# apple/ml-stable-diffusion

Hardware: AMD Instinct MI355X
Metric: diffusion iter/s (UNet steps/s), SD2.1-base 512x512 fp16 (higher is better)
Workload: dtype fp16; 1 GPU; BASELINE config 2: SD2.1-base (865.9 M-parameter UNet), random-init, denoising iteration at 512x512 (64x64 latents), CFG batch 2 per prompt, DDIM, device-resident loop; unet=sd21-base, latent=64, attention=ORIGINAL, prompts_per_gpu=1, global_batch=2, hip_graph=True, parallelism=dp1 (independent prompts per rank, no data-path collective)

## Files before the change

include/sd_mi355x.h:

```cpp
#ifndef SD_MI355X_H
#define SD_MI355X_H

#include <stddef.h>
#include <stdint.h>

#ifdef __cplusplus
extern "C" {
#endif

typedef enum sd_status {
  SD_OK = 0,
  SD_ERR_INVALID_ARGUMENT = -1,
  SD_ERR_NOT_FOUND = -2,
  SD_ERR_HIP = -3,
  SD_ERR_UNSUPPORTED = -4,
  SD_ERR_INTERNAL = -5
} sd_status;

typedef enum sd_dtype { SD_F16 = 0, SD_F32 = 1 } sd_dtype;

typedef enum sd_attention_impl {
  SD_ATTN_ORIGINAL = 0,
  SD_ATTN_SPLIT_EINSUM = 1,
  SD_ATTN_SPLIT_EINSUM_V2 = 2
} sd_attention_impl;

const char* sd_last_error(void);
const char* sd_version(void);
int sd_device_count(void);

typedef struct sd_weights sd_weights;
int sd_weights_create(sd_weights** out);
int sd_weights_add(sd_weights* w, const char* name, const void* data, sd_dtype dtype, const int64_t* shape,
                   int ndim);
int sd_weights_load_safetensors(sd_weights* w, const char* path, const char* prefix);
int sd_weights_count(const sd_weights* w);
void sd_weights_destroy(sd_weights* w);

#define SD_MAX_LEVELS 6

typedef struct sd_unet_config {
  int32_t batch;
  int32_t in_channels, out_channels;
  int32_t height, width;
  int32_t n_levels;
  int32_t block_out_channels[SD_MAX_LEVELS];
  int32_t down_cross_attn[SD_MAX_LEVELS];
  int32_t up_cross_attn[SD_MAX_LEVELS];
  int32_t layers_per_block;
  int32_t attention_head_dim[SD_MAX_LEVELS];
  int32_t transformer_layers_per_block[SD_MAX_LEVELS];
  int32_t cross_attention_dim;
  int32_t context_len;
  int32_t norm_num_groups;
  float norm_eps;
  int32_t flip_sin_to_cos;
  float freq_shift;
  int32_t addition_time_embed_dim;
  int32_t projection_class_embeddings_input_dim;
  int32_t num_time_ids;
  int32_t support_controlnet;
  int32_t is_controlnet;
  int32_t is_vae_decoder;
  int32_t attention_impl;
  int32_t use_graph;
  int32_t compute_fp32;
} sd_unet_config;

typedef struct sd_unet sd_unet;

int sd_unet_create(const sd_unet_config* cfg, const sd_weights* w, int device, sd_unet** out);
void sd_unet_destroy(sd_unet* u);
int sd_unet_set_attention(sd_unet* u, int impl);
int sd_unet_num_residuals(const sd_unet* u);
size_t sd_unet_device_bytes(const sd_unet* u);

#define SD_FLAG_DEVICE_PTRS 1

typedef struct sd_unet_io {
  const void* sample;
  const void* timestep;
  const void* encoder_hidden_states;
  const void* time_ids;
  const void* text_embeds;
  const void* controlnet_cond;
  const void* const* additional_residuals;
  int32_t num_additional_residuals;
  void* noise_pred;
  void* const* residual_outputs;
  int32_t flags;
  const float* step_noise;
} sd_unet_io;

int sd_unet_forward(sd_unet* u, const sd_unet_io* io);

int sd_unet_time_forward(sd_unet* u, int warmup, int iters, float* ms_per_iter);

int sd_unet_profile(sd_unet* u, int iters, int cap, float* ms, double* flop, char* labels, int label_bytes,
                    int* n_ops);

int sd_tune_set_candidate(int tile, int staging, int splitk);
int sd_tune_set_plan_table(const char* rows, sd_unet* u, int* n_plans);

int sd_unet_denoise_loop(sd_unet* u, const sd_unet_io* io, float* latents, int n_images, int n_steps,
                         const float* timesteps, const float* coef, const float* sample_scale, int history,
                         float guidance_scale, float* history_io, float* ms_per_step);

int sd_unet_attach_controlnets(sd_unet* u, sd_unet* const* controlnets, int n);
int sd_controlnet_set_cond(sd_unet* controlnet, const void* controlnet_cond, int flags);

int sd_vae_decoder_create(const sd_unet_config* cfg, const sd_weights* w, int device, sd_unet** out);
int sd_vae_decode(sd_unet* vae, const void* z, sd_dtype z_dtype, float* image, int flags);
int sd_vae_encoder_create(const sd_unet_config* cfg, const sd_weights* w, int device, sd_unet** out);
int sd_vae_encode(sd_unet* vae, const void* x, sd_dtype x_dtype, float* moments, int flags);

typedef struct sd_text_encoder_config {
  int32_t vocab_size, hidden_size, intermediate_size, num_hidden_layers, num_attention_heads;
  int32_t max_position_embeddings;
  int32_t hidden_act;
  int32_t projection_dim;
  float layer_norm_eps;
  int32_t use_graph;
} sd_text_encoder_config;
typedef struct sd_text_encoder sd_text_encoder;
int sd_text_encoder_create(const sd_text_encoder_config* cfg, const sd_weights* w, int device, sd_text_encoder** out);
void sd_text_encoder_destroy(sd_text_encoder* t);
size_t sd_text_encoder_device_bytes(const sd_text_encoder* t);
int sd_text_encoder_encode(sd_text_encoder* t, const int32_t* input_ids, int eos_index, float* last_hidden_state,
                           float* hidden_embeds, float* pooled);

int sd_op_attention(int impl, const void* q, const void* k, const void* v, void* out, int B, int heads, int d,
                    int Sq, int Sk, int variant, int iters, float* ms);
int sd_op_layernorm(const void* x, const float* weight, const float* bias, void* out, int B, int C, int S, float eps,
                    int iters, float* ms);
int sd_op_groupnorm(const void* x, const float* weight, const float* bias, void* out, int B, int C, int H, int W,
                    int groups, float eps, int silu, int iters, float* ms);
int sd_op_groupnorm_shortcut(const void* x0, const void* x1, const float* gn_weight, const float* gn_bias, const void* w, const float* bias,
                             void* out_gn, void* out_sc, int B, int C0, int C1, int H, int W, int N, int groups, float eps, int silu,
                             int side, int iters, float* ms);
int sd_op_conv2d(const void* x, const void* w, const float* bias, const void* res, void* out, int B, int Cin, int H,
                 int W, int Cout, int ksize, int stride, int upsample, int tile, int splitk, int force_generic,
                 int iters, float* ms);
int sd_op_conv2d_groupnorm(const void* x, const void* w, const float* bias, const void* res, const float* gn_weight,
                           const float* gn_bias, void* conv_out, void* out, int B, int Cin, int H, int W, int Cout, int ksize,
                           int groups, float eps, int silu, int tile, int producer_stats, int* entries, int iters, float* ms);
int sd_op_conv2d_groupnorm_proj(const void* x, const void* w, const float* bias, const void* res, const float* gn_weight,
                                const float* gn_bias, const void* proj_w, const float* proj_bias, void* conv_out, void* out, int B,
                                int Cin, int H, int W, int Cout, int ksize, int Nproj, int groups, float eps, int fold, int tile,
                                int* entries, int iters, float* ms);
int sd_op_conv2d_groupnorm_conv3x3(const void* x, const void* w, const float* bias, const void* res, const float* gn_weight,
                                   const float* gn_bias, const void* w2, const float* bias2, const void* res2, void* conv_out, void* out,
                                   int B, int Cin, int H, int W, int Cout, int ksize, int N2, int groups, float eps, int silu, int fold,
                                   int tile, int staging2, int* entries, int iters, float* ms);
int sd_op_ffn_out_proj(const void* g, const void* w1, const float* b1, const void* res1, const void* w2, const float* b2, const void* res2,
                       void* out, float* gn_sums, int B, int C, int S, int groups, int fused, int iters, float* ms);
int sd_op_cross_attention_fused(const void* x, const float* ln_weight, const float* ln_bias, const void* wq, const void* k,
                                const void* v, void* out, int B, int heads, int Sq, int Sk, float eps, int nst, int iters,
                                float* ms);
int sd_op_cross_attention_block(const void* x, const float* ln_weight, const float* ln_bias, const void* wq, const void* k, const void* v,
                                const void* wo, const float* bo, const void* a1, const void* wo1, const float* bo1, void* out, int B, int heads,
                                int Sq, int Sk, float eps, int fused, int iters, float* ms);
int sd_op_geglu(const void* x, const void* w, const float* bias, void* out, int M, int C, int N2, int iters, float* ms);
int sd_op_geglu_ln(const void* x, const float* ln_weight, const float* ln_bias, const void* w, const float* bias, void* out, int M, int C,
                   int N2, float eps, int kernel, int iters, float* ms);
int sd_op_qkv_ln(const void* x, const float* ln_weight, const float* ln_bias, const void* w, void* out_qk, void* out_vt, int B, int HW, int C,
                 float eps, float q_scale, int vt_perm, int kernel, int iters, float* ms);
int sd_op_gn_proj_qkv(const void* x_in, const void* conv_w, const float* gn_weight, const float* gn_bias, const void* proj_w,
                      const float* proj_bias, const float* ln_weight, const float* ln_bias, const void* wqkv, void* out_h, void* out_qk,
                      void* out_vt, int B, int H, int W, int C, int groups, float gn_eps, float ln_eps, float q_scale, int vt_perm, int fused,
                      int* entries, int iters, float* ms);
int sd_op_timestep_embedding(const float* t, float* out, int n, int dim, int flip_sin_to_cos, float freq_shift);
int sd_numpy_randn(uint32_t seed, double* out, size_t n);
int sd_torch_randn(uint32_t seed, double* out, size_t n);
int sd_philox_randn(uint64_t seed, uint32_t offset, double* out, size_t n);
int sd_calibrate(int device, float* out9);
int sd_selftest_mfma(void);

#ifdef __cplusplus
}
#endif
#endif
```

ml-stable-diffusion_amd/csrc/capi.cpp:

```cpp
#include <algorithm>
#include <climits>
#include <cmath>
#include <cstdlib>
#include <cstring>

#include "unet.h"

namespace sd {
extern thread_local std::string g_last_error;
int selftest_mfma();

namespace {

template <typename F>
int guarded(F&& f) {
  try {
    f();
    g_last_error.clear();
    return kOk;
  } catch (const Error& e) {
    g_last_error = e.what();
    return e.code;
  } catch (const std::bad_alloc&) {
    g_last_error = "out of host memory";
// ... 316 lines not shown
    {
      size_t pb = 0;
      int nc = 0;
      if (perm && attention8_sk_scratch(a, &pb, &nc)) {
        a.sk_part = reinterpret_cast<float*>(sc.dev<char>(pb));
        a.sk_part_bytes = pb;
        a.sk_cnt = sc.dev<unsigned>(nc);
        a.sk_cnt_n = nc;
        SD_HIP(hipMemset(a.sk_cnt, 0, (size_t)nc * sizeof(unsigned)));
      } else {
        SD_REQUIRE(variant < 100, kInvalidArgument, "attention variant %d: the balanced form cannot run this shape", variant);
      }
    }
    sc.timed(iters, ms, [&] { launch_attention(a, sc.stream); });
    std::vector<half_t> ot((size_t)B * Sq * C);
    SD_HIP(hipMemcpy(ot.data(), o, ot.size() * 2, hipMemcpyDeviceToHost));
    half_t* oh = reinterpret_cast<half_t*>(out);
    for (int b = 0; b < B; ++b)
      for (int c = 0; c < C; ++c)
        for (int s = 0; s < Sq; ++s) oh[((size_t)b * C + c) * Sq + s] = ot[((size_t)b * Sq + s) * C + c];
  });
}

int sd_op_layernorm(const void* x, const float* weight, const float* bias, void* out, int B, int C, int S, float eps,
                    int iters, float* ms) {
  return guarded([&] {
    SD_REQUIRE(x && weight && bias && out, kInvalidArgument, "NULL argument");
    Scratch sc;
    std::vector<half_t> xt = nchw_to_nhwc(reinterpret_cast<const half_t*>(x), B, C, 1, S);
    half_t* dx = sc.dev<half_t>(xt.size(), xt.data());
    half_t* dy = sc.dev<half_t>(xt.size());
    float* dw = sc.dev<float>(C, weight);
    float* db = sc.dev<float>(C, bias);
    sc.timed(iters, ms, [&] { launch_layernorm(dx, dw, db, dy, B * S, C, eps, sc.stream); });
    SD_HIP(hipMemcpy(xt.data(), dy, xt.size() * 2, hipMemcpyDeviceToHost));
    nhwc_to_nchw(xt.data(), reinterpret_cast<half_t*>(out), B, C, 1, S);
  });
}

int sd_op_groupnorm(const void* x, const float* weight, const float* bias, void* out, int B, int C, int H, int W,
                    int groups, float eps, int silu, int iters, float* ms) {
  return guarded([&] {
    SD_REQUIRE(x && weight && bias && out, kInvalidArgument, "NULL argument");
    Scratch sc;
    std::vector<half_t> xt = nchw_to_nhwc(reinterpret_cast<const half_t*>(x), B, C, H, W);
    half_t* dx = sc.dev<half_t>(xt.size(), xt.data());
    half_t* dy = sc.dev<half_t>(xt.size());
    float* dw = sc.dev<float>(C, weight);
    float* db = sc.dev<float>(C, bias);
    float* partial = sc.dev<float>(groupnorm_scratch_floats(B, H * W, groups));
    sc.timed(iters, ms, [&] {
      launch_groupnorm(dx, C, nullptr, 0, partial, dw, db, dy, B, H * W, groups, eps, silu, sc.stream);
    });
    SD_HIP(hipMemcpy(xt.data(), dy, xt.size() * 2, hipMemcpyDeviceToHost));
    nhwc_to_nchw(xt.data(), reinterpret_cast<half_t*>(out), B, C, H, W);
  });
}

int sd_op_groupnorm_shortcut(const void* x0, const void* x1, const float* gn_weight, const float* gn_bias, const void* w, const float* bias,
                             void* out_gn, void* out_sc, int B, int C0, int C1, int H, int W, int N, int groups, float eps, int silu,
                             int side, int iters, float* ms) {
  return guarded([&] {
    SD_REQUIRE(x0 && gn_weight && gn_bias && w && out_gn && out_sc, kInvalidArgument, "NULL argument");
    if (!x1) C1 = 0;
    const int C = C0 + C1;
    Scratch sc;
    std::vector<half_t> x0t = nchw_to_nhwc(reinterpret_cast<const half_t*>(x0), B, C0, H, W);
    half_t* d0 = sc.dev<half_t>(x0t.size(), x0t.data());
    half_t* d1 = nullptr;
    if (x1) {
      std::vector<half_t> x1t = nchw_to_nhwc(reinterpret_cast<const half_t*>(x1), B, C1, H, W);
      d1 = sc.dev<half_t>(x1t.size(), x1t.data());
    }
    const size_t gn_n = (size_t)B * H * W * C, sc_n = (size_t)B * H * W * N;
    half_t* dy = sc.dev<half_t>(gn_n);
    half_t* ds = sc.dev<half_t>(sc_n);
    float* dgw = sc.dev<float>(C, gn_weight);
    float* dgb = sc.dev<float>(C, gn_bias);
    float* partial = sc.dev<float>(groupnorm_scratch_floats(B, H * W, groups));
    ConvDesc d;
    d.x0 = d0;
    d.C0 = C0;
    d.x1 = d1;
    d.C1 = C1;
    d.w = sc.dev<half_t>((size_t)N * C, reinterpret_cast<const half_t*>(w));
    d.bias = bias ? sc.dev<float>(N, bias) : nullptr;
    d.out = ds;
    d.B = B; d.Hi = H; d.Wi = W; d.Ho = H; d.Wo = W;
    d.N = N;
    SD_REQUIRE(conv_fast_path_ok(d), kInvalidArgument, "groupnorm_shortcut: C0=%d C1=%d N=%d not MFMA-tileable", C0, C1, N);
    SD_REQUIRE(!side || gn_side_gemm_ok(d), kUnsupported, "groupnorm_shortcut: the GEMM cannot ride in the GroupNorm launch (M=%d)", B * H * W);
    ConvWorkspace ws;
    ws.partial_bytes = conv_workspace_bytes(d);
    if (ws.partial_bytes) ws.partial = reinterpret_cast<float*>(sc.dev<char>(ws.partial_bytes));
    sc.timed(iters, ms, [&] {
      if (side) {
        launch_groupnorm(d0, C0, d1, C1, partial, dgw, dgb, dy, B, H * W, groups, eps, silu, sc.stream, 0, &d);
      } else {
        launch_groupnorm(d0, C0, d1, C1, partial, dgw, dgb, dy, B, H * W, groups, eps, silu, sc.stream);
        launch_conv(d, ws, sc.stream);
      }
    });
    std::vector<half_t> ot(gn_n);
    SD_HIP(hipMemcpy(ot.data(), dy, gn_n * 2, hipMemcpyDeviceToHost));
    nhwc_to_nchw(ot.data(), reinterpret_cast<half_t*>(out_gn), B, C, H, W);
    ot.resize(sc_n);
    SD_HIP(hipMemcpy(ot.data(), ds, sc_n * 2, hipMemcpyDeviceToHost));
    nhwc_to_nchw(ot.data(), reinterpret_cast<half_t*>(out_sc), B, N, H, W);
  });
}

int sd_op_conv2d(const void* x, const void* w, const float* bias, const void* res, void* out, int B, int Cin, int H,
                 int W, int Cout, int ksize, int stride, int upsample, int tile, int splitk, int force_generic,
                 int iters, float* ms) {
  return guarded([&] {
    SD_REQUIRE(x && w && out, kInvalidArgument, "NULL argument");
    SD_REQUIRE((ksize == 1 || ksize == 3) && (stride == 1 || stride == 2) && (upsample == 0 || upsample == 1),
               kInvalidArgument, "conv2d: ksize %d stride %d upsample %d not on the path", ksize, stride, upsample);
    Scratch sc;
    const int up = upsample ? 2 : 1, pad = ksize / 2;
    const int Ho = (H * up + 2 * pad - ksize) / stride + 1, Wo = (W * up + 2 * pad - ksize) / stride + 1;
    std::vector<half_t> xt = nchw_to_nhwc(reinterpret_cast<const half_t*>(x), B, Cin, H, W);
    const half_t* wh = reinterpret_cast<const half_t*>(w);
    const int kk = ksize * ksize;
    std::vector<half_t> wt((size_t)Cout * Cin * kk);
    for (int o = 0; o < Cout; ++o)
      for (int c = 0; c < Cin; ++c)
        for (int t = 0; t < kk; ++t) wt[((size_t)o * kk + t) * Cin + c] = wh[((size_t)o * Cin + c) * kk + t];
    ConvDesc d;
    d.x0 = sc.dev<half_t>(xt.size(), xt.data());
    d.C0 = Cin;
    d.w = sc.dev<half_t>(wt.size(), wt.data());
    d.bias = bias ? sc.dev<float>(Cout, bias) : nullptr;
    std::vector<half_t> rt;
    if (res) {
      rt = nchw_to_nhwc(reinterpret_cast<const half_t*>(res), B, Cout, Ho, Wo);
      d.res = sc.dev<half_t>(rt.size(), rt.data());
    }
    const size_t on = (size_t)B * Ho * Wo * Cout;
    half_t* dout = sc.dev<half_t>(on);
    d.out = dout;
    d.B = B; d.Hi = H; d.Wi = W; d.Ho = Ho; d.Wo = Wo;
    d.ksize = ksize; d.stride = stride; d.up = up; d.N = Cout;
    d.tile = tile % 10;
    d.staging = tile / 10;
    if (tile >= 110 && tile <= 116) {
      d.tile = 11;
      d.staging = tile - 110;
    }
    if (tile >= 140 && tile <= 142) {
      d.tile = 12;
      d.staging = tile - 140;
    }
    d.splitk = splitk;
    d.debug = force_generic >= 2 ? force_generic - 1 : 0;
    if (d.debug & 4) d.prof = sc.dev<long long>(8);
    const bool fast = force_generic != 1 && conv_fast_path_ok(d);
    ConvWorkspace ws;
    if (fast && d.tile == 9) {
      SD_REQUIRE(wstream_shape_ok(d), kInvalidArgument, "conv2d: shape not eligible for plan tile 9 (wstream.hip)");
      half_t* wtd = sc.dev<half_t>(wstream_tiled_halves(Cout, Cin, ksize));
      launch_wstream_retile(d.w, wtd, Cout, Cin, ksize, sc.stream);
      d.w_tiled = wtd;
    }
    if (fast && d.tile == 11) {
      SD_REQUIRE(bvgemm_shape_ok(d), kInvalidArgument, "conv2d: shape not eligible for plan tile 11 (bvgemm.hip)");
      half_t* wtd = sc.dev<half_t>(bvgemm_tiled_halves(Cout, Cin));
      launch_bvgemm_retile(d.w, wtd, Cout, Cin, false, sc.stream);
      d.w_bv = wtd;
    }
    if (fast && d.tile != 11 && d.tile != 12) {
      ws.partial_bytes = conv_workspace_bytes(d);
      if (ws.partial_bytes) ws.partial = reinterpret_cast<float*>(sc.dev<char>(ws.partial_bytes));
    }
    const bool small_n = !fast && force_generic == 0 && Cout <= 8 && Cin % 8 == 0 && ksize == 3 && stride == 1 && !res;
    sc.timed(iters, ms, [&] {
      if (fast)
        launch_conv(d, ws, sc.stream);
      else if (small_n)
        launch_conv_small_n(d, nullptr, sc.stream);
      else
        launch_conv_generic(d, 0, sc.stream);
    });
    if (d.prof) {
      long long t[8];
      SD_HIP(hipMemcpy(t, d.prof, sizeof(t), hipMemcpyDeviceToHost));
      fprintf(stderr, "[sd prof] block0: prologue %lld, k-loop %lld, epilogue %lld shader cycles; total %lld cycles = %lld ticks of the 100 MHz wall clock\n",
              t[1] - t[0], t[2] - t[1], t[3] - t[2], t[3] - t[0], t[4]);
    }
    std::vector<half_t> ot(on);
    SD_HIP(hipMemcpy(ot.data(), dout, on * 2, hipMemcpyDeviceToHost));
    nhwc_to_nchw(ot.data(), reinterpret_cast<half_t*>(out), B, Cout, Ho, Wo);
  });
}

int sd_op_conv2d_groupnorm(const void* x, const void* w, const float* bias, const void* res, const float* gn_weight,
                           const float* gn_bias, void* conv_out, void* out, int B, int Cin, int H, int W, int Cout, int ksize,
                           int groups, float eps, int silu, int tile, int producer_stats, int* entries, int iters, float* ms) {
  return guarded([&] {
    SD_REQUIRE(x && w && gn_weight && gn_bias && out, kInvalidArgument, "NULL argument");
    SD_REQUIRE(ksize == 1 || ksize == 3, kInvalidArgument, "conv2d_groupnorm: ksize %d", ksize);
    Scratch sc;
    std::vector<half_t> xt = nchw_to_nhwc(reinterpret_cast<const half_t*>(x), B, Cin, H, W);
    const half_t* wh = reinterpret_cast<const half_t*>(w);
    const int kk = ksize * ksize;
    std::vector<half_t> wt((size_t)Cout * Cin * kk);
    for (int o = 0; o < Cout; ++o)
      for (int c = 0; c < Cin; ++c)
        for (int t = 0; t < kk; ++t) wt[((size_t)o * kk + t) * Cin + c] = wh[((size_t)o * Cin + c) * kk + t];
    ConvDesc d;
    d.x0 = sc.dev<half_t>(xt.size(), xt.data());
    d.C0 = Cin;
    d.w = sc.dev<half_t>(wt.size(), wt.data());
    d.bias = bias ? sc.dev<float>(Cout, bias) : nullptr;
    std::vector<half_t> rt;
    if (res) {
      rt = nchw_to_nhwc(reinterpret_cast<const half_t*>(res), B, Cout, H, W);
      d.res = sc.dev<half_t>(rt.size(), rt.data());
    }
    const size_t on = (size_t)B * H * W * Cout;
    half_t* dconv = sc.dev<half_t>(on);
    half_t* dy = sc.dev<half_t>(on);
    d.out = dconv;
    d.B = B; d.Hi = H; d.Wi = W; d.Ho = H; d.Wo = W;
    d.ksize = ksize; d.stride = 1; d.up = 1; d.N = Cout;
    d.tile = tile % 10;
    d.staging = tile / 10;
    d.splitk = 1;
    const bool fast = conv_fast_path_ok(d);
    float* partial = sc.dev<float>(groupnorm_scratch_floats(B, H * W, groups));
    {
      std::vector<float> poison(groupnorm_scratch_floats(B, H * W, groups), 1.0e30f);
      SD_HIP(hipMemcpy(partial, poison.data(), poison.size() * sizeof(float), hipMemcpyHostToDevice));
    }
    if (producer_stats == 1) {
      d.gn_partial = partial;
      d.gn_groups = groups;
    }
    float* dgw = sc.dev<float>(Cout, gn_weight);
    float* dgb = sc.dev<float>(Cout, gn_bias);
    ConvWorkspace ws;
    if (fast && d.tile == 9) {
      SD_REQUIRE(wstream_shape_ok(d), kInvalidArgument, "conv2d_groupnorm: shape not eligible for plan tile 9");
      half_t* wtd = sc.dev<half_t>(wstream_tiled_halves(Cout, Cin, ksize));
      launch_wstream_retile(d.w, wtd, Cout, Cin, ksize, sc.stream);
      d.w_tiled = wtd;
    }
    if (producer_stats == 2) {
      SD_REQUIRE(fast, kInvalidArgument, "conv2d_groupnorm: GroupNorm twins need the MFMA path");
      d.n_twins = 1;
      d.twin[0].y = dy;
      d.twin[0].ld = Cout;
      d.twin[0].c_off = 0;
      d.twin[0].cpg = Cout / groups;
      d.twin[0].gamma = dgw;
      d.twin[0].beta = dgb;
      d.twin[0].eps = eps;
      d.twin[0].silu = silu;
      SD_REQUIRE(Cout % groups == 0 && reduce_twin_ok(H * W, Cout, 1, d.twin), kInvalidArgument,
                 "conv2d_groupnorm: shape not eligible for a GroupNorm twin (HW=%d C=%d groups=%d)", H * W, Cout, groups);
    }
    if (fast) {
      ws.partial_bytes = conv_workspace_bytes(d);
      if (ws.partial_bytes) ws.partial = reinterpret_cast<float*>(sc.dev<char>(ws.partial_bytes));
    }
    int n_entries = 0;
    sc.timed(iters, ms, [&] {
      n_entries = fast ? launch_conv(d, ws, sc.stream) : launch_conv_generic(d, 0, sc.stream);
      if (producer_stats != 2)
        launch_groupnorm(dconv, Cout, nullptr, 0, partial, dgw, dgb, dy, B, H * W, groups, eps, silu, sc.stream, n_entries);
    });
    if (entries) *entries = n_entries;
    std::vector<half_t> ot(on);
    if (conv_out) {
      SD_HIP(hipMemcpy(ot.data(), dconv, on * 2, hipMemcpyDeviceToHost));
      nhwc_to_nchw(ot.data(), reinterpret_cast<half_t*>(conv_out), B, Cout, H, W);
    }
    SD_HIP(hipMemcpy(ot.data(), dy, on * 2, hipMemcpyDeviceToHost));
    nhwc_to_nchw(ot.data(), reinterpret_cast<half_t*>(out), B, Cout, H, W);
  });
}

int sd_op_conv2d_groupnorm_proj(const void* x, const void* w, const float* bias, const void* res, const float* gn_weight,
                                const float* gn_bias, const void* proj_w, const float* proj_bias, void* conv_out, void* out, int B,
                                int Cin, int H, int W, int Cout, int ksize, int Nproj, int groups, float eps, int fold, int tile,
                                int* entries, int iters, float* ms) {
  return guarded([&] {
    SD_REQUIRE(x && w && gn_weight && gn_bias && proj_w && out, kInvalidArgument, "NULL argument");
    SD_REQUIRE(ksize == 1 || ksize == 3, kInvalidArgument, "conv2d_groupnorm_proj: ksize %d", ksize);
    Scratch sc;
    std::vector<half_t> xt = nchw_to_nhwc(reinterpret_cast<const half_t*>(x), B, Cin, H, W);
    const half_t* wh = reinterpret_cast<const half_t*>(w);
    const int kk = ksize * ksize;
    std::vector<half_t> wt((size_t)Cout * Cin * kk);
    for (int o = 0; o < Cout; ++o)
      for (int c = 0; c < Cin; ++c)
        for (int t = 0; t < kk; ++t) wt[((size_t)o * kk + t) * Cin + c] = wh[((size_t)o * Cin + c) * kk + t];
    ConvDesc d;
    d.x0 = sc.dev<half_t>(xt.size(), xt.data());
    d.C0 = Cin;
    d.w = sc.dev<half_t>(wt.size(), wt.data());
    d.bias = bias ? sc.dev<float>(Cout, bias) : nullptr;
    std::vector<half_t> rt;
    if (res) {
      rt = nchw_to_nhwc(reinterpret_cast<const half_t*>(res), B, Cout, H, W);
      d.res = sc.dev<half_t>(rt.size(), rt.data());
    }
    const size_t on = (size_t)B * H * W * Cout, pn = (size_t)B * H * W * Nproj;
    half_t* dconv = sc.dev<half_t>(on);
    half_t* dnorm = sc.dev<half_t>(on);
    half_t* dy = sc.dev<half_t>(pn);
    d.out = dconv;
    d.B = B; d.Hi = H; d.Wi = W; d.Ho = H; d.Wo = W;
    d.ksize = ksize; d.stride = 1; d.up = 1; d.N = Cout;
    d.tile = tile % 10;
    d.staging = tile / 10;
    d.splitk = 1;
    SD_REQUIRE(conv_fast_path_ok(d), kInvalidArgument, "conv2d_groupnorm_proj: the producer must run on the MFMA path");
    const size_t pf = groupnorm_scratch_floats(B, H * W, groups);
    float* partial = sc.dev<float>(pf);
    {
      std::vector<float> poison(pf, 1.0e30f);
      SD_HIP(hipMemcpy(partial, poison.data(), pf * sizeof(float), hipMemcpyHostToDevice));
    }
    d.gn_partial = partial;
    d.gn_groups = groups;
    float* dgw = sc.dev<float>(Cout, gn_weight);
    float* dgb = sc.dev<float>(Cout, gn_bias);
    ConvDesc pd;
    pd.C0 = Cout;
    pd.w = sc.dev<half_t>((size_t)Nproj * Cout, reinterpret_cast<const half_t*>(proj_w));
    pd.bias = proj_bias ? sc.dev<float>(Nproj, proj_bias) : nullptr;
    pd.out = dy;
    pd.B = B; pd.Hi = H; pd.Wi = W; pd.Ho = H; pd.Wo = W;
    pd.N = Nproj;
    SD_REQUIRE(conv_fast_path_ok(pd), kInvalidArgument, "conv2d_groupnorm_proj: the projection must run on the MFMA path");
    ConvWorkspace ws;
    ws.partial_bytes = std::max(conv_workspace_bytes(d), conv_workspace_bytes(pd));
    if (ws.partial_bytes) ws.partial = reinterpret_cast<float*>(sc.dev<char>(ws.partial_bytes));
    int n_entries = 0;
    sc.timed(iters, ms, [&] {
      n_entries = launch_conv(d, ws, sc.stream);
      ConvDesc pp = pd;
      if (fold && n_entries >= 1 && n_entries <= 128) {
        pp.x0 = dconv;
// ... 867 lines not shown
```

ml-stable-diffusion_amd/csrc/igemm.hip:

```cpp
#include <cstdio>
#include <cstdlib>
#include <cstring>
#include <string>
#include <type_traits>

#include "kernels.h"

namespace sd {

namespace {

constexpr int BK = 64;
constexpr int LDS_ROW = BK + 8;

struct IgemmArgs {
  const half_t* x0;
  const half_t* x1;
  const half_t* w;
  const float* bias;
  const float* temb;
  const half_t* res;
  half_t* out;
  float* partial;
  int C0, C1, Ctot;
// ... 1047 lines not shown
        const char* ws = Ws + ((unsigned)(st + 1) % D) * (BN * ROWB);
        read_step(nx, nw, xs, ws, tapn);
        const bool w_live = !LAST || tap + D < 9;
        if (w_live) issue_next_w();
        if constexpr (GNL) {
          if (!LAST) {
            if (tap == 0) {
              issue_x_piece(0, rsn, offn[0], soffn, xst ^ 1);
              issue_x_piece(1, rsn, offn[1], soffn, xst ^ 1);
            } else if (tap <= 4) {
              issue_x_piece(tap + 1, rsn, offn[tap + 1 < HALO_PPW ? tap + 1 : 0], soffn, xst ^ 1);
            }
            if (tap == 3) {
              gn_transform(0, xst ^ 1, ch + 1);
              gn_transform(1, xst ^ 1, ch + 1);
            } else if (tap >= 4 && tap <= 7) {
              gn_transform(tap - 2, xst ^ 1, ch + 1);
            }
          }
        } else {
          const bool x_live = !LAST && tap < HALO_PPW;
          if (x_live) issue_x_piece(tap, rsn, offn[tap < HALO_PPW ? tap : 0], soffn, xst ^ 1);
        }
        mfma_step(cx, cw);
        if constexpr (DBG == 0) {
#pragma unroll
          for (int g = 0; g < 4; ++g) {
            __builtin_amdgcn_sched_group_barrier(0x008, 1, 0);
            __builtin_amdgcn_sched_group_barrier(0x100, 2, 0);
          }
#pragma unroll
          for (int g = 0; g < 3; ++g) {
            __builtin_amdgcn_sched_group_barrier(0x008, 1, 0);
            __builtin_amdgcn_sched_group_barrier(0x010, 1, 0);
          }
          __builtin_amdgcn_sched_group_barrier(0x008, 1, 0);
        }
      };
      if (((tap + PAR) & 1) == 0) body(xfA, wfA, xfB, wfB);
      else body(xfB, wfB, xfA, wfA);
      __builtin_amdgcn_sched_barrier(0);
    }
  };
  {
    using T = std::true_type;
    using F = std::false_type;
    using P0 = std::integral_constant<int, 0>;
    using P1 = std::integral_constant<int, 1>;
    int ch = ch_begin;
    for (; ch + 2 < ch_end; ch += 2) {
      chunk(P0{}, F{}, ch);
      chunk(P1{}, F{}, ch + 1);
    }
    if (ch + 2 == ch_end) {
      chunk(P0{}, F{}, ch);
      chunk(P1{}, T{}, ch + 1);
    } else if (ch + 1 == ch_end) {
      chunk(P0{}, T{}, ch);
    }
  }
  asm volatile("s_waitcnt vmcnt(0) lgkmcnt(0)" ::: "memory");
  __syncthreads();

  {
    floatx4* red = reinterpret_cast<floatx4*>(smem);
#pragma unroll
    for (int j = 0; j < 2; ++j)
#pragma unroll
      for (int q = 0; q < 4; ++q) {
        floatx4 v;
#pragma unroll
        for (int e = 0; e < 4; ++e) v[e] = wk ? acc[0][j][4 * q + e] : acc[1][j][4 * q + e];
        red[((wave * 2 + j) * 4 + q) * 64 + lane] = v;
      }
    if (tid < BN) sconst[tid] = const_b + const_t;
    __syncthreads();
  }
  floatx16 fin[2];
  {
    const floatx4* red = reinterpret_cast<const floatx4*>(smem);
#pragma unroll
    for (int j = 0; j < 2; ++j)
#pragma unroll
      for (int q = 0; q < 4; ++q) {
        const floatx4 v = red[(((wave ^ 1) * 2 + j) * 4 + q) * 64 + lane];
#pragma unroll
        for (int e = 0; e < 4; ++e) fin[j][4 * q + e] = (wk ? acc[1][j][4 * q + e] : acc[0][j][4 * q + e]) + v[e];
      }
  }
  const int ml = (wm * 2 + wk) * 32 + frow;
  if (a.slab) {
    const int y = y0 + (ml >> 4), x = x0 + (ml & 15);
    if (y < H && x < W) {
      const int m = (b * H + y) * W + x;
      float* prow = a.partial + ((size_t)split * a.M + m) * a.N;
#pragma unroll
      for (int j = 0; j < 2; ++j)
#pragma unroll
        for (int q = 0; q < 4; ++q) {
          const int n = n_blk + j * 32 + 8 * q + 4 * hi;
          if (n < a.N) {
            floatx4 v = {fin[j][4 * q], fin[j][4 * q + 1], fin[j][4 * q + 2], fin[j][4 * q + 3]};
            out_store(reinterpret_cast<floatx4*>(prow + n), v);
          }
        }
    }
    return;
  }
  constexpr int OROW = BN + 8;
  half_t* ot = reinterpret_cast<half_t*>(smem + 32 * 1024);
#pragma unroll
  for (int j = 0; j < 2; ++j)
#pragma unroll
    for (int q = 0; q < 4; ++q) {
      const int nl = j * 32 + 8 * q + 4 * hi;
      const floatx4 bb = *reinterpret_cast<const floatx4*>(sconst + nl);
      half4 o = {(half_t)(fin[j][4 * q] + bb[0]), (half_t)(fin[j][4 * q + 1] + bb[1]), (half_t)(fin[j][4 * q + 2] + bb[2]),
                 (half_t)(fin[j][4 * q + 3] + bb[3])};
      *reinterpret_cast<half4*>(ot + ml * OROW + nl) = o;
    }
  __syncthreads();
  constexpr int WC = BN / 8;
  const bool gn = a.gn_partial != nullptr;
  float fs[8] = {0.f, 0.f, 0.f, 0.f, 0.f, 0.f, 0.f, 0.f}, fq[8] = {0.f, 0.f, 0.f, 0.f, 0.f, 0.f, 0.f, 0.f};
  for (int idx = tid; idx < BM * WC; idx += 256) {
    const int r = idx / WC, c = idx - r * WC;
    const int y = y0 + (r >> 4), x = x0 + (r & 15);
    const int n = n_blk + c * 8;
    if (y < H && x < W && n < a.N) {
      const size_t m = (size_t)(b * H + y) * W + x;
      half8 v = *reinterpret_cast<const half8*>(ot + r * OROW + c * 8);
      half_t* dst = a.out + m * a.N + n;
      if (n + 8 <= a.N) {
        if (a.res) {
          const half8 rr = *reinterpret_cast<const half8*>(a.res + m * a.N + n);
#pragma unroll
          for (int e = 0; e < 8; ++e) v[e] = (half_t)((float)v[e] + (float)rr[e]);
        }
        out_store(reinterpret_cast<half8*>(dst), v);
        if (gn) {
#pragma unroll
          for (int e = 0; e < 8; ++e) {
            const float f = (float)v[e];
            fs[e] += f;
            fq[e] = fmaf(f, f, fq[e]);
          }
        }
      } else {
        for (int e = 0; e < a.N - n; ++e) dst[e] = a.res ? (half_t)((float)v[e] + (float)a.res[m * a.N + n + e]) : v[e];
      }
    }
  }
  if (gn) tile_gn_stats<BN>(a, reinterpret_cast<float*>(smem), fs, fq, n_blk, b, ty * a.tiles_x + tx);
}

#undef HALO_SRC

template <int BM, int BN, int WGM, int WGN, int D, bool LNF, int DBG = 0, bool GNF = false>
__device__ __forceinline__ void gemm_pipe_body(const IgemmArgs& a, int bid_in, int split) {
  static_assert(!(GNF && LNF), "one fold at a time");
  static_assert(WGM * WGN == 4, "4 waves");
  constexpr int TM = BM / WGM / 32, TN = BN / WGN / 32;
  constexpr int XR = BM / 32, WR = BN / 32, PER = ((DBG & 2) ? 0 : XR) + ((DBG & 1) ? 0 : WR), ROWB = BK * 2, KK = BK / 16;
  static_assert(DBG != 3, "one operand must still arrive");
  static_assert((D - 1) * PER <= 63, "vmcnt range");
  extern __shared__ __attribute__((aligned(16))) char smem[];
  char* const Xs = smem;
  char* const Ws = smem + D * BM * ROWB;
  float* sconst = reinterpret_cast<float*>(smem + (size_t)D * (BM + BN) * ROWB);
  float* gn_stat = sconst + 2 * BN;
  half_t* gn_tab = reinterpret_cast<half_t*>(gn_stat + 128);

  const int tid = threadIdx.x, lane = tid & 63;
  const int wave = __builtin_amdgcn_readfirstlane(tid >> 6);
  const int wm = wave / WGN, wn = wave % WGN;
  const int nbm = (a.M + BM - 1) / BM, nbn = (a.N + BN - 1) / BN;
  const int nwg = nbm * nbn;
  int bid = bid_in;
  {
    int q = nwg >> 3, r = nwg & 7, xcd = bid & 7, idx = bid >> 3;
    int base = (xcd < r) ? xcd * (q + 1) : r * (q + 1) + (xcd - r) * q;
    bid = base + idx;
  }
  const int bn_idx = a.n_fast ? bid % nbn : bid / nbm, bm_idx = a.n_fast ? bid / nbn : bid % nbm;
  const int m_blk = bm_idx * BM, n_blk = bn_idx * BN;
  const int kt_begin = split * a.nk_per_split;
  int kt_end = kt_begin + a.nk_per_split;
  if (kt_end > a.nk_total) kt_end = a.nk_total;
  const int T = kt_end - kt_begin;

  constexpr unsigned kOob = 0x80000000u;
  const int pchunk = tid & 7, lrow = tid >> 3;
  const unsigned lchunk = (unsigned)(pchunk ^ ((lrow >> 1) & 7)) * 16u;
  unsigned xoff0[XR], xoff1[XR], woff[WR];
#pragma unroll
  for (int i = 0; i < XR; ++i) {
    const int m = m_blk + lrow + 32 * i;
    xoff0[i] = m < a.M ? (unsigned)m * (unsigned)a.C0 * 2u + lchunk : kOob;
    xoff1[i] = m < a.M ? (unsigned)m * (unsigned)a.C1 * 2u + lchunk : kOob;
  }
#pragma unroll
  for (int i = 0; i < WR; ++i) {
    int n = n_blk + lrow + 32 * i;
    if (n > a.N - 1) n = a.N - 1;
    woff[i] = (unsigned)n * (unsigned)a.K * 2u + lchunk;
  }
  const unsigned x0_bytes = (unsigned)((size_t)a.M * a.C0 * 2), x1_bytes = (unsigned)((size_t)a.M * a.C1 * 2);
  const unsigned w_bytes = (unsigned)((size_t)a.N * a.K * 2);

  int iw_kt = kt_begin, iw_stage = 0;
  auto issue_tile = [&]() {
    const bool live = iw_kt < kt_end;
    const int k = iw_kt * BK;
    const bool second = k >= a.C0;
    const __amdgpu_buffer_rsrc_t rs_x = __builtin_amdgcn_make_buffer_rsrc(
        const_cast<half_t*>(second ? a.x1 : a.x0), 0, (int)(live ? (second ? x1_bytes : x0_bytes) : 0u), 0x00020000);
    const __amdgpu_buffer_rsrc_t rs_w =
        __builtin_amdgcn_make_buffer_rsrc(const_cast<half_t*>(a.w), 0, (int)(live ? w_bytes : 0u), 0x00020000);
    const int xs_off = (second ? k - a.C0 : k) * 2;
    char* xs = Xs + iw_stage * (BM * ROWB) + wave * 1024;
    char* ws = Ws + iw_stage * (BN * ROWB) + wave * 1024;
    if constexpr ((DBG & 2) == 0) {
#pragma unroll
      for (int i = 0; i < XR; ++i) dma16_to_lds(rs_x, xs + i * 4096, second ? xoff1[i] : xoff0[i], xs_off);
    }
    if constexpr ((DBG & 1) == 0) {
#pragma unroll
      for (int i = 0; i < WR; ++i) dma16_to_lds(rs_w, ws + i * 4096, woff[i], k * 2);
    }
    ++iw_kt;
    iw_stage = (iw_stage + 1 == D) ? 0 : iw_stage + 1;
  };

  floatx16 acc[TM][TN];
#pragma unroll
  for (int i = 0; i < TM; ++i)
#pragma unroll
    for (int j = 0; j < TN; ++j)
#pragma unroll
      for (int r = 0; r < 16; ++r) acc[i][j][r] = 0.f;
  float ln_s1[TM] = {}, ln_s2[TM] = {};

  const int frow = lane & 31, hi = lane >> 5;
  const int fsw = (frow >> 1) & 7;
  int foff[KK];
#pragma unroll
  for (int kk = 0; kk < KK; ++kk) foff[kk] = ((kk * 2 + hi) ^ fsw) * 16;
  const int xrow = (wm * TM * 32 + frow) * ROWB, wrow = (wn * TN * 32 + frow) * ROWB;

  const bool temb_uniform = a.temb != nullptr && (a.HoWo % BM) == 0;
  float const_b = 0.f, const_t = 0.f, const_c = 0.f;
  if (!a.slab && tid < BN) {
    const int n = n_blk + tid;
    if (n < a.N) {
      if (a.bias) const_b = a.bias[n];
      if (temb_uniform) const_t = a.temb[(size_t)(m_blk / a.HoWo) * a.temb_stride + n];
      if constexpr (LNF) const_c = a.ln_colsum[n];
    }
  }
  constexpr int RIT = BM * BN / 8 / 256;
  constexpr bool RES_PRE = RIT <= 4;
  half8 resv[RES_PRE ? RIT : 1];
  const bool use_resv = RES_PRE && a.res_pre && a.res != nullptr && !a.slab && a.out_mode == kOutHalf && n_blk < a.n_trans;
  if constexpr (RES_PRE) {
    if (use_resv) {
#pragma unroll
      for (int it = 0; it < RIT; ++it) {
        const int idx = tid + it * 256;
        const int r = idx / (BN / 8), c = idx - r * (BN / 8);
        const int m = m_blk + r, n = n_blk + c * 8;
        const half8 z = {0, 0, 0, 0, 0, 0, 0, 0};
        resv[it] = (m < a.M && n + 8 <= a.ldo) ? *reinterpret_cast<const half8*>(a.res + (size_t)m * a.ldo + n) : z;
      }
    }
  }

  struct Frags {
    half8 x[KK][TM];
    half8 w[KK][TN];
    half8 gm[GNF ? KK : 1], gs[GNF ? KK : 1], gh[GNF ? KK : 1];
  };
  int rd_kt = kt_begin;
  auto read_step = [&](Frags& f, int stage) {
    const char* xs = Xs + stage * (BM * ROWB) + xrow;
    const char* ws = Ws + stage * (BN * ROWB) + wrow;
#pragma unroll
    for (int kk = 0; kk < KK; ++kk) {
#pragma unroll
      for (int i = 0; i < TM; ++i) f.x[kk][i] = *reinterpret_cast<const half8*>(xs + i * 32 * ROWB + foff[kk]);
#pragma unroll
      for (int j = 0; j < TN; ++j) f.w[kk][j] = *reinterpret_cast<const half8*>(ws + j * 32 * ROWB + foff[kk]);
      if constexpr (GNF) {
        const int k0 = rd_kt * BK + (kk * 2 + hi) * 8;
        f.gm[kk] = *reinterpret_cast<const half8*>(gn_tab + k0);
        f.gs[kk] = *reinterpret_cast<const half8*>(gn_tab + a.K + k0);
        f.gh[kk] = *reinterpret_cast<const half8*>(gn_tab + 2 * a.K + k0);
      }
    }
    ++rd_kt;
  };
  auto mfma_step = [&](const Frags& f) {
#pragma unroll
    for (int kk = 0; kk < KK; ++kk) {
#pragma unroll
      for (int i = 0; i < TM; ++i) {
        half8 xv = f.x[kk][i];
// ... 488 lines not shown
  const int b = row / a.Ho, oy = row - b * a.Ho, ox0 = gx * PX;
  const half8 z = {0, 0, 0, 0, 0, 0, 0, 0};
  half8 xv[3][PX + 2];
#pragma unroll
  for (int r = 0; r < 3; ++r) {
    const int iy = oy - 1 + r;
#pragma unroll
    for (int c = 0; c < PX + 2; ++c) {
      const int ix = ox0 - 1 + c;
      const bool ok = live && iy >= 0 && iy < a.Hi && ix >= 0 && ix < a.Wi;
      xv[r][c] = ok ? *reinterpret_cast<const half8*>(a.x0 + (((size_t)b * a.Hi + iy) * a.Wi + ix) * a.C0 + cl * 8) : z;
    }
  }
  half8 wv[NMAX][9];
#pragma unroll
  for (int n = 0; n < NMAX; ++n)
#pragma unroll
    for (int t = 0; t < 9; ++t)
      wv[n][t] = (live && n < a.N) ? *reinterpret_cast<const half8*>(a.w + (size_t)n * a.K + (size_t)t * a.Ctot + cl * 8) : z;
  float acc[NMAX][PX];
#pragma unroll
  for (int n = 0; n < NMAX; ++n)
#pragma unroll
    for (int px = 0; px < PX; ++px) acc[n][px] = 0.f;
#pragma unroll
  for (int r = 0; r < 3; ++r)
#pragma unroll
    for (int kx = 0; kx < 3; ++kx)
#pragma unroll
      for (int px = 0; px < PX; ++px)
#pragma unroll
        for (int n = 0; n < NMAX; ++n)
#pragma unroll
          for (int e = 0; e < 4; ++e) {
            const half2v x2 = {xv[r][px + kx][2 * e], xv[r][px + kx][2 * e + 1]};
            const half2v w2 = {wv[n][r * 3 + kx][2 * e], wv[n][r * 3 + kx][2 * e + 1]};
            acc[n][px] = __builtin_amdgcn_fdot2(x2, w2, acc[n][px], false);
          }
#pragma unroll
  for (int n = 0; n < NMAX; ++n)
#pragma unroll
    for (int px = 0; px < PX; ++px) {
      float v = acc[n][px];
#pragma unroll
      for (int o = LPC / 2; o > 0; o >>= 1) v += __shfl_xor(v, o);
      acc[n][px] = v;
    }
  const int sel = cl & 15;
  float v = 0.f;
#pragma unroll
  for (int n = 0; n < NMAX; ++n)
#pragma unroll
    for (int px = 0; px < PX; ++px) v = (sel == n * PX + px) ? acc[n][px] : v;
  const int n = sel >> 2, px = sel & 3;
  if (g < total && cl < 16 && n < a.N) {
    v += a.bias ? a.bias[n] : 0.f;
    const int rem = oy * a.Wo + ox0 + px;
    if (out_nchw)
      out_nchw[((size_t)b * a.N + n) * a.HoWo + rem] = v;
    else
      a.out[((size_t)b * a.HoWo + rem) * a.N + n] = (half_t)v;
  }
}

const half_t* device_zero_chunk() {
  static half_t* p = nullptr;
  if (!p) {
    SD_HIP(hipMalloc(reinterpret_cast<void**>(&p), 256));
    SD_HIP(hipMemset(p, 0, 256));
    SD_HIP(hipDeviceSynchronize());
  }
  return p;
}

IgemmArgs make_args(const ConvDesc& d) {
  IgemmArgs a{};
  a.x0 = d.x0;
  a.x1 = d.x1;
  a.w = d.w;
  a.bias = d.bias;
  a.temb = d.temb;
  a.res = d.res;
  a.out = d.out;
  a.partial = nullptr;
  a.C0 = d.C0;
  a.C1 = d.x1 ? d.C1 : 0;
  a.Ctot = a.C0 + a.C1;
  a.B = d.B;
  a.Hi = d.Hi;
  a.Wi = d.Wi;
  a.Ho = d.Ho;
  a.Wo = d.Wo;
  a.HoWo = d.Ho * d.Wo;
  a.ksize = d.ksize;
  a.stride = d.stride;
  a.up = d.up;
  a.pad = d.pad >= 0 ? d.pad : d.ksize / 2;
  a.M = d.B * d.Ho * d.Wo;
  a.N = d.N;
  a.K = d.ksize * d.ksize * a.Ctot;
  a.temb_stride = d.temb_stride;
  a.nk_total = a.K / BK;
  a.nk_per_split = a.nk_total;
  a.splitk = 1;
  a.slab = 0;
  a.out_mode = d.out_mode;
  a.ldT = d.ldT;
  a.debug = d.debug;
  a.prof = d.prof;
  a.zeros = device_zero_chunk();
  a.tiles_x = cdiv(d.Wo, 16);
  a.tiles_y = cdiv(d.Ho, 8);
  a.ln_colsum = d.ln_colsum;
  a.ln_eps = d.ln_eps;
  a.n_trans = d.out_t ? d.n_trans : 0x7fffffff;
  a.ldo = d.out_t ? d.n_trans : d.N;
  a.out_t = d.out_t;
  a.vt_perm = d.out_t ? d.vt_perm : 0;
  static const int res_pre = tune_env_int("SD_RES_PREFETCH", 1) != 0;
  a.res_pre = res_pre;
  a.gn_partial = nullptr;
  a.gn_G = a.gn_cpg = a.gn_T = 0;
  a.gnf_partial = d.gnf_partial;
  a.gnf_gamma = d.gnf_gamma;
  a.gnf_beta = d.gnf_beta;
  a.gnf_eps = d.gnf_eps;
  a.gnf_G = d.gnf_groups;
  a.gnf_entries = d.gnf_entries;
  a.q_scale = d.q_scale;
  a.q_cols = d.out_t ? d.q_cols : 0;
  return a;
}

struct Plan {
  int tile;
  int splitk;
  int staging = 0;
};

bool halo_ks_ok(const ConvDesc& d) {
  const int c1 = d.x1 ? d.C1 : 0;
  return d.ksize == 3 && d.stride == 1 && (d.up == 1 || d.up == 2) && d.pad < 0 && d.out_mode == kOutHalf && d.Wo >= 8 && d.Ho >= 8 &&
         d.C0 % BK == 0 && c1 % BK == 0 && d.N % 4 == 0;
}

bool gemm_pipe_ok(const IgemmArgs& a) {
  const size_t lim = (size_t)1 << 31;
  return a.ksize == 1 && a.stride == 1 && a.up == 1 && (size_t)a.M * std::max(a.C0, a.C1) * 2 < lim && (size_t)a.N * a.K * 2 < lim;
}

void tile_dims(int tile, int& bm, int& bn) {
  switch (tile) {
    case 7: bm = 128; bn = 64; break;
    case 1: bm = 128; bn = 128; break;
    case 2: bm = 128; bn = 64; break;
    case 3: bm = 64; bn = 64; break;
    default: bm = 64; bn = 128; break;
  }
}

struct TunedConv { int kind, ksize, stride, up, ctot, n, m, tile, staging, splitk; };
#if __has_include("tuned_convs.inc")
static const TunedConv kTuned[] = {
#include "tuned_convs.inc"
};
static const int kNumTuned = sizeof(kTuned) / sizeof(kTuned[0]);
#else
static const TunedConv* kTuned = nullptr;
static const int kNumTuned = 0;
#endif

bool parse_plan_row(const char* line, TunedConv& r) {
  return sscanf(line, " {%d, %d, %d, %d, %d, %d, %d, %d, %d, %d}", &r.kind, &r.ksize, &r.stride, &r.up, &r.ctot, &r.n, &r.m, &r.tile,
                &r.staging, &r.splitk) == 10;
}
std::vector<TunedConv>& runtime_table() {
  static std::vector<TunedConv> table = [] {
    std::vector<TunedConv> t;
    const char* path = tune_env_set("SD_PLAN_TABLE") ? getenv("SD_PLAN_TABLE") : nullptr;
    if (!path) return t;
    FILE* f = fopen(path, "r");
    if (!f) {
      fprintf(stderr, "[sd] SD_PLAN_TABLE=%s cannot be opened - ignored\n", path);
      return t;
    }
    char line[512];
    while (fgets(line, sizeof(line), f)) {
      TunedConv r;
      if (parse_plan_row(line, r)) t.push_back(r);
    }
    fclose(f);
    fprintf(stderr, "[sd] SD_PLAN_TABLE=%s: %zu plans\n", path, t.size());
    return t;
  }();
  return table;
}

struct TuneCandidate { int tile = 0, staging = 0, splitk = 0; };
TuneCandidate g_tune;

int conv_kind(const ConvDesc& d) {
  if (d.out_t) return 3;
  if (d.out_mode == kOutGeglu) return 2;
  return d.ln_colsum ? 1 : 0;
}

Plan choose_plan(const ConvDesc& d, const IgemmArgs& a) {
  Plan p{d.tile, d.splitk};
  p.staging = d.staging;
  const bool geglu = d.out_mode == kOutGeglu;
  const bool can_split = d.out_mode == kOutHalf && !d.ln_colsum && !d.out_t;
  auto is_halo = [](int c) { return c == 7; };
  static const int ws_mode = tune_env_int("SD_WSTREAM", 1);
  auto tile_ok = [&](int c) {
    if (c == 9) return ws_mode != 0 && d.w_tiled != nullptr && can_split && wstream_shape_ok(d);
    if (!((c >= 1 && c <= 4) || c == 7)) return false;
    if (is_halo(c)) return halo_ks_ok(d) && !d.ln_colsum && !d.out_t && !geglu;
    int bm, bn;
    tile_dims(c, bm, bn);
    if (geglu && c != 1 && c != 4) return false;
    if (d.out_t && d.n_trans % bn != 0) return false;
    return true;
  };
  if (!tile_ok(p.tile)) p.tile = 0;
  auto blocks_of = [&](int c) {
    int bm, bn;
    tile_dims(c, bm, bn);
    const long mt = is_halo(c) ? (long)a.B * a.tiles_x * a.tiles_y : cdiv(a.M, bm);
    return mt * cdiv(a.N, bn);
  };
  auto ksteps = [&](int c) { return is_halo(c) ? a.Ctot / BK : a.nk_total; };
  auto max_split = [&](int c) {
    const int per_min = is_halo(c) ? 2 : 16;
    int s = 1;
    while (can_split && s < 16 && ksteps(c) / (s * 2) >= per_min) s *= 2;
    return s;
  };
  const bool pinned = p.tile != 0 || p.splitk != 0 || p.staging != 0;
  if (!pinned && g_tune.tile != 0 && tile_ok(g_tune.tile)) {
    p.tile = g_tune.tile;
    p.staging = g_tune.staging;
    p.splitk = g_tune.splitk;
  } else if (!pinned) {
    const int kind = conv_kind(d);
    auto match = [&](const TunedConv& t) {
      return t.kind == kind && t.ksize == a.ksize && t.stride == a.stride && t.up == a.up && t.ctot == a.Ctot && t.n == a.N &&
             t.m == a.M && tile_ok(t.tile);
    };
    const TunedConv* hit = nullptr;
    for (const TunedConv& t : runtime_table())
      if (!hit && match(t)) hit = &t;
    for (int i = 0; i < kNumTuned && !hit; ++i)
      if (match(kTuned[i])) hit = &kTuned[i];
    if (hit) {
      p.tile = hit->tile;
      p.staging = hit->staging;
      p.splitk = hit->splitk;
    }
  }
  if (p.tile == 0 && tile_ok(9) && a.ksize == 3 && a.HoWo <= 64 && a.M <= 256) p.tile = 9;
  if (p.tile == 9) {
    p.splitk = 1;
    return p;
  }
  if (p.tile == 0 && tile_ok(7)) {
    p.tile = 7;
    if (p.staging == 0) p.staging = 3;
  }
  if (p.tile == 0) {
    p.tile = 3;
    for (int c : {1, 2, 4, 3}) {
      if (!tile_ok(c)) continue;
      if (blocks_of(c) * max_split(c) >= 384 || c == 3) { p.tile = c; break; }
    }
    if (!tile_ok(p.tile)) p.tile = 4;
  }
  if (p.splitk == 0) {
    p.splitk = 1;
    const int ms = max_split(p.tile);
    const long want = p.tile == 7 ? 192 : 384;
    while (blocks_of(p.tile) * p.splitk < want && p.splitk < ms) p.splitk *= 2;
  }
  if (!can_split) p.splitk = 1;
  if (p.splitk > ksteps(p.tile)) p.splitk = ksteps(p.tile);
  if (p.splitk < 1) p.splitk = 1;
  return p;
}

constexpr size_t halo_gnl_lds_cap = 160 * 1024;
inline size_t halo_gnl_lds_bytes(int d, int ctot) {
  const size_t k_loop = halo_lds_bytes(64, d) - 64 * sizeof(float) + (((size_t)6 * ctot + 15) & ~(size_t)15);
  const size_t epilogue = 32 * 1024 + 128 * (64 + 8) * 2 + 64 * sizeof(float);
  return std::max(k_loop, epilogue);
}
template <int D, int DBG = 0, bool GNL = false>
void launch_halo_ks_d(const IgemmArgs& a, hipStream_t s) {
  const size_t lds = GNL ? halo_gnl_lds_bytes(D, a.Ctot) : halo_lds_bytes(64, D);
  static_assert(halo_lds_bytes(64, D) <= 160 * 1024, "LDS");
  auto k = conv3x3_halo_ks_kernel<D, DBG, GNL>;
  static DynLdsOnce once;
  once.set(k, GNL ? halo_gnl_lds_cap : lds);
  dim3 grid(a.B * a.tiles_x * a.tiles_y * cdiv(a.N, 64), a.splitk);
  hipLaunchKernelGGL(k, grid, dim3(256), lds, s, a);
}

void launch_halo_ks(IgemmArgs a, int splitk, int staging, hipStream_t s) {
  const int nch = a.Ctot / BK;
  a.nk_total = nch;
  a.nk_per_split = cdiv(nch, splitk);
  a.splitk = cdiv(nch, a.nk_per_split);
  if (a.debug >= 32) {
    switch (a.debug - 32) {
      case 1: launch_halo_ks_d<4, 1>(a, s); return;
      case 2: launch_halo_ks_d<4, 2>(a, s); return;
      case 3: launch_halo_ks_d<4, 3>(a, s); return;
      case 4: launch_halo_ks_d<4, 4>(a, s); return;
      case 8: launch_halo_ks_d<4, 8>(a, s); return;
      case 12: launch_halo_ks_d<4, 12>(a, s); return;
      case 13: launch_halo_ks_d<4, 13>(a, s); return;
      case 14: launch_halo_ks_d<4, 14>(a, s); return;
      case 15: launch_halo_ks_d<4, 15>(a, s); return;
      default: break;
    }
  }
  if (a.gnf_partial) {
    if (staging >= 3 && halo_gnl_lds_bytes(4, a.Ctot) <= halo_gnl_lds_cap) launch_halo_ks_d<4, 0, true>(a, s);
    else launch_halo_ks_d<3, 0, true>(a, s);
    return;
  }
  if (staging >= 5) { launch_halo_ks_d<8>(a, s); return; }
  if (staging >= 4) { launch_halo_ks_d<6>(a, s); return; }
  if (staging >= 3) { launch_halo_ks_d<4>(a, s); return; }
  if (staging >= 2) { launch_halo_ks_d<3>(a, s); return; }
  launch_halo_ks_d<2>(a, s);
}

template <int BM, int BN, int WGM, int WGN, bool TRANS, bool GLDS, int NST, bool LNF = false, int KG = 1>
void launch_variant(const IgemmArgs& a, hipStream_t s) {
  const size_t lds = (size_t)KG * NST * (BM + BN) * (GLDS ? BK : LDS_ROW) * sizeof(half_t) + 2 * BN * sizeof(float);
  static_assert((size_t)KG * NST * (BM + BN) * BK * sizeof(half_t) + 2 * BN * sizeof(float) <= 160 * 1024, "LDS");
  static_assert((size_t)BN * (BM + 8) <= (size_t)NST * (BM + BN) * (GLDS ? BK : LDS_ROW), "transposed staging fits");
  static_assert((size_t)BM * (BN + 8) * 2 + 16 + (kGnScratchFloats + 2 * BN) * sizeof(float) <=
                    (size_t)NST * (BM + BN) * (GLDS ? BK : LDS_ROW) * sizeof(half_t),
                "GroupNorm statistics scratch fits behind the staged tile");
  dim3 grid(cdiv(a.M, BM) * cdiv(a.N, BN), a.splitk);
  auto k = igemm_kernel<BM, BN, WGM, WGN, TRANS, GLDS, NST, 0, LNF, KG>;
  static DynLdsOnce once;
  once.set(k, lds);
  hipLaunchKernelGGL(k, grid, dim3(256 * KG), lds, s, a);
}

template <int BM, int BN, int DBG>
void launch_debug(const IgemmArgs& a, hipStream_t s) {
  const size_t lds = (size_t)2 * (BM + BN) * BK * sizeof(half_t) + 2 * BN * sizeof(float);
  dim3 grid(cdiv(a.M, BM) * cdiv(a.N, BN), a.splitk);
  auto k = igemm_kernel<BM, BN, 2, 2, false, true, 2, DBG>;
  SD_HIP(hipFuncSetAttribute((const void*)k, hipFuncAttributeMaxDynamicSharedMemorySize, (int)lds));
  hipLaunchKernelGGL(k, grid, dim3(256), lds, s, a);
}
template <int BM, int BN>
bool launch_debug_mode(const IgemmArgs& a, int dbg, hipStream_t s) {
  switch (dbg) {
    case 4: launch_debug<BM, BN, 4>(a, s); return true;
    case 5: launch_debug<BM, BN, 5>(a, s); return true;
    case 6: launch_debug<BM, BN, 6>(a, s); return true;
    case 14: launch_debug<BM, BN, 14>(a, s); return true;
    case 22: launch_debug<BM, BN, 22>(a, s); return true;
    case 30: launch_debug<BM, BN, 30>(a, s); return true;
    default: return false;
  }
}

constexpr size_t kLdsBudget = 160 * 1024;
template <int BM, int BN>
constexpr size_t ring_bytes(int nst) {
  return (size_t)nst * (BM + BN) * BK * sizeof(half_t);
}
template <int BM, int BN>
constexpr bool ring_fits(int nst) {
  return (size_t)nst * (BM + BN) * BK * sizeof(half_t) + 2 * BN * sizeof(float) <= kLdsBudget;
}
template <int BM, int BN, int WGM, int WGN, int D, bool LNF>
void launch_pipe_dbg(const IgemmArgs& a, hipStream_t s) {
  constexpr size_t lds = (size_t)D * (BM + BN) * BK * sizeof(half_t) + 2 * BN * sizeof(float);
  dim3 grid(cdiv(a.M, BM) * cdiv(a.N, BN), a.splitk);
  if (a.debug == 65) {
    auto k = gemm_pipe_kernel<BM, BN, WGM, WGN, D, LNF, 1>;
    SD_HIP(hipFuncSetAttribute((const void*)k, hipFuncAttributeMaxDynamicSharedMemorySize, (int)lds));
    hipLaunchKernelGGL(k, grid, dim3(256), lds, s, a);
  } else {
    auto k = gemm_pipe_kernel<BM, BN, WGM, WGN, D, LNF, 2>;
    SD_HIP(hipFuncSetAttribute((const void*)k, hipFuncAttributeMaxDynamicSharedMemorySize, (int)lds));
    hipLaunchKernelGGL(k, grid, dim3(256), lds, s, a);
  }
}

template <int BM, int BN, int WGM, int WGN, int D, bool LNF>
void launch_pipe(const IgemmArgs& a, hipStream_t s) {
  constexpr size_t lds = (size_t)D * (BM + BN) * BK * sizeof(half_t) + 2 * BN * sizeof(float);
  static_assert(lds <= kLdsBudget, "LDS");
  static_assert((size_t)BM * (BN + 8) * 2 + 16 + (kGnScratchFloats + 2 * BN) * sizeof(float) <= (size_t)D * (BM + BN) * BK * sizeof(half_t),
                "staged tile + GroupNorm statistics scratch fit the K-loop buffers");
  static_assert((size_t)BN * (BM + 8) <= (size_t)D * (BM + BN) * BK, "transposed staging fits");
  dim3 grid(cdiv(a.M, BM) * cdiv(a.N, BN), a.splitk);
  if constexpr (D == 2 && !LNF) {
    if (a.debug == 65 || a.debug == 66) {
      launch_pipe_dbg<BM, BN, WGM, WGN, D, LNF>(a, s);
      return;
    }
  }
  if constexpr (BM == 64 && BN == 64 && !LNF) {
    if (a.gnf_partial) {
      const size_t lds_g = lds + 128 * sizeof(float) + (size_t)3 * a.K * sizeof(half_t);
      auto kg = gemm_pipe_kernel<BM, BN, WGM, WGN, D, false, 0, true>;
      static DynLdsOnce once_g;
      once_g.set(kg, lds + 128 * sizeof(float) + (size_t)3 * 2048 * sizeof(half_t));
      hipLaunchKernelGGL(kg, grid, dim3(256), lds_g, s, a);
      return;
    }
  }
  auto k = gemm_pipe_kernel<BM, BN, WGM, WGN, D, LNF>;
  static DynLdsOnce once;
  once.set(k, lds);
  hipLaunchKernelGGL(k, grid, dim3(256), lds, s, a);
}
template <int BM, int BN, int WGM, int WGN, bool LNF>
void launch_ring(const IgemmArgs& a, int staging, hipStream_t s) {
  if (staging == 12 || staging == 13) {
    if constexpr (!LNF) {
      if (a.nk_per_split >= 4) {
        if (staging == 13) {
          if constexpr (2 * ring_bytes<BM, BN>(4) + 2 * BN * sizeof(float) <= kLdsBudget) { launch_variant<BM, BN, WGM, WGN, false, true, 4, false, 2>(a, s); return; }
        }
        if constexpr (2 * ring_bytes<BM, BN>(3) + 2 * BN * sizeof(float) <= kLdsBudget) { launch_variant<BM, BN, WGM, WGN, false, true, 3, false, 2>(a, s); return; }
      }
    }
    staging -= 10;
  }
  if (staging == 8 && gemm_pipe_ok(a)) {
    launch_pipe<BM, BN, WGM, WGN, 2, LNF>(a, s);
    return;
  }
  if ((staging == 6 || staging == 7) && gemm_pipe_ok(a)) {
    if (staging == 7) {
      if constexpr (ring_fits<BM, BN>(4)) { launch_pipe<BM, BN, WGM, WGN, 4, LNF>(a, s); return; }
    }
    launch_pipe<BM, BN, WGM, WGN, 3, LNF>(a, s);
    return;
  }
  if (staging >= 6) staging = 3;
  if (staging >= 5) {
    if constexpr (ring_fits<BM, BN>(8)) { launch_variant<BM, BN, WGM, WGN, false, true, 8, LNF>(a, s); return; }
  }
  if (staging >= 4) {
    if constexpr (ring_fits<BM, BN>(6)) { launch_variant<BM, BN, WGM, WGN, false, true, 6, LNF>(a, s); return; }
  }
  if (staging >= 3) {
    if constexpr (ring_fits<BM, BN>(4)) { launch_variant<BM, BN, WGM, WGN, false, true, 4, LNF>(a, s); return; }
  }
  if (staging >= 2) { launch_variant<BM, BN, WGM, WGN, false, true, 3, LNF>(a, s); return; }
  launch_variant<BM, BN, WGM, WGN, false, true, 2, LNF>(a, s);
}

template <int BM, int BN, int WGM, int WGN>
void launch_tile(const IgemmArgs& a, bool trans, int staging, hipStream_t s) {
  if (a.ln_colsum) {
    launch_ring<BM, BN, WGM, WGN, true>(a, staging == 1 ? 0 : staging, s);
    return;
  }
  if (trans) {
    if (staging == 1) launch_variant<BM, BN, WGM, WGN, true, false, 2>(a, s);
    else if (staging >= 2) launch_variant<BM, BN, WGM, WGN, true, true, 3>(a, s);
    else launch_variant<BM, BN, WGM, WGN, true, true, 2>(a, s);
  } else {
    if (staging == 1) launch_variant<BM, BN, WGM, WGN, false, false, 2>(a, s);
    else launch_ring<BM, BN, WGM, WGN, false>(a, staging, s);
  }
}

}

bool conv_fast_path_ok(const ConvDesc& d) {
  const int c1 = d.x1 ? d.C1 : 0;
  if (d.C0 % BK != 0 || c1 % BK != 0) return false;
  if (d.N % 4 != 0) return false;
  if (d.out_mode == kOutGeglu && d.N % 64 != 0) return false;
  if (!(d.ksize == 1 || d.ksize == 3)) return false;
  if (!(d.up == 1 || d.up == 2)) return false;
  return true;
}

bool conv_plan_is_wstream(const ConvDesc& d0) {
  if (!conv_fast_path_ok(d0) || !wstream_shape_ok(d0)) return false;
  ConvDesc d = d0;
  if (!d.w_tiled) d.w_tiled = d.w;
  const IgemmArgs a = make_args(d);
  return choose_plan(d, a).tile == 9;
}

size_t conv_workspace_bytes(const ConvDesc& d) {
  if (!conv_fast_path_ok(d)) return 0;
  IgemmArgs a = make_args(d);
  Plan p = choose_plan(d, a);
  static const bool tuning = getenv("SD_TUNE") != nullptr;
  const bool can_split = d.out_mode == kOutHalf && !d.ln_colsum && !d.out_t;
  int splits = (tuning && can_split) ? std::max(p.splitk, 16) : p.splitk;
  bool slab = d.n_twins > 0;
  if (d.w_tiled && can_split && wstream_shape_ok(d)) {
    splits = std::max(splits, wstream_splits(d, 4));
    slab = true;
  }
  if (splits == 1 && slab) return (size_t)a.M * a.N * sizeof(float);
  return splits > 1 ? (size_t)splits * a.M * a.N * sizeof(float) : 0;
}

int conv_plan_table_set(const char* text) {
  std::vector<TunedConv>& t = runtime_table();
  t.clear();
  if (!text) return 0;
  const char* p = text;
  while (*p) {
    const char* e = strchr(p, '\n');
    std::string line(p, e ? (size_t)(e - p) : strlen(p));
    TunedConv r;
    if (parse_plan_row(line.c_str(), r)) t.push_back(r);
    if (!e) break;
    p = e + 1;
  }
  return (int)t.size();
}

void conv_tune_set_candidate(int tile, int staging, int splitk) {
  g_tune.tile = tile;
  g_tune.staging = staging;
  g_tune.splitk = splitk;
}

namespace {
int setup_gn_stats(const ConvDesc& d, IgemmArgs& a, int bm) {
  a.gn_partial = nullptr;
  if (!d.gn_partial || d.gn_groups < 1 || a.splitk > 1 || a.slab || d.out_mode != kOutHalf || d.out_t || d.debug) return 0;
  if (a.N % d.gn_groups != 0 || a.N % 8 != 0) return 0;
  const int cpg = a.N / d.gn_groups;
  if (cpg > 64) return 0;
  int T;
  if (bm == 0) {
    T = a.tiles_x * a.tiles_y;
  } else {
    if (a.HoWo % bm != 0) return 0;
    T = a.HoWo / bm;
  }
  if (2 * T > kGnMaxSlabs) return 0;
  a.gn_partial = d.gn_partial;
  a.gn_G = d.gn_groups;
  a.gn_cpg = cpg;
  a.gn_T = T;
  return 2 * T;
}
}

namespace {
int launch_slab_combine(const ConvDesc& d, IgemmArgs& a, hipStream_t s) {
  static const int stats_mode = tune_env_int("SD_REDUCE_STATS", 0);
  a.gn_partial = nullptr;
  if (stats_mode != 0 && d.gn_partial && d.gn_groups >= 1 && d.gn_groups <= 256 && a.N % d.gn_groups == 0 && (a.N / d.gn_groups) % 4 == 0 &&
      a.HoWo <= 256 && d.out_mode == kOutHalf && !d.out_t) {
    int ppb = std::max(1, a.B * a.HoWo / 512);
    const int slabs = cdiv(a.HoWo, ppb);
    const size_t lds = (size_t)ppb * (a.N / 4) * 2 * sizeof(float);
    if (slabs <= kGnMaxSlabs && lds <= 64 * 1024) {
      a.gn_partial = d.gn_partial;
      a.gn_G = d.gn_groups;
      a.gn_cpg = a.N / d.gn_groups;
      a.gn_T = slabs;
      hipLaunchKernelGGL(splitk_reduce_stats_kernel, dim3(slabs, a.B), dim3(256), lds, s, a, ppb);
      return slabs;
    }
  }
  const size_t total4 = (size_t)a.M * a.N / 4;
  const int blocks = (int)std::min<size_t>((total4 + 255) / 256, 2048);
  hipLaunchKernelGGL(splitk_reduce_kernel, dim3(blocks), dim3(256), 0, s, a);
  return 0;
}
}

namespace {
void choose_tile_order(IgemmArgs& a, int tile) {
  int bm, bn;
  tile_dims(tile, bm, bn);
  const bool halo_tile = tile == 7;
  const double nbn = (double)cdiv(a.N, bn);
  const double nbm = halo_tile ? (double)a.B * a.tiles_x * a.tiles_y : (double)cdiv(a.M, bm);
  const double a_bytes = 2.0 * a.B * a.Hi * a.Wi * a.Ctot, w_bytes = 2.0 * a.N * a.K;
  const double l2 = 3.5e6;
  const double m_fast_cost = w_bytes + a_bytes * (a_bytes <= l2 ? std::min(8.0, nbn) : nbn);
  const double n_fast_cost = a_bytes + w_bytes * (w_bytes <= l2 ? std::min(8.0, nbm) : nbm);
  static const int forced = tune_env_int("SD_TILE_ORDER", -1);
  if (forced == 2) a.n_fast = nbn > 1 && a_bytes * (nbn - 1) > 7.0 * w_bytes;
  else a.n_fast = forced >= 0 ? (forced != 0) : (nbn > 1 && n_fast_cost < m_fast_cost);
}
}

bool conv_gn_loader_ok(const ConvDesc& d) {
  const int c1 = d.x1 ? d.C1 : 0;
  const int ctot = d.C0 + c1;
  return d.ksize == 3 && d.stride == 1 && d.up == 1 && halo_ks_ok(d) && !d.ln_colsum && !d.out_t && d.out_mode == kOutHalf && !d.debug &&
         d.gnf_groups >= 1 && d.gnf_groups <= 32 && ctot % d.gnf_groups == 0 && ctot <= 2048 && d.Hi == d.Ho && d.Wi == d.Wo &&
         halo_gnl_lds_bytes(3, ctot) <= halo_gnl_lds_cap;
}

int launch_conv(const ConvDesc& d, const ConvWorkspace& ws, hipStream_t s) {
  SD_REQUIRE(conv_fast_path_ok(d), kInvalidArgument, "launch_conv: shape not MFMA-tileable (C0=%d C1=%d N=%d k=%d)",
             d.C0, d.C1, d.N, d.ksize);
  SD_REQUIRE(!d.ln_colsum || (d.ksize == 1 && !d.x1 && d.bias && d.out_mode != kOutHalfT), kInvalidArgument,
             "LayerNorm fold needs a 1x1 single-source GEMM with a (folded) bias");
  SD_REQUIRE(!d.out_t || (d.out_mode == kOutHalf && d.n_trans % 64 == 0 && d.n_trans < d.N && (d.Ho * d.Wo) % 8 == 0 &&
                          d.ldT % 8 == 0 && !d.res && !d.temb),
             kInvalidArgument, "fused q|k|v: n_trans %d N %d HoWo %d ldT %d", d.n_trans, d.N, d.Ho * d.Wo, d.ldT);
  SD_REQUIRE(!d.vt_perm || (d.out_t && (d.Ho * d.Wo) % 16 == 0), kInvalidArgument, "permuted V^T needs the fused q|k|v epilogue and HoWo %% 16 == 0");
  SD_REQUIRE(d.q_cols == 0 || (d.out_t && d.q_cols % 4 == 0 && d.q_cols <= d.n_trans), kInvalidArgument, "pre-scaled queries need the fused q|k|v epilogue (q_cols %d)", d.q_cols);
  {
    static const bool wsg_on = tune_env_int("SD_WSGEMM", 1) != 0;
    const bool forced = d.tile == 10;
    if (d.w_ws && wsgemm_shape_ok(d) && (forced || (wsg_on && wsgemm_wanted(d) && d.tile == 0 && d.splitk == 0 && d.staging == 0 && g_tune.tile == 0))) {
      launch_wsgemm(d, s);
      return 0;
    }
    SD_REQUIRE(!forced, kInvalidArgument, "plan tile 10 (wsgemm.hip) needs the pre-tiled weights and an eligible GEGLU shape");
  }
  {
    static const bool bv_on = tune_env_int("SD_BVGEMM", 1) != 0;
    if (bv_on && d.w_bv && d.tile == 0 && d.splitk == 0 && d.staging == 0 && g_tune.tile == 0 && bvgemm_wanted(d)) {
      launch_bvgemm(d, 0, s);
      return 0;
    }
  }
  if (d.tile == 11) {
    SD_REQUIRE(d.w_bv && bvgemm_shape_ok(d), kInvalidArgument, "plan tile 11 (bvgemm.hip) needs the pre-tiled weights and an eligible 1x1 shape");
    launch_bvgemm(d, d.staging, s);
    return 0;
  }
  {
    static const bool sm_on = tune_env_int("SD_SMGEMM", 1) != 0;
    const bool forced = d.tile == 12;
    if (forced || (sm_on && d.tile == 0 && d.splitk == 0 && d.staging == 0 && g_tune.tile == 0 && smgemm_wanted(d))) {
      launch_smgemm(d, forced ? d.staging : 0, s);
      return 0;
    }
  }
  {
    static const bool sg_on = tune_env_int("SD_SMGEGLU", 1) != 0;
    const bool forced = d.tile == 13;
    if (forced || (sg_on && d.tile == 0 && d.splitk == 0 && d.staging == 0 && g_tune.tile == 0 && smgeglu_wanted(d))) {
      launch_smgeglu(d, forced ? d.staging : 0, s);
      return 0;
    }
  }
  IgemmArgs a = make_args(d);
  Plan p = choose_plan(d, a);
  bool halo = p.tile == 7;
  const bool twins = d.n_twins > 0;
  SD_REQUIRE(!twins || (d.out_mode == kOutHalf && !d.ln_colsum && !d.out_t && !d.debug && reduce_twin_ok(a.HoWo, a.N, d.n_twins, d.twin)),
             kInvalidArgument, "GroupNorm twins need a plain fp16 output and whole (sample, group) slices (HoWo=%d N=%d)", a.HoWo, a.N);
  if (d.gnf_partial && d.ksize == 3) {
    SD_REQUIRE(conv_gn_loader_ok(d) && d.gnf_silu == 1 && d.gnf_gamma && d.gnf_beta && d.gnf_entries >= 1 && d.gnf_entries <= 128 && !twins, kInvalidArgument,
               "GroupNorm in the conv loader: Ctot=%d groups=%d entries=%d up=%d", a.Ctot, d.gnf_groups, d.gnf_entries, d.up);
    p.tile = 7;
    if (p.staging != 2 && p.staging != 3) p.staging = 3;
    p.splitk = 1;
  } else if (d.gnf_partial) {
    SD_REQUIRE(d.ksize == 1 && d.stride == 1 && !d.x1 && d.out_mode == kOutHalf && !d.ln_colsum && !d.out_t && !twins && gemm_pipe_ok(a) &&
                   d.gnf_gamma && d.gnf_beta && d.gnf_groups >= 1 && d.gnf_groups <= 32 && a.K % d.gnf_groups == 0 && a.K <= 2048 &&
                   d.gnf_entries >= 1 && d.gnf_entries <= 128 && a.HoWo % 64 == 0,
               kInvalidArgument, "GroupNorm fold: K=%d groups=%d entries=%d HoWo=%d", a.K, d.gnf_groups, d.gnf_entries, a.HoWo);
    p.tile = 3;
    if (p.staging != 6 && p.staging != 7 && p.staging != 8) p.staging = 6;
    p.splitk = 1;
  }
  halo = p.tile == 7;
  if (p.tile == 9) {
    const int nw = p.staging == 4 ? 4 : 8;
    const int S = wstream_splits(d, nw);
    const size_t need = (size_t)S * a.M * a.N * sizeof(float);
    SD_REQUIRE(ws.partial && ws.partial_bytes >= need, kInternal, "wstream workspace too small (%zu < %zu)", ws.partial_bytes, need);
    static const bool log_ws = tune_env_set("SD_LOG_CONVS");
    if (log_ws)
      fprintf(stderr, "[sd conv] k%d up%d C0=%d C1=%d M=%d N=%d K=%d tile=9 nw=%d slabs=%d twins=%d\n", a.ksize, a.up, a.C0, a.C1, a.M, a.N,
              a.K, nw, S, d.n_twins);
    launch_wstream(d, ws.partial, nw, s);
    a.partial = ws.partial;
    a.splitk = S;
    a.slab = 1;
    int entries = 0;
    if (twins) launch_reduce_twin(a.partial, S, a.M, a.N, a.HoWo, a.bias, a.temb, a.temb_stride, a.res, a.out, d.n_twins, d.twin, s);
    else entries = launch_slab_combine(d, a, s);
    SD_HIP(hipGetLastError());
    return entries;
  }
  if (halo) {
    const int nch = a.Ctot / BK;
    a.nk_per_split = cdiv(nch, p.splitk);
    a.splitk = cdiv(nch, a.nk_per_split);
  } else {
    a.splitk = p.splitk;
    a.nk_per_split = cdiv(a.nk_total, p.splitk);
    a.splitk = cdiv(a.nk_total, a.nk_per_split);
  }
  a.slab = (a.splitk > 1 || twins) ? 1 : 0;
  if (a.slab) {
    size_t need = (size_t)a.splitk * a.M * a.N * sizeof(float);
    SD_REQUIRE(ws.partial && ws.partial_bytes >= need, kInternal, "split-K workspace too small (%zu < %zu)",
               ws.partial_bytes, need);
    a.partial = ws.partial;
  }
  const bool trans = d.out_mode == kOutHalfT;
  const int st = p.staging;
  choose_tile_order(a, p.tile);
  static const bool log_plans = tune_env_set("SD_LOG_CONVS");
  if (log_plans)
    fprintf(stderr, "[sd conv] k%d s%d up%d C0=%d C1=%d M=%d N=%d K=%d mode=%d tile=%d splitk=%d\n", a.ksize, a.stride, a.up,
            a.C0, a.C1, a.M, a.N, a.K, d.out_mode, p.tile, a.splitk);
  int gn_entries = 0;
  if (halo) {
    gn_entries = setup_gn_stats(d, a, 0);
    launch_halo_ks(a, a.splitk, st, s);
  } else if (d.debug && d.debug < 64) {
    const bool ok = p.tile == 1 ? launch_debug_mode<128, 128>(a, d.debug, s) : launch_debug_mode<64, 64>(a, d.debug, s);
    SD_REQUIRE(ok && !trans, kInvalidArgument, "no ablation kernel for debug mode %d", d.debug);
    return 0;
  } else {
    if (!trans) {
      int bm, bn;
      tile_dims(p.tile >= 1 && p.tile <= 3 ? p.tile : 4, bm, bn);
      gn_entries = setup_gn_stats(d, a, bm);
    }
    switch (p.tile) {
      case 1: launch_tile<128, 128, 2, 2>(a, trans, st, s); break;
      case 2: launch_tile<128, 64, 2, 2>(a, trans, st, s); break;
      case 3: launch_tile<64, 64, 2, 2>(a, trans, st, s); break;
      default: launch_tile<64, 128, 2, 2>(a, trans, st, s); break;
    }
  }
  if (twins) {
    launch_reduce_twin(a.partial, a.splitk, a.M, a.N, a.HoWo, a.bias, a.temb, a.temb_stride, a.res, a.out, d.n_twins, d.twin, s);
  } else if (a.slab) {
    gn_entries = launch_slab_combine(d, a, s);
  }
  SD_HIP(hipGetLastError());
  return gn_entries;
}

bool gn_side_gemm_ok(const ConvDesc& d) {
  if (!(d.ksize == 1 && d.stride == 1 && d.up == 1 && d.out_mode == kOutHalf && !d.ln_colsum && !d.out_t && d.n_twins == 0 && !d.gnf_partial &&
        !d.gn_partial && !d.temb && !d.debug && conv_fast_path_ok(d)))
    return false;
  const IgemmArgs a = make_args(d);
  return gemm_pipe_ok(a) && a.M >= 256;
}

namespace {
constexpr int kSideD = 4;
IgemmArgs side_args(const ConvDesc& d) {
  SD_REQUIRE(gn_side_gemm_ok(d), kInvalidArgument, "side GEMM: not a plain 1x1 GEMM of the pipelined kernel (C0=%d C1=%d N=%d)", d.C0, d.C1, d.N);
  IgemmArgs a = make_args(d);
  a.splitk = 1;
  a.slab = 0;
  choose_tile_order(a, 3);
  return a;
}
constexpr size_t kSideLds = (size_t)kSideD * (64 + 64) * BK * sizeof(half_t) + 2 * 64 * sizeof(float);
}

void launch_gn_apply_side(const half_t* x0, int C0, const half_t* x1, int C1, const float* partial, int entries, const float* gamma,
                          const float* beta, half_t* y, int B, int HW, int G, float eps, int silu, int slabs, int ppb, const ConvDesc& side,
                          hipStream_t s) {
  IgemmArgs a = side_args(side);
  GnSideArgs g{x0, x1, C0, x1 ? C1 : 0, partial, entries, gamma, beta, y, HW, G, eps, silu, ppb, slabs, B, 0};
  g.n_gn_pad = (slabs * B + 7) / 8 * 8;
  auto k = gn_apply_side_kernel<kSideD>;
  static DynLdsOnce once;
  once.set(k, kSideLds);
  hipLaunchKernelGGL(k, dim3(g.n_gn_pad + cdiv(a.M, 64) * cdiv(a.N, 64)), dim3(256), kSideLds, s, g, a);
  SD_HIP(hipGetLastError());
}

void launch_gn_fused_side(int vw, const half_t* x0, int C0, const half_t* x1, int C1, const float* gamma, const float* beta, half_t* y, int B,
                          int HW, int G, float eps, int silu, const ConvDesc& side, hipStream_t s) {
  IgemmArgs a = side_args(side);
  GnSideArgs g{x0, x1, C0, x1 ? C1 : 0, nullptr, 0, gamma, beta, y, HW, G, eps, silu, 0, G, B, 0};
  g.n_gn_pad = (G * B + 7) / 8 * 8;
  const dim3 grid(g.n_gn_pad + cdiv(a.M, 64) * cdiv(a.N, 64));
  static DynLdsOnce o8, o4, o2;
  if (vw == 8) {
    auto k = gn_fused_side_kernel<8, kSideD>;
    o8.set(k, kSideLds);
    hipLaunchKernelGGL(k, grid, dim3(256), kSideLds, s, g, a);
  } else if (vw == 4) {
    auto k = gn_fused_side_kernel<4, kSideD>;
    o4.set(k, kSideLds);
    hipLaunchKernelGGL(k, grid, dim3(256), kSideLds, s, g, a);
  } else {
    auto k = gn_fused_side_kernel<2, kSideD>;
    o2.set(k, kSideLds);
    hipLaunchKernelGGL(k, grid, dim3(256), kSideLds, s, g, a);
  }
  SD_HIP(hipGetLastError());
}

int launch_conv_generic(const ConvDesc& d, int act_silu_out, hipStream_t s) {
  IgemmArgs a = make_args(d);
  if (a.ksize == 3 && a.stride == 1 && a.up == 1 && a.Ctot == 4 && !d.x1 && d.pad < 0 && d.out_mode == kOutHalf && a.N % 8 == 0 &&
      !d.temb && !act_silu_out) {
    const size_t lds = std::max((size_t)(128 + 64) * BK * 2 + 2 * 64 * sizeof(float),
                                (size_t)128 * (64 + 8) * 2 + 16 + (kGnScratchFloats + 2 * 64) * sizeof(float));
    a.splitk = 1;
    const int gn_entries = setup_gn_stats(d, a, 128);
    hipLaunchKernelGGL(conv3x3_cin4_kernel, dim3(cdiv(a.M, 128) * cdiv(a.N, 64)), dim3(256), lds, s, a);
    SD_HIP(hipGetLastError());
    return gn_entries;
  }
  if (a.K <= SC_KMAX && d.out_mode == kOutHalf && a.N >= 64) {
    hipLaunchKernelGGL(conv_small_cin_kernel, dim3(cdiv(a.M, SC_PIX)), dim3(256), 0, s, a, act_silu_out);
    SD_HIP(hipGetLastError());
    return 0;
  }
  SD_REQUIRE(d.out_mode != kOutGeglu || d.N % 64 == 0, kUnsupported, "generic GEGLU needs N %% 64 == 0 (N=%d)", d.N);
  size_t total = (size_t)a.M * a.N;
  int blocks = (int)std::min<size_t>((total + 255) / 256, 65535);
  hipLaunchKernelGGL(conv_generic_kernel, dim3(blocks), dim3(256), 0, s, a, act_silu_out);
  SD_HIP(hipGetLastError());
  return 0;
}

void launch_conv_small_n(const ConvDesc& d, float* out_nchw_f32, hipStream_t s) {
  IgemmArgs a = make_args(d);
  SD_REQUIRE(a.N <= 8 && a.Ctot % 8 == 0 && a.C0 % 8 == 0, kInvalidArgument, "conv_small_n: N=%d Ctot=%d", a.N,
             a.Ctot);
  static const int rows_mode = tune_env_int("SD_CONV_OUT_ROWS", 1);
  const int chunks = a.Ctot / 8;
  const int lpc = chunks <= 16 ? 16 : (chunks <= 32 ? 32 : 64);
  if (rows_mode != 0 && a.ksize == 3 && a.stride == 1 && a.up == 1 && a.pad == 1 && !d.x1 && a.N <= 4 && chunks <= 64 &&
      a.Wo % 4 == 0 && a.Hi == a.Ho && a.Wi == a.Wo) {
    const int pg = 64 / lpc;
    const int groups = a.B * a.Ho * (a.Wo / 4);
    const dim3 grid(cdiv(cdiv(groups, pg), 4));
    if (lpc == 16) hipLaunchKernelGGL(conv3x3_small_n_rows_kernel<16>, grid, dim3(256), 0, s, a, out_nchw_f32);
    else if (lpc == 32) hipLaunchKernelGGL(conv3x3_small_n_rows_kernel<32>, grid, dim3(256), 0, s, a, out_nchw_f32);
    else hipLaunchKernelGGL(conv3x3_small_n_rows_kernel<64>, grid, dim3(256), 0, s, a, out_nchw_f32);
    SD_HIP(hipGetLastError());
    return;
  }
  hipLaunchKernelGGL(conv_small_n_kernel<8>, dim3(cdiv(a.M, 4)), dim3(256), 0, s, a, out_nchw_f32);
  SD_HIP(hipGetLastError());
}

}
```

ml-stable-diffusion_amd/csrc/kernels.h:

```cpp
#pragma once
#include "sd_common.h"

namespace sd {

enum OutMode : int {
  kOutHalf = 0,
  kOutHalfT = 1,
  kOutGeglu = 2,
};

struct GnTwin {
  half_t* y = nullptr;
  int ld = 0, c_off = 0;
  int cpg = 0;
  const float* gamma = nullptr;
  const float* beta = nullptr;
  float eps = 1e-5f;
  int silu = 0;
};

struct ConvDesc {
  const half_t* x0 = nullptr;
  const half_t* x1 = nullptr;
  int C0 = 0, C1 = 0;
  const half_t* w = nullptr;
  const float* bias = nullptr;
  const float* temb = nullptr;
  int temb_stride = 0;
  const half_t* res = nullptr;
  half_t* out = nullptr;
  int B = 1, Hi = 1, Wi = 1;
  int Ho = 1, Wo = 1;
  int ksize = 1, stride = 1, up = 1;
  int pad = -1;
  int N = 0;
  int out_mode = kOutHalf;
  int ldT = 0;
  int tile = 0;
  int splitk = 0;
  long long* prof = nullptr;
  int debug = 0;
  int staging = 0;
  const float* ln_colsum = nullptr;
  float ln_eps = 1e-5f;
  half_t* out_t = nullptr;
  int n_trans = 0;
  int vt_perm = 0;
  float q_scale = 1.f;
  int q_cols = 0;
  float* gn_partial = nullptr;
  int gn_groups = 0;
  const float* gnf_partial = nullptr;
  const float* gnf_gamma = nullptr;
  const float* gnf_beta = nullptr;
  float gnf_eps = 1e-6f;
  int gnf_groups = 0, gnf_entries = 0;
  int gnf_silu = 0;
  const half_t* w_tiled = nullptr;
  const half_t* w_ws = nullptr;
  const half_t* w_bv = nullptr;
  GnTwin twin[2];
  int n_twins = 0;
};

constexpr int kGnMaxSlabs = 256;

struct ConvWorkspace {
  float* partial = nullptr;
  size_t partial_bytes = 0;
};

size_t conv_workspace_bytes(const ConvDesc& d);
int launch_conv(const ConvDesc& d, const ConvWorkspace& ws, hipStream_t s);
bool conv_fast_path_ok(const ConvDesc& d);
bool conv_gn_loader_ok(const ConvDesc& d);
void conv_tune_set_candidate(int tile, int staging, int splitk);
int conv_plan_table_set(const char* text);

bool conv_plan_is_wstream(const ConvDesc& d);
bool wstream_shape_ok(const ConvDesc& d);
int wstream_splits(const ConvDesc& d, int nw);
size_t wstream_tiled_halves(int N, int Ctot, int ksize);
void launch_wstream_retile(const half_t* w, half_t* wt, int N, int Ctot, int ksize, hipStream_t s);
int launch_wstream(const ConvDesc& d, float* partial, int nw, hipStream_t s);
bool reduce_twin_ok(int HW, int N, int n_twins, const GnTwin* tw);
void launch_reduce_twin(const float* partial, int S, int M, int N, int HW, const float* bias, const float* temb, int temb_stride,
                        const half_t* res, half_t* out, int n_twins, const GnTwin* tw, hipStream_t s);

bool wsgemm_shape_ok(const ConvDesc& d);
bool wsgemm_wanted(const ConvDesc& d);
size_t wsgemm_tiled_halves(int N);
void launch_wsgemm_retile(const half_t* w, half_t* wt, int N, bool geglu, hipStream_t s);
void launch_wsgemm(const ConvDesc& d, hipStream_t s);

bool bvgemm_shape_ok(const ConvDesc& d);
size_t bvgemm_tiled_halves(int N, int K);
void launch_bvgemm_retile(const half_t* w, half_t* wt, int N, int K, bool geglu, hipStream_t s);
void launch_bvgemm(const ConvDesc& d, int variant, hipStream_t s);
bool bvgemm_wanted(const ConvDesc& d);

bool smgemm_shape_ok(const ConvDesc& d, int variant);
bool smgemm_wanted(const ConvDesc& d);
void launch_smgemm(const ConvDesc& d, int variant, hipStream_t s);

bool smgeglu_shape_ok(const ConvDesc& d, int variant);
bool smgeglu_wanted(const ConvDesc& d);
void launch_smgeglu(const ConvDesc& d, int variant, hipStream_t s);
size_t smgeglu_prof_entries(const ConvDesc& d, int variant);

void run_calibration(int device, float* out);

int launch_conv_generic(const ConvDesc& d, int act_silu_out, hipStream_t s);

void launch_conv_small_n(const ConvDesc& d, float* out_nchw_f32, hipStream_t s);

enum AttnImpl : int { kAttnOriginal = 0, kAttnSplitEinsum = 1, kAttnSplitEinsumV2 = 2 };

struct AttnDesc {
  const half_t* q = nullptr;
  const half_t* k = nullptr;
  const half_t* vt = nullptr;
  half_t* out = nullptr;
  int B = 1, heads = 1, d = 64, Sq = 0, Sk = 0;
  int ldq = 0, ldk = 0, ldv = 0, ldo = 0;
  int impl = kAttnOriginal;
  int variant = 0;
  int vt_perm = 0;
  int q_prescaled = 0;
  float* sk_part = nullptr;
  size_t sk_part_bytes = 0;
  unsigned* sk_cnt = nullptr;
  int sk_cnt_n = 0;
  int sk_force = 0;
  int sk_upw = 0;
};
inline float attention_q_prescale(int d) { return 1.4426950408889634f / sqrtf((float)d); }
void launch_attention(const AttnDesc& d, hipStream_t s);
bool attention_supported(int d);
bool attention8_ok(const AttnDesc& d);
bool attention8_shape_ok(int d, int Sq, int Sk);
void launch_attention8(const AttnDesc& d, hipStream_t s);
bool attention8_sk_scratch(const AttnDesc& d, size_t* part_bytes, int* n_counters);

struct XAttnDesc {
  const half_t* x = nullptr;
  const half_t* wq = nullptr;
  const float* bias = nullptr;
  const float* colsum = nullptr;
  const half_t* k = nullptr;
  const half_t* vt = nullptr;
  half_t* out = nullptr;
  int M = 0, C = 0, S = 0, L = 0, ldv = 0, heads = 0;
  float ln_eps = 1e-5f;
  int impl = kAttnOriginal;
  int nst = 0;
};
bool xattn_fused_ok(int C, int heads, int S, int L);
void launch_xattn_fused(const XAttnDesc& d, hipStream_t s);

struct XAttnOutDesc {
  const half_t* x = nullptr;
  const half_t* wq_t = nullptr;
  const float* q_bias = nullptr;
  const float* q_colsum = nullptr;
  const half_t* k = nullptr;
  const half_t* vt = nullptr;
  const half_t* wo_t = nullptr;
  const float* o_bias = nullptr;
  half_t* out = nullptr;
  int M = 0, C = 0, S = 0, L = 0, ldv = 0, heads = 0;
  float ln_eps = 1e-5f;
  int impl = kAttnOriginal;
  const half_t* h0 = nullptr;
  const half_t* wo1_t = nullptr;
  const float* o1_bias = nullptr;
};
struct GnProjQkvDesc {
  const half_t* x = nullptr;
  const float* gn_partial = nullptr;
  const float* gn_gamma = nullptr;
  const float* gn_beta = nullptr;
  int gn_entries = 0, gn_groups = 32;
  float gn_eps = 1e-6f;
  const half_t* wp_t = nullptr;
  const float* p_bias = nullptr;
  half_t* h = nullptr;
  const half_t* wqkv_t = nullptr;
  const float* qkv_bias = nullptr;
  const float* qkv_colsum = nullptr;
  float ln_eps = 1e-5f;
  half_t* qk = nullptr;
  half_t* vt = nullptr;
  int M = 0, C = 0, S = 0, ldT = 0;
  bool vt_perm = false;
  float q_scale = 1.f;
  int tok = 0;
  long long* clk = nullptr;
};
bool gn_proj_qkv_ok(int C, int heads, int S, int M, int ldT, int G);
void launch_gn_proj_qkv(const GnProjQkvDesc& d, hipStream_t s);
bool xattn_out_ok(int C, int heads, int S, int L);
void launch_xattn_out_retile(const half_t* w, half_t* wt, int C, hipStream_t s);
void launch_xattn_out(const XAttnOutDesc& d, hipStream_t s);
struct FfnProjDesc {
  const half_t* g = nullptr;
  const half_t* w1_t = nullptr;
  const float* b1 = nullptr;
  const half_t* res1 = nullptr;
  const half_t* w2_t = nullptr;
  const float* b2 = nullptr;
  const half_t* res2 = nullptr;
  half_t* out = nullptr;
  float* gn_partial = nullptr;
  int gn_groups = 0;
  int M = 0, C = 0, K1 = 0, S = 0;
};
bool ffn_proj_ok(int C, int K1, int M, int S);
int launch_ffn_proj(const FfnProjDesc& d, hipStream_t s);
void launch_xattn_out_retile_nk(const half_t* w, half_t* wt, int N, int K, hipStream_t s);

void launch_layernorm(const half_t* x, const float* w, const float* b, half_t* y, int M, int C, float eps,
                      hipStream_t s);
int groupnorm_num_slabs(int B, int HW);
size_t groupnorm_scratch_floats(int B, int HW, int G);
void launch_groupnorm(const half_t* x0, int C0, const half_t* x1, int C1, float* partial, const float* gamma,
                      const float* beta, half_t* y, int B, int HW, int G, float eps, int silu, hipStream_t s,
                      int producer_entries = 0, const ConvDesc* side = nullptr);
bool gn_side_gemm_ok(const ConvDesc& d);
void launch_gn_apply_side(const half_t* x0, int C0, const half_t* x1, int C1, const float* partial, int entries, const float* gamma,
                          const float* beta, half_t* y, int B, int HW, int G, float eps, int silu, int slabs, int ppb, const ConvDesc& side,
                          hipStream_t s);
void launch_gn_fused_side(int vw, const half_t* x0, int C0, const half_t* x1, int C1, const float* gamma, const float* beta, half_t* y, int B,
                          int HW, int G, float eps, int silu, const ConvDesc& side, hipStream_t s);
bool groupnorm_wants_producer_stats(int HW, int C, int G);

void launch_row_softmax(half_t* x, int rows, int cols, float scale, hipStream_t s);

struct ConvF32Desc {
  const float* x = nullptr;
  const void* w = nullptr;
  int w_kind = 0;
  const float* bias = nullptr;
  const float* res = nullptr;
  float* out = nullptr;
  int B = 1, Hi = 1, Wi = 1, Cin = 0, Ho = 1, Wo = 1, N = 0;
  int ksize = 1, stride = 1, up = 1;
  int pad = -1;
};
void launch_conv_f32(const ConvF32Desc& d, hipStream_t s);
size_t groupnorm_f32_scratch_bytes(int B, int G);
void launch_groupnorm_f32(const float* x, void* scratch, const float* gamma, const float* beta, float* y, int B, int HW, int C, int G,
                          float eps, int silu, hipStream_t s);
// ... 37 lines not shown
```

ml-stable-diffusion_amd/csrc/unet.cpp:

```cpp
#include "unet.h"

#ifndef SD_GN_QKV_DEFAULT
#define SD_GN_QKV_DEFAULT 1
#endif

#include <algorithm>
#include <cmath>
#include <cstdlib>
#include <cstring>

namespace sd {

namespace {
constexpr int kTembCap = 65536;
inline int round_up(int x, int a) { return (x + a - 1) / a * a; }
}

UNet::UNet(const sd_unet_config& cfg, const WeightStore& ws, int device) : cfg_(cfg), ws_(&ws), device_(device) {
  SD_REQUIRE(cfg.n_levels >= 1 && cfg.n_levels <= SD_MAX_LEVELS, kInvalidArgument, "n_levels=%d", cfg.n_levels);
  SD_REQUIRE(cfg.batch >= 1 && cfg.height >= 1 && cfg.width >= 1, kInvalidArgument, "bad batch/size");
  SD_REQUIRE(cfg.norm_num_groups >= 1 && cfg.norm_num_groups <= 64, kUnsupported, "norm_num_groups=%d",
             cfg.norm_num_groups);
  int ndev = 0;
  SD_HIP(hipGetDeviceCount(&ndev));
  SD_REQUIRE(ndev > 0, kHipError, "no HIP device visible: libsdmi355 has no CPU fallback");
  SD_REQUIRE(device >= 0 && device < ndev, kInvalidArgument, "device %d out of range (%d visible)", device, ndev);
  SD_HIP(hipSetDevice(device));
  SD_HIP(hipStreamCreateWithFlags(&stream_, hipStreamNonBlocking));
  if (tune_env_int("SD_SIDE_TIME", 0) != 0) {
    SD_HIP(hipStreamCreateWithFlags(&side_, hipStreamNonBlocking));
    SD_HIP(hipEventCreateWithFlags(&ev_fork_, hipEventDisableTiming));
    SD_HIP(hipEventCreateWithFlags(&ev_join_, hipEventDisableTiming));
  }
  if (cfg_.support_controlnet && !cfg_.is_controlnet && tune_env_int("SD_CN_CONCURRENT", 1) != 0) {
    SD_HIP(hipStreamCreateWithFlags(&cn_stream_, hipStreamNonBlocking));
    SD_HIP(hipEventCreateWithFlags(&ev_cn_fork_, hipEventDisableTiming));
    SD_HIP(hipEventCreateWithFlags(&ev_cn_join_, hipEventDisableTiming));
  }
  f32_ = cfg_.compute_fp32 != 0;
  SD_REQUIRE(!f32_ || cfg_.is_vae_decoder, kUnsupported,
             "compute_fp32 is the VAE graphs' option (torch2coreml.py:570-578, :726-733); the UNet kernels store fp16");
  if (cfg_.is_vae_decoder == 2)
    build_vae_encoder();
  else if (cfg_.is_vae_decoder)
    build_vae_decoder();
  else
    build_unet();
  ws_ = nullptr;
  SD_HIP(hipStreamSynchronize(stream_));
}

UNet::~UNet() {
  (void)hipSetDevice(device_);
  if (graph_) (void)hipGraphExecDestroy(graph_);
  if (loop_graph_) (void)hipGraphExecDestroy(loop_graph_);
  if (stream_) {
    (void)hipStreamSynchronize(stream_);
    (void)hipStreamDestroy(stream_);
  }
  if (side_) {
    (void)hipStreamSynchronize(side_);
    (void)hipStreamDestroy(side_);
    (void)hipEventDestroy(ev_fork_);
    (void)hipEventDestroy(ev_join_);
  }
  if (cn_stream_) {
    (void)hipStreamSynchronize(cn_stream_);
    (void)hipStreamDestroy(cn_stream_);
    (void)hipEventDestroy(ev_cn_fork_);
    (void)hipEventDestroy(ev_cn_join_);
  }
}

Tensor UNet::new_tensor(int B, int H, int W, int C) {
  Tensor t;
  t.B = B;
  t.H = H;
  t.W = W;
  t.C = C;
  t.p = arena_.alloc_n<half_t>(t.numel() * (f32_ ? 2 : 1));
  return t;
}

half_t* UNet::upload_conv_weight(const std::string& name, int cout, int cin, int k, bool geglu) {
  const HostTensor& t = ws_->get(name + ".weight");
  const size_t expect = (size_t)cout * cin * k * k;
  SD_REQUIRE(t.numel() == expect, kInvalidArgument, "%s.weight has %zu elements, expected %zu (%d,%d,%d,%d)",
             name.c_str(), t.numel(), expect, cout, cin, k, k);
  std::vector<half_t> host(expect);
  const int kk = k * k;
  for (int o = 0; o < cout; ++o) {
    int dst_o = o;
    if (geglu) {
      const int half_n = cout / 2;
      const bool gate = o >= half_n;
      const int j = gate ? o - half_n : o;
      dst_o = (j / 32) * 64 + (gate ? 32 : 0) + (j % 32);
    }
    for (int c = 0; c < cin; ++c)
      for (int t2 = 0; t2 < kk; ++t2)
        host[((size_t)dst_o * kk + t2) * cin + c] = (half_t)t.data[((size_t)o * cin + c) * kk + t2];
  }
  half_t* d = arena_.alloc_n<half_t>(expect);
  SD_HIP(hipMemcpy(d, host.data(), expect * sizeof(half_t), hipMemcpyHostToDevice));
  return d;
}

float* UNet::upload_vec(const std::string& name, int n, bool geglu) {
  const HostTensor& t = ws_->get(name);
  SD_REQUIRE((int)t.numel() == n, kInvalidArgument, "%s has %zu elements, expected %d", name.c_str(), t.numel(), n);
  std::vector<float> host(t.data);
  if (geglu) {
    const int half_n = n / 2;
    for (int o = 0; o < n; ++o) {
      const bool gate = o >= half_n;
      const int j = gate ? o - half_n : o;
      host[(j / 32) * 64 + (gate ? 32 : 0) + (j % 32)] = t.data[o];
    }
  }
  float* d = arena_.alloc_n<float>(n);
  SD_HIP(hipMemcpy(d, host.data(), (size_t)n * sizeof(float), hipMemcpyHostToDevice));
  return d;
}

Tensor UNet::conv(std::vector<Op>& ops, const std::string& name, const Tensor& x, const Tensor* x2, int cout, int k,
                  int stride, int up, bool bias, const float* temb, const half_t* res, int out_mode, int ldT,
                  bool silu_out, int pad) {
  const int cin = x.C + (x2 ? x2->C : 0);
  const bool geglu = out_mode == kOutGeglu;
  const float* b = bias ? upload_vec(name + ".bias", cout, geglu) : nullptr;
  if (f32_) {
    const HostTensor& t = ws_->get(name + ".weight");
    const size_t expect = (size_t)cout * cin * k * k;
    SD_REQUIRE(!geglu && t.numel() == expect, kInvalidArgument, "%s.weight has %zu elements, expected %zu", name.c_str(), t.numel(), expect);
    std::vector<float> host(expect);
    const int kk = k * k;
    for (int o = 0; o < cout; ++o)
      for (int c = 0; c < cin; ++c)
        for (int t2 = 0; t2 < kk; ++t2) host[((size_t)o * kk + t2) * cin + c] = t.data[((size_t)o * cin + c) * kk + t2];
    float* d = arena_.alloc_n<float>(expect);
    SD_HIP(hipMemcpy(d, host.data(), expect * sizeof(float), hipMemcpyHostToDevice));
    w_f32_pending_ = true;
    return conv_w(ops, name, reinterpret_cast<const half_t*>(d), b, x, x2, cout, k, stride, up, temb, res, out_mode, ldT, silu_out,
                  nullptr, pad);
  }
  const half_t* w = upload_conv_weight(name, cout, cin, k, geglu);
  return conv_w(ops, name, w, b, x, x2, cout, k, stride, up, temb, res, out_mode, ldT, silu_out, nullptr, pad);
}

Tensor UNet::conv_stacked(std::vector<Op>& ops, const std::vector<std::string>& names, const Tensor& x, int cout_each) {
  const int cin = x.C, n = (int)names.size();
  std::vector<half_t> host((size_t)n * cout_each * cin);
  for (int i = 0; i < n; ++i) {
    const HostTensor& t = ws_->get(names[i] + ".weight");
    SD_REQUIRE(t.numel() == (size_t)cout_each * cin, kInvalidArgument, "%s.weight: bad shape", names[i].c_str());
    for (size_t j = 0; j < t.numel(); ++j) host[(size_t)i * cout_each * cin + j] = (half_t)t.data[j];
  }
  half_t* d = arena_.alloc_n<half_t>(host.size());
  SD_HIP(hipMemcpy(d, host.data(), host.size() * sizeof(half_t), hipMemcpyHostToDevice));
  return conv_w(ops, names[0], d, nullptr, x, nullptr, n * cout_each, 1, 1, 1, nullptr, nullptr, kOutHalf, 0, false);
}

UNet::LnFold UNet::fold_layernorm(const std::string& ln, const std::vector<std::string>& names, int cin, int cout_each,
                                  bool geglu) {
  const HostTensor& g = ws_->get(ln + ".weight");
  const HostTensor& be = ws_->get(ln + ".bias");
  SD_REQUIRE((int)g.numel() == cin && (int)be.numel() == cin, kInvalidArgument, "%s: expected %d channels", ln.c_str(),
             cin);
  const int n = (int)names.size(), ntot = n * cout_each;
  SD_REQUIRE(!geglu || n == 1, kInternal, "GEGLU fold takes one projection");
  std::vector<half_t> w((size_t)ntot * cin);
  std::vector<float> colsum(ntot), bias(ntot);
  for (int i = 0; i < n; ++i) {
    const HostTensor& t = ws_->get(names[i] + ".weight");
    SD_REQUIRE(t.numel() == (size_t)cout_each * cin, kInvalidArgument, "%s.weight: bad shape", names[i].c_str());
    const HostTensor* tb = ws_->has(names[i] + ".bias") ? &ws_->get(names[i] + ".bias") : nullptr;
    SD_REQUIRE(!tb || (int)tb->numel() == cout_each, kInvalidArgument, "%s.bias: bad shape", names[i].c_str());
    for (int o = 0; o < cout_each; ++o) {
      int dst = i * cout_each + o;
      if (geglu) {
        const int half_n = cout_each / 2;
        const bool gate = o >= half_n;
        const int j = gate ? o - half_n : o;
        dst = (j / 32) * 64 + (gate ? 32 : 0) + (j % 32);
      }
      double cs = 0.0, bb = tb ? (double)tb->data[o] : 0.0;
      for (int c = 0; c < cin; ++c) {
        const float wv = t.data[(size_t)o * cin + c];
        const half_t h = (half_t)(wv * g.data[c]);
        w[(size_t)dst * cin + c] = h;
        cs += (double)(float)h;
        bb += (double)wv * (double)be.data[c];
      }
      colsum[dst] = (float)cs;
      bias[dst] = (float)bb;
    }
  }
  LnFold f;
  f.w = arena_.alloc_n<half_t>(w.size());
  f.colsum = arena_.alloc_n<float>(ntot);
  f.bias = arena_.alloc_n<float>(ntot);
  SD_HIP(hipMemcpy(f.w, w.data(), w.size() * sizeof(half_t), hipMemcpyHostToDevice));
  SD_HIP(hipMemcpy(f.colsum, colsum.data(), ntot * sizeof(float), hipMemcpyHostToDevice));
  SD_HIP(hipMemcpy(f.bias, bias.data(), ntot * sizeof(float), hipMemcpyHostToDevice));
  return f;
}

bool UNet::can_fold_ln(const Tensor& x, int cout, bool geglu) const {
  ConvDesc d;
  d.C0 = x.C;
  d.N = cout;
  d.ksize = 1;
  d.out_mode = geglu ? kOutGeglu : kOutHalf;
  static const bool off = tune_env_set("SD_NO_LN_FOLD");
  return !off && conv_fast_path_ok(d);
}

Tensor UNet::conv_w(std::vector<Op>& ops, const std::string& name, const half_t* w, const float* bias, const Tensor& x,
                    const Tensor* x2, int cout, int k, int stride, int up, const float* temb, const half_t* res,
                    int out_mode, int ldT, bool silu_out, ConvExtra* ex, int pad_override) {
  const bool geglu = out_mode == kOutGeglu;
  ConvDesc d;
  d.x0 = x.p;
  d.C0 = x.C;
  if (x2) {
    SD_REQUIRE(x2->B == x.B && x2->H == x.H && x2->W == x.W, kInternal, "%s: concat shape mismatch", name.c_str());
    d.x1 = x2->p;
    d.C1 = x2->C;
  }
  d.w = w;
  d.bias = bias;
  d.temb = temb;
  d.temb_stride = kTembCap;
  d.res = res;
  d.B = x.B;
  d.Hi = x.H;
  d.Wi = x.W;
  const int Hup = x.H * up, Wup = x.W * up, pad = k / 2;
  if (pad_override >= 0) {
    SD_REQUIRE(pad_override == 0 && stride == 2 && k == 3, kUnsupported, "%s: explicit padding %d", name.c_str(), pad_override);
    d.pad = 0;
    d.Ho = (Hup + 1 - k) / stride + 1;
    d.Wo = (Wup + 1 - k) / stride + 1;
  } else {
    d.Ho = (Hup + 2 * pad - k) / stride + 1;
    d.Wo = (Wup + 2 * pad - k) / stride + 1;
  }
  d.ksize = k;
  d.stride = stride;
  d.up = up;
  d.N = cout;
  d.out_mode = out_mode;
  d.ldT = ldT;
  Tensor out;
  std::string gn_in_name;
  if (ex) d.ln_colsum = ex->ln_colsum;
  if (ex) d.vt_perm = ex->vt_perm ? 1 : 0;
  if (ex) {
    d.q_scale = ex->q_scale;
    d.q_cols = ex->q_cols;
  }
  if (ex && ex->n_trans > 0) {
    out = new_tensor(x.B, d.Ho, d.Wo, ex->n_trans);
    ex->vt = arena_.alloc_n<half_t>((size_t)x.B * (cout - ex->n_trans) * ldT);
    d.out_t = ex->vt;
    d.n_trans = ex->n_trans;
  } else if (out_mode == kOutHalfT) {
    out.B = x.B; out.H = 1; out.W = ldT; out.C = cout;
    out.p = arena_.alloc_n<half_t>((size_t)x.B * cout * ldT);
  } else {
    out = new_tensor(x.B, d.Ho, d.Wo, geglu ? cout / 2 : cout);
  }
  d.out = out.p;
  if (f32_) {
    SD_REQUIRE(!x2 && !temb && !ex && out_mode == kOutHalf && !silu_out, kInternal, "%s: not a VAE conv", name.c_str());
    ConvF32Desc fd;
    fd.x = reinterpret_cast<const float*>(x.p);
    fd.w = w;
    fd.w_kind = w_f32_pending_ ? 1 : 0;
    w_f32_pending_ = false;
    fd.bias = bias;
    fd.res = reinterpret_cast<const float*>(res);
    fd.out = reinterpret_cast<float*>(out.p);
    fd.B = x.B; fd.Hi = x.H; fd.Wi = x.W; fd.Cin = x.C; fd.Ho = d.Ho; fd.Wo = d.Wo; fd.N = cout;
    fd.ksize = k; fd.stride = stride; fd.up = up; fd.pad = d.pad;
    ops.push_back([fd](hipStream_t s) { launch_conv_f32(fd, s); });
    char buf[256];
    snprintf(buf, sizeof(buf), "conv%dx%d fp32 %d->%d @%dx%d %s", k, k, x.C, cout, d.Ho, d.Wo, name.c_str());
    ops.back().label = buf;
    ops.back().flop = 2.0 * x.B * d.Ho * d.Wo * (double)cout * x.C * k * k;
    return out;
  }
  SD_REQUIRE(!ex || (conv_fast_path_ok(d) && !silu_out), kInternal, "%s: LayerNorm fold / fused q|k|v off the MFMA path",
             name.c_str());
  std::shared_ptr<GnHook> hook;
  if (out_mode == kOutHalf && !(ex && ex->n_trans > 0)) {
    hook = std::make_shared<GnHook>();
    out.gn = hook;
    hook->ops_pos = (int)ops.size();
    hook->ops_list = &ops;
  }
  auto with_hook = [hook](const ConvDesc& d0) {
    ConvDesc dd = d0;
    if (hook) {
      dd.gn_partial = hook->partial;
      dd.gn_groups = hook->groups;
      dd.n_twins = hook->n_twins;
      for (int k = 0; k < hook->n_twins; ++k) dd.twin[k] = hook->twin[k];
    }
    return dd;
  };
  if (conv_fast_path_ok(d) && !silu_out) {
    static const int ws_mode = tune_env_int("SD_WSTREAM", 1);
    const int Mrows = x.B * d.Ho * d.Wo;
    static const bool tuning = getenv("SD_TUNE") != nullptr;
    const bool ws_candidate = tuning ? ((k == 3 && Mrows <= 512) || (k == 1 && Mrows <= 128)) : conv_plan_is_wstream(d);
    if (ws_mode != 0 && !ex && wstream_shape_ok(d) && ws_candidate) {
      const int cin_t = x.C + (x2 ? x2->C : 0);
      half_t* wt = arena_.alloc_n<half_t>(wstream_tiled_halves(cout, cin_t, k));
      launch_wstream_retile(w, wt, cout, cin_t, k, stream_);
      d.w_tiled = wt;
    }
    {
      static const bool wsg_on = tune_env_int("SD_WSGEMM", 1) != 0;
      if (wsg_on && wsgemm_wanted(d)) {
        half_t* wt = arena_.alloc_n<half_t>(wsgemm_tiled_halves(cout));
        launch_wsgemm_retile(w, wt, cout, geglu, stream_);
        d.w_ws = wt;
      }
    }
    {
      static const bool bv_on = tune_env_int("SD_BVGEMM", 1) != 0;
      if (bv_on && !d.w_ws && bvgemm_wanted(d)) {
        half_t* wt = arena_.alloc_n<half_t>(bvgemm_tiled_halves(cout, x.C));
        launch_bvgemm_retile(w, wt, cout, x.C, geglu, stream_);
        d.w_bv = wt;
      }
    }
    if (hook) {
      hook->twin_capable = !ex && d.Ho * d.Wo <= 256;
      hook->desc = d;
    }
    ws_need_ = std::max(ws_need_, conv_workspace_bytes(d));
    std::shared_ptr<GnIn> gi = std::move(pending_gn_in_);
    pending_gn_in_.reset();
    if (gi) {
      gn_in_name = gi->norm_name;
      const half_t* xp = x.p;
      const int C = x.C, B = x.B, HW = x.H * x.W;
      ops.push_back([this, d, hook, with_hook, gi, xp, C, B, HW](hipStream_t s) {
        ConvDesc dd = with_hook(d);
        const int e = gi->hook->consume();
        if (e >= 1 && e <= 128) {
          dd.gnf_partial = gi->partial;
          dd.gnf_gamma = gi->gamma;
          dd.gnf_beta = gi->beta;
          dd.gnf_eps = gi->eps;
          dd.gnf_groups = gi->groups;
          dd.gnf_entries = e;
          dd.gnf_silu = gi->silu;
        } else {
          launch_groupnorm(xp, C, nullptr, 0, gi->partial, gi->gamma, gi->beta, gi->y, B, HW, gi->groups, gi->eps, gi->silu, s, e);
          dd.x0 = gi->y;
        }
        const int n = launch_conv(dd, ws_conv_, s);
        if (hook) hook->produced(n);
      });
    } else {
      ops.push_back([this, d, hook, with_hook](hipStream_t s) {
        const int n = launch_conv(with_hook(d), ws_conv_, s);
        if (hook) hook->produced(n);
      });
    }
  } else {
    const int so = silu_out ? 1 : 0;
    ops.push_back([d, so, hook, with_hook](hipStream_t s) {
      const int n = launch_conv_generic(with_hook(d), so, s);
      if (hook) hook->produced(n);
    });
  }
  SD_REQUIRE(!pending_gn_in_, kInternal, "%s: a GroupNorm was queued for a conv that cannot take it", name.c_str());
  {
    const int cin = x.C + (x2 ? x2->C : 0);
    char buf[320];
    const int kind = d.out_t ? 3 : (geglu ? 2 : (d.ln_colsum ? 1 : 0));
    snprintf(buf, sizeof(buf), "%s%s %d->%d @%dx%d M=%d K=%d %s #%d,%d,%d,%d,%d,%d,%d", k == 3 ? "conv3x3" : (geglu ? "geglu1x1" : "gemm1x1"),
             ex && ex->ln_colsum ? "+ln" : "", cin, cout, d.Ho, d.Wo, x.B * d.Ho * d.Wo, cin * k * k, name.c_str(), kind, k,
             stride, up, cin, cout, x.B * d.Ho * d.Wo);
    ops.back().label = buf;
    if (!gn_in_name.empty()) {
      std::string l = buf;
      const size_t at = l.rfind(" #");
      ops.back().label = l.substr(0, at) + " +gn(" + gn_in_name + ")" + l.substr(at);
    }
    ops.back().flop = 2.0 * x.B * d.Ho * d.Wo * (double)cout * cin * k * k;
  }
  return out;
}

Tensor UNet::group_norm(std::vector<Op>& ops, const std::string& name, const Tensor& x, const Tensor* x2, float eps,
                        bool silu, const ConvDesc* side, const std::string& side_label, double side_flop) {
  SD_REQUIRE(!side || !f32_, kInternal, "%s: side GEMM on the fp32 path", name.c_str());
  const int C = x.C + (x2 ? x2->C : 0);
  const int G = cfg_.norm_num_groups;
  SD_REQUIRE(C % G == 0, kUnsupported, "%s: %d channels not divisible by %d groups", name.c_str(), C, G);
  if (f32_) {
    SD_REQUIRE(!x2, kInternal, "%s: concat GroupNorm on the fp32 path", name.c_str());
    void* scratch = arena_.alloc(groupnorm_f32_scratch_bytes(x.B, G));
    const float* gamma = upload_vec(name + ".weight", C);
    const float* beta = upload_vec(name + ".bias", C);
    Tensor y = new_tensor(x.B, x.H, x.W, C);
    const float* xp = reinterpret_cast<const float*>(x.p);
    float* yp = reinterpret_cast<float*>(y.p);
    const int B = x.B, HW = x.H * x.W, si = silu ? 1 : 0;
    ops.push_back([=](hipStream_t s) { launch_groupnorm_f32(xp, scratch, gamma, beta, yp, B, HW, C, G, eps, si, s); });
    ops.back().label = "groupnorm fp32 C=" + std::to_string(C) + " @" + std::to_string(x.H) + "x" + std::to_string(x.W) + " " + name;
    return y;
  }
  const float* gamma = upload_vec(name + ".weight", C);
  const float* beta = upload_vec(name + ".bias", C);
  Tensor y = new_tensor(x.B, x.H, x.W, C);
  {
    static const int twin_mode = tune_env_int("SD_GN_TWIN", 0);
    static const int twin_max_hw = tune_env_int("SD_GN_TWIN_MAX_HW", 256);
    const int cpg = C / G;
    const Tensor* srcs[2] = {&x, x2};
    bool ok = twin_mode != 0 && !side && x.H * x.W <= std::min(256, twin_max_hw) && cpg % 4 == 0 && (!x2 || x.C % cpg == 0);
    for (int i = 0; i < 2 && ok; ++i) {
      const Tensor* t = srcs[i];
      if (!t) continue;
      const GnHook* hk = t->gn.get();
      ok = hk && hk->twin_capable && hk->ops_list == &ops && hk->n_twins < 2 && hk->desc.N == t->C && t->C % cpg == 0;
      if (ok) {
        GnTwin tw[2];
        int n = hk->n_twins;
        for (int k = 0; k < n; ++k) tw[k] = hk->twin[k];
        tw[n].cpg = cpg;
        tw[n].c_off = i == 0 ? 0 : x.C;
        tw[n].ld = C;
        ok = reduce_twin_ok(t->H * t->W, t->C, n + 1, tw);
      }
    }
    if (ok) {
      for (int i = 0; i < 2; ++i) {
        const Tensor* t = srcs[i];
        if (!t) continue;
        GnHook* hk = t->gn.get();
        GnTwin& tw = hk->twin[hk->n_twins++];
        tw.y = y.p;
        tw.ld = C;
        tw.c_off = i == 0 ? 0 : x.C;
        tw.cpg = cpg;
        tw.gamma = gamma;
        tw.beta = beta;
        tw.eps = eps;
        tw.silu = silu ? 1 : 0;
        ConvDesc dd = hk->desc;
        dd.n_twins = hk->n_twins;
        ws_need_ = std::max(ws_need_, conv_workspace_bytes(dd));
      }
      return y;
    }
  }
  float* partial = arena_.alloc_n<float>(groupnorm_scratch_floats(x.B, x.H * x.W, G));
  const half_t* p0 = x.p;
  const half_t* p1 = x2 ? x2->p : nullptr;
  const int C0 = x.C, C1 = x2 ? x2->C : 0, B = x.B, HW = x.H * x.W, si = silu ? 1 : 0;
  half_t* yp = y.p;
  std::shared_ptr<GnHook> hook;
  if (!x2 && x.gn && !x.gn->partial && x.gn->n_twins == 0 && groupnorm_wants_producer_stats(HW, C, G)) {
    SD_REQUIRE(x.gn->ops_list == &ops && x.gn->ops_pos >= 0 && x.gn->ops_pos < (int)ops.size(), kInternal,
               "%s: GroupNorm producer statistics need the producing op earlier in the same launch list", name.c_str());
    hook = x.gn;
    hook->partial = partial;
    hook->groups = G;
  }
  if (side) {
    const ConvDesc sd = *side;
    ops.push_back([=](hipStream_t s) {
      launch_groupnorm(p0, C0, p1, C1, partial, gamma, beta, yp, B, HW, G, eps, si, s, hook ? hook->consume() : 0, &sd);
    });
    ops.back().label = "groupnorm C=" + std::to_string(C) + " @" + std::to_string(x.H) + "x" + std::to_string(x.W) + " " + name + " || " + side_label;
    ops.back().flop = side_flop;
    return y;
  }
  ops.push_back([=](hipStream_t s) {
    launch_groupnorm(p0, C0, p1, C1, partial, gamma, beta, yp, B, HW, G, eps, si, s, hook ? hook->consume() : 0);
  });
  ops.back().label = "groupnorm C=" + std::to_string(C) + " @" + std::to_string(x.H) + "x" + std::to_string(x.W) + " " + name;
  return y;
}

Tensor UNet::layer_norm(std::vector<Op>& ops, const std::string& name, const Tensor& x) {
  const float* w = upload_vec(name + ".weight", x.C);
  const float* b = upload_vec(name + ".bias", x.C);
  Tensor y = new_tensor(x.B, x.H, x.W, x.C);
  const half_t* xp = x.p;
  half_t* yp = y.p;
  const int M = x.M(), C = x.C;
  ops.push_back([=](hipStream_t s) { launch_layernorm(xp, w, b, yp, M, C, 1e-5f, s); });
  ops.back().label = "layernorm C=" + std::to_string(C) + " M=" + std::to_string(M) + " " + name;
  return y;
}

const float* UNet::register_temb(const std::string& name, int cout) {
  SD_REQUIRE(temb_used_ + cout <= kTembCap, kInternal, "time_emb_proj outputs exceed %d", kTembCap);
  temb_layers_.push_back({name, cout});
  const float* p = temb_all_ + temb_used_;
  temb_used_ += cout;
  return p;
}

Tensor UNet::resnet(std::vector<Op>& ops, const std::string& p, const Tensor& x, const Tensor* x2, int cout,
                    bool has_temb) {
  const int cin = x.C + (x2 ? x2->C : 0);
  static const int side_mode = tune_env_int("SD_GN_SIDE", 1);
  static const int twin_mode = tune_env_int("SD_GN_TWIN", 0);
  static const int twin_max_hw = tune_env_int("SD_GN_TWIN_MAX_HW", 256);
  const bool twin_here = twin_mode != 0 && x.H * x.W <= std::min(256, twin_max_hw);
  const half_t* side_out = nullptr;
  Tensor t0;
  if (cin != cout && side_mode != 0 && !twin_here && !f32_) {
    ConvDesc sd;
    sd.x0 = x.p;
    sd.C0 = x.C;
    if (x2) {
      sd.x1 = x2->p;
// ... 1410 lines not shown
```

ml-stable-diffusion_amd/csrc/unet.h:

```cpp
#pragma once
#include <functional>

#include "../../include/sd_mi355x.h"
#include "kernels.h"
#include "weights.h"

namespace sd {

struct GnHook {
  float* partial = nullptr;
  int groups = 0;
  int entries = 0;
  bool fresh = false;
  void produced(int n) {
    entries = n;
    fresh = true;
  }
  int consume() {
    const int n = fresh ? entries : 0;
    fresh = false;
    return n;
  }
  int ops_pos = -1;
  const void* ops_list = nullptr;
  bool twin_capable = false;
  ConvDesc desc;
  GnTwin twin[2];
  int n_twins = 0;
};

struct Tensor {
  half_t* p = nullptr;
  int B = 0, H = 0, W = 0, C = 0;
  std::shared_ptr<GnHook> gn;
  int M() const { return B * H * W; }
  size_t numel() const { return (size_t)B * H * W * C; }
};

struct PreQkv {
  Tensor qk;
  half_t* vt = nullptr;
  bool vt_perm = false;
  bool q_pre = false;
};

struct Op {
  std::function<void(hipStream_t)> fn;
  std::string label;
  double flop = 0;
  Op() = default;
  template <class F, class = std::enable_if_t<!std::is_same<std::decay_t<F>, Op>::value>>
  Op(F&& f) : fn(std::forward<F>(f)) {}
  void operator()(hipStream_t s) const { fn(s); }
};

struct OpTime {
  std::string label;
  double flop;
  float ms;
};

class UNet {
 public:
  UNet(const sd_unet_config& cfg, const WeightStore& ws, int device);
  ~UNet();

  void forward(const sd_unet_io& io);
  float time_forward(int warmup, int iters);
  void drop_graphs() { invalidate_graphs(); }
  std::vector<OpTime> profile(int iters);
  void denoise_loop(const sd_unet_io& io, float* latents, int n_images, int n_steps, const float* timesteps,
                    const float* coef, const float* sample_scale, int history, float guidance, float* history_io,
                    float* ms_per_step);
  void attach_controlnets(const std::vector<UNet*>& cns);
  void set_controlnet_cond(const void* cond, int flags);
  void set_attention(int impl);
  void vae_decode(const void* z, int z_is_f32, float* image, int flags);
  void vae_encode(const void* x, int x_is_f32, float* moments, int flags);
  int num_residuals() const { return (int)res_shapes_.size(); }
  size_t device_bytes() const { return arena_.bytes(); }
  const sd_unet_config& config() const { return cfg_; }

 private:
  void build_unet();
  void build_vae_decoder();
  void build_vae_encoder();
  void run_vae_graph();
  Tensor new_tensor(int B, int H, int W, int C);
  half_t* upload_conv_weight(const std::string& name, int cout, int cin, int k, bool geglu);
  float* upload_vec(const std::string& name, int n, bool geglu = false);
  Tensor conv(std::vector<Op>& ops, const std::string& name, const Tensor& x, const Tensor* x2, int cout, int k,
              int stride, int up, bool bias, const float* temb, const half_t* res, int out_mode = kOutHalf,
              int ldT = 0, bool silu_out = false, int pad = -1);
  struct ConvExtra {
    const float* ln_colsum = nullptr;
    int n_trans = 0;
    half_t* vt = nullptr;
    bool vt_perm = false;
    float q_scale = 1.f;
    int q_cols = 0;
  };
  Tensor conv_w(std::vector<Op>& ops, const std::string& name, const half_t* w, const float* bias, const Tensor& x,
                const Tensor* x2, int cout, int k, int stride, int up, const float* temb, const half_t* res,
                int out_mode, int ldT, bool silu_out, ConvExtra* ex = nullptr, int pad = -1);
  struct LnFold {
    half_t* w;
    float* colsum;
    float* bias;
  };
  LnFold fold_layernorm(const std::string& ln, const std::vector<std::string>& names, int cin, int cout_each,
                        bool geglu);
  bool can_fold_ln(const Tensor& x, int cout, bool geglu) const;
  Tensor conv_stacked(std::vector<Op>& ops, const std::vector<std::string>& names, const Tensor& x, int cout_each);
  Tensor group_norm(std::vector<Op>& ops, const std::string& name, const Tensor& x, const Tensor* x2, float eps,
                    bool silu, const ConvDesc* side = nullptr, const std::string& side_label = std::string(), double side_flop = 0);
  Tensor layer_norm(std::vector<Op>& ops, const std::string& name, const Tensor& x);
  Tensor resnet(std::vector<Op>& ops, const std::string& p, const Tensor& x, const Tensor* x2, int cout,
                bool has_temb = true);
  Tensor transformer(std::vector<Op>& ops, const std::string& p, const Tensor& x, int heads, int depth);
  Tensor transformer_block(std::vector<Op>& ops, const std::string& b, const Tensor& h, int heads, const std::string* proj_out = nullptr,
                           const Tensor* tres = nullptr, bool* tail_done = nullptr, const PreQkv* pre = nullptr);
  Tensor vae_attention(std::vector<Op>& ops, const std::string& p, const Tensor& h);
  Tensor attention(std::vector<Op>& ops, const Tensor& q, const half_t* k, const half_t* vt, int heads, int Sq,
                   int Sk, int ldk, int ldv, int ldq, bool vt_perm = false, bool q_prescaled = false);
  float* sk_part_ = nullptr;
  size_t sk_part_bytes_ = 0;
  unsigned* sk_cnt_ = nullptr;
  int sk_cnt_n_ = 0;
  void down_and_mid(std::vector<Op>& ops, Tensor& h, std::vector<Tensor>& skips);
  const float* register_temb(const std::string& name, int cout);
  void finalize_temb();
  void upload_inputs(const sd_unet_io& io, bool loop_mode);
  void run_ops(const std::vector<Op>& ops);
  void run_ops_on(const std::vector<Op>& ops, hipStream_t s);
  void run_as_controlnet(hipStream_t s, const half_t* x_nhwc, const float* tbuf);
  void set_context_from(const half_t* ehs_dev, hipStream_t s);
  void run_attached();
  void invalidate_graphs();
  hipGraphExec_t capture(const std::function<void()>& body);
  void run_forward_ops();
  void run_time_and_main();
  void run_main(bool with_time);
  void ensure_graph();

  sd_unet_config cfg_;
  const WeightStore* ws_ = nullptr;
  int device_ = 0;
  bool f32_ = false;
  struct GnIn {
    std::shared_ptr<GnHook> hook;
    float* partial = nullptr;
    const float* gamma = nullptr;
    const float* beta = nullptr;
    half_t* y = nullptr;
    float eps = 1e-5f;
    int groups = 32, silu = 1;
    std::string norm_name;
  };
  std::shared_ptr<GnIn> pending_gn_in_;
  bool gn_loader_conv(std::vector<Op>& ops, const std::string& norm, const std::string& cv, const Tensor& x, int cout, const float* temb,
                      const half_t* res, Tensor* out);
  bool gn_loader_ok(const std::vector<Op>& ops, const Tensor& x, int cout) const;
  bool w_f32_pending_ = false;
  hipStream_t stream_ = nullptr;
  hipStream_t side_ = nullptr;
  hipEvent_t ev_fork_ = nullptr, ev_join_ = nullptr;
  int temb_join_pos_ = -1;
  hipStream_t cn_stream_ = nullptr;
  hipEvent_t ev_cn_fork_ = nullptr, ev_cn_join_ = nullptr;
  int cn_join_pos_ = -1;
  bool cn_join_pending_ = false;
  Arena arena_;

  half_t* in_sample_ = nullptr;
  half_t* in_timestep_ = nullptr;
  half_t* in_ehs_ = nullptr;
  half_t* in_time_ids_ = nullptr;
  half_t* in_text_embeds_ = nullptr;
  half_t* in_cond_ = nullptr;
  std::vector<half_t*> in_res_nchw_;
  std::vector<Tensor> res_nhwc_;
  std::vector<std::vector<int>> res_shapes_;
  float* noise_pred_ = nullptr;
  float* in_z_ = nullptr;
  half_t* z_half_ = nullptr;
  float* image_ = nullptr;
  void* in_x_ = nullptr;
  int vae_in_f32_ = 0;
  size_t image_elems_ = 0;
  std::vector<float*> res_out_;
  std::vector<Tensor> cn_out_;

  Tensor x_in_;
  float* tbuf_ = nullptr;
  float* emb_ = nullptr;
  float* temb_all_ = nullptr;
  float* temb_tab_ = nullptr;
  int temb_tab_cap_ = 0;
  float *tt_tab_ = nullptr, *tsin_tab_ = nullptr, *e1_tab_ = nullptr, *emb_tab_ = nullptr;
  struct TimePath {
    const float* freq = nullptr;
    const half_t *w1 = nullptr, *w2 = nullptr;
    const float *b1 = nullptr, *b2 = nullptr;
    int c0 = 0, tdim = 0;
    bool ok = false;
  } tpath_;
  int temb_used_ = 0;
  std::vector<std::pair<std::string, int>> temb_layers_;
  half_t* temb_w_all_ = nullptr;
  float* temb_b_all_ = nullptr;
  Tensor ctx_;
  ConvWorkspace ws_conv_;
  size_t ws_need_ = 0;

  std::vector<Op> in_ops_, time_ops_, ctx_ops_, cond_ops_, main_ops_;
  std::vector<Op> out_ops_;
  std::vector<UNet*> attached_;
  std::vector<uint16_t> last_ehs_, last_cond_;
  bool have_ctx_ = false, have_cond_ = false, have_inputs_ = false;
  hipGraphExec_t graph_ = nullptr, loop_graph_ = nullptr;
  int loop_graph_key_ = -1;

  float* latents_ = nullptr;
  float* eps_hist_ = nullptr;
  float* tab_timesteps_ = nullptr;
  float* tab_coef_ = nullptr;
  float* tab_scale_ = nullptr;
  int* step_ = nullptr;
  int tab_cap_ = 0;
  float* noise_tab_ = nullptr;
  size_t noise_cap_ = 0;
};

}

struct sd_unet {
  std::unique_ptr<sd::UNet> impl;
};
```

ml-stable-diffusion_amd/python_hip_stable_diffusion/_lib.py:

```python
import ctypes as C
import os

import numpy as np

_HERE = os.path.dirname(os.path.abspath(__file__))
LIB_PATH = os.environ.get("SD_MI355X_LIB", os.path.join(os.path.dirname(_HERE), "lib", "libsdmi355.so"))

SD_MAX_LEVELS = 6
SD_FLAG_DEVICE_PTRS = 1
ATTENTION_IMPLEMENTATIONS = {"ORIGINAL": 0, "SPLIT_EINSUM": 1, "SPLIT_EINSUM_V2": 2}


class LibraryNotBuilt(ImportError):
    pass


class UNetConfig(C.Structure):
    _fields_ = [
        ("batch", C.c_int32), ("in_channels", C.c_int32), ("out_channels", C.c_int32),
        ("height", C.c_int32), ("width", C.c_int32), ("n_levels", C.c_int32),
        ("block_out_channels", C.c_int32 * SD_MAX_LEVELS),
        ("down_cross_attn", C.c_int32 * SD_MAX_LEVELS),
        ("up_cross_attn", C.c_int32 * SD_MAX_LEVELS),
        ("layers_per_block", C.c_int32),
        ("attention_head_dim", C.c_int32 * SD_MAX_LEVELS),
        ("transformer_layers_per_block", C.c_int32 * SD_MAX_LEVELS),
        ("cross_attention_dim", C.c_int32), ("context_len", C.c_int32),
        ("norm_num_groups", C.c_int32), ("norm_eps", C.c_float),
        ("flip_sin_to_cos", C.c_int32), ("freq_shift", C.c_float),
        ("addition_time_embed_dim", C.c_int32), ("projection_class_embeddings_input_dim", C.c_int32),
        ("num_time_ids", C.c_int32), ("support_controlnet", C.c_int32), ("is_controlnet", C.c_int32),
        ("is_vae_decoder", C.c_int32),
        ("attention_impl", C.c_int32), ("use_graph", C.c_int32), ("compute_fp32", C.c_int32),
    ]


class UNetIO(C.Structure):
    _fields_ = [
        ("sample", C.c_void_p), ("timestep", C.c_void_p), ("encoder_hidden_states", C.c_void_p),
        ("time_ids", C.c_void_p), ("text_embeds", C.c_void_p), ("controlnet_cond", C.c_void_p),
        ("additional_residuals", C.POINTER(C.c_void_p)), ("num_additional_residuals", C.c_int32),
        ("noise_pred", C.c_void_p), ("residual_outputs", C.POINTER(C.c_void_p)), ("flags", C.c_int32),
        ("step_noise", C.c_void_p),
    ]


_lib = None

_P, _I, _F = C.c_void_p, C.c_int, C.c_float
_FP = C.POINTER(C.c_float)
SYMBOLS = [
    ("sd_last_error", C.c_char_p, []),
    ("sd_version", C.c_char_p, []),
    ("sd_device_count", _I, []),
    ("sd_weights_create", _I, [C.POINTER(_P)]),
    ("sd_weights_add", _I, [_P, C.c_char_p, _P, _I, C.POINTER(C.c_int64), _I]),
    ("sd_weights_load_safetensors", _I, [_P, C.c_char_p, C.c_char_p]),
    ("sd_weights_count", _I, [_P]),
    ("sd_weights_destroy", None, [_P]),
    ("sd_unet_create", _I, [C.POINTER(UNetConfig), _P, _I, C.POINTER(_P)]),
    ("sd_unet_destroy", None, [_P]),
    ("sd_unet_set_attention", _I, [_P, _I]),
    ("sd_unet_num_residuals", _I, [_P]),
    ("sd_unet_device_bytes", C.c_size_t, [_P]),
    ("sd_unet_forward", _I, [_P, C.POINTER(UNetIO)]),
    ("sd_unet_time_forward", _I, [_P, _I, _I, _FP]),
    ("sd_unet_denoise_loop", _I, [_P, C.POINTER(UNetIO), _FP, _I, _I, _FP, _FP, _FP, _I, _F, _FP, _FP]),
    ("sd_tune_set_candidate", _I, [_I, _I, _I]),
    ("sd_tune_set_plan_table", _I, [C.c_char_p, C.c_void_p, C.POINTER(C.c_int)]),
    ("sd_unet_profile", _I, [_P, _I, _I, _FP, C.POINTER(C.c_double), C.c_char_p, _I, C.POINTER(_I)]),
    ("sd_unet_attach_controlnets", _I, [_P, C.POINTER(_P), _I]),
    ("sd_controlnet_set_cond", _I, [_P, _P, _I]),
    ("sd_vae_decoder_create", _I, [C.POINTER(UNetConfig), _P, _I, C.POINTER(_P)]),
    ("sd_vae_decode", _I, [_P, _P, _I, _FP, _I]),
    ("sd_vae_encoder_create", _I, [C.POINTER(UNetConfig), _P, _I, C.POINTER(_P)]),
    ("sd_vae_encode", _I, [_P, _P, _I, _FP, _I]),
    ("sd_text_encoder_create", _I, [_P, _P, _I, C.POINTER(_P)]),
    ("sd_text_encoder_destroy", None, [_P]),
    ("sd_text_encoder_device_bytes", C.c_size_t, [_P]),
    ("sd_text_encoder_encode", _I, [_P, C.POINTER(C.c_int32), _I, _FP, _FP, _FP]),
    ("sd_op_attention", _I, [_I, _P, _P, _P, _P, _I, _I, _I, _I, _I, _I, _I, _FP]),
    ("sd_op_layernorm", _I, [_P, _FP, _FP, _P, _I, _I, _I, _F, _I, _FP]),
    ("sd_op_groupnorm", _I, [_P, _FP, _FP, _P, _I, _I, _I, _I, _I, _F, _I, _I, _FP]),
    ("sd_op_groupnorm_shortcut", _I, [_P, _P, _FP, _FP, _P, _FP, _P, _P, _I, _I, _I, _I, _I, _I, _I, _F, _I, _I, _I, _FP]),
    ("sd_op_conv2d", _I, [_P, _P, _FP, _P, _P, _I, _I, _I, _I, _I, _I, _I, _I, _I, _I, _I, _I, _FP]),
    ("sd_op_conv2d_groupnorm", _I, [_P, _P, _FP, _P, _FP, _FP, _P, _P, _I, _I, _I, _I, _I, _I, _I, _F, _I, _I, _I, C.POINTER(_I), _I, _FP]),
    ("sd_op_conv2d_groupnorm_proj", _I, [_P, _P, _FP, _P, _FP, _FP, _P, _FP, _P, _P, _I, _I, _I, _I, _I, _I, _I, _I, _F, _I, _I, C.POINTER(_I), _I, _FP]),
    ("sd_op_conv2d_groupnorm_conv3x3", _I, [_P, _P, _FP, _P, _FP, _FP, _P, _FP, _P, _P, _P, _I, _I, _I, _I, _I, _I, _I, _I, _F, _I, _I, _I, _I,
                                            C.POINTER(_I), _I, _FP]),
    ("sd_op_cross_attention_fused", _I, [_P, _FP, _FP, _P, _P, _P, _P, _I, _I, _I, _I, _F, _I, _I, _FP]),
    ("sd_op_ffn_out_proj", _I, [_P, _P, _FP, _P, _P, _FP, _P, _P, _FP, _I, _I, _I, _I, _I, _I, _FP]),
    ("sd_op_cross_attention_block", _I, [_P, _FP, _FP, _P, _P, _P, _P, _FP, _P, _P, _FP, _P, _I, _I, _I, _I, _F, _I, _I, _FP]),
    ("sd_op_geglu", _I, [_P, _P, _FP, _P, _I, _I, _I, _I, _FP]),
    ("sd_op_geglu_ln", _I, [_P, _FP, _FP, _P, _FP, _P, _I, _I, _I, C.c_float, _I, _I, _FP]),
    ("sd_op_qkv_ln", _I, [_P, _FP, _FP, _P, _P, _P, _I, _I, _I, C.c_float, C.c_float, _I, _I, _I, _FP]),
    ("sd_op_gn_proj_qkv", _I, [_P, _P, _FP, _FP, _P, _FP, _FP, _FP, _P, _P, _P, _P, _I, _I, _I, _I, _I, C.c_float, C.c_float, C.c_float, _I, _I,
                               C.POINTER(C.c_int), _I, _FP]),
    ("sd_op_timestep_embedding", _I, [_FP, _FP, _I, _I, _I, _F]),
    ("sd_numpy_randn", _I, [C.c_uint32, C.POINTER(C.c_double), C.c_size_t]),
    ("sd_torch_randn", _I, [C.c_uint32, C.POINTER(C.c_double), C.c_size_t]),
    ("sd_philox_randn", _I, [C.c_uint64, C.c_uint32, C.POINTER(C.c_double), C.c_size_t]),
    ("sd_calibrate", _I, [_I, _FP]),
    ("sd_selftest_mfma", _I, []),
]


def lib():
    global _lib
    if _lib is not None:
        return _lib
    if not os.path.exists(LIB_PATH):
        raise LibraryNotBuilt(
            f"{LIB_PATH} is missing - build it with `python -c 'import __graft_entry__ as g; g.build()'` "
            f"or `make -C ml-stable-diffusion_amd/csrc`. There is no CPU fallback.")
    if not os.environ.get("SD_MI355X_NO_TORCH"):
        try:
            import torch
        except Exception:
            pass
    handle = C.CDLL(LIB_PATH, mode=C.RTLD_GLOBAL)
    for name, restype, argtypes in SYMBOLS:
        fn = getattr(handle, name)
        fn.restype = restype
        fn.argtypes = argtypes
    _lib = handle
    return handle


_EXC = {-1: ValueError, -2: FileNotFoundError, -3: RuntimeError, -4: NotImplementedError, -5: RuntimeError}


def check(status):
    if status != 0:
        msg = lib().sd_last_error().decode("utf-8", "replace")
        raise _EXC.get(status, RuntimeError)(msg)


def ptr(a):
    return None if a is None else a.ctypes.data_as(C.c_void_p)


def fptr(a):
    return None if a is None else a.ctypes.data_as(_FP)


def f16(a):
    return np.ascontiguousarray(a, dtype=np.float16)


def f32(a):
    return np.ascontiguousarray(a, dtype=np.float32)


def attention(impl, q, k, v, heads, dim_head, variant=0, iters=1):
    if impl not in ATTENTION_IMPLEMENTATIONS:
        raise ValueError(f"unknown attention implementation {impl!r}")
    q, k, v = f16(q), f16(k), f16(v)
    B, Cq, _, Sq = q.shape
    Sk = k.shape[3]
    if Cq != heads * dim_head or k.shape[1] != Cq or v.shape != k.shape:
        raise ValueError("attention: inconsistent q/k/v shapes")
    out = np.empty_like(q)
    ms = C.c_float(0)
    check(lib().sd_op_attention(ATTENTION_IMPLEMENTATIONS[impl], ptr(q), ptr(k), ptr(v), ptr(out), B, heads,
                                dim_head, Sq, Sk, variant, iters, C.byref(ms)))
    return out, ms.value


def layernorm(x, weight, bias, eps=1e-5, iters=1):
    x, weight, bias = f16(x), f32(weight), f32(bias)
    B, Cn, _, S = x.shape
    out = np.empty_like(x)
    ms = C.c_float(0)
    check(lib().sd_op_layernorm(ptr(x), fptr(weight), fptr(bias), ptr(out), B, Cn, S, eps, iters, C.byref(ms)))
    return out, ms.value


def groupnorm(x, weight, bias, groups=32, eps=1e-5, silu=False, iters=1):
    x, weight, bias = f16(x), f32(weight), f32(bias)
    B, Cn, H, W = x.shape
    out = np.empty_like(x)
    ms = C.c_float(0)
    check(lib().sd_op_groupnorm(ptr(x), fptr(weight), fptr(bias), ptr(out), B, Cn, H, W, groups, eps, int(silu),
                                iters, C.byref(ms)))
    return out, ms.value


def conv2d(x, w, bias=None, res=None, stride=1, upsample=False, tile=0, splitk=0, force_generic=False, iters=1):
    x, w = f16(x), f16(w)
    B, Cin, H, W = x.shape
    Cout, Cin2, k, k2 = w.shape
    if Cin2 != Cin or k != k2:
        raise ValueError("conv2d: weight shape does not match input")
    up = 2 if upsample else 1
    pad = k // 2
    Ho = (H * up + 2 * pad - k) // stride + 1
    Wo = (W * up + 2 * pad - k) // stride + 1
    bias = None if bias is None else f32(bias)
    res = None if res is None else f16(res)
    out = np.empty((B, Cout, Ho, Wo), np.float16)
    ms = C.c_float(0)
    check(lib().sd_op_conv2d(ptr(x), ptr(w), fptr(bias), ptr(res), ptr(out), B, Cin, H, W, Cout, k, stride,
                             int(upsample), tile, splitk, int(force_generic), iters, C.byref(ms)))
    return out, ms.value


def groupnorm_shortcut(x0, x1, gn_weight, gn_bias, w, bias=None, groups=32, eps=1e-5, silu=True, side=True, iters=1):
    x0, w = f16(x0), f16(w)
    x1 = None if x1 is None else f16(x1)
    B, C0, H, W = x0.shape
    C1 = 0 if x1 is None else x1.shape[1]
    N = w.shape[0]
    w = np.ascontiguousarray(w.reshape(N, -1))
    if w.shape[1] != C0 + C1 or (x1 is not None and x1.shape != (B, C1, H, W)):
        raise ValueError("groupnorm_shortcut: inconsistent shapes")
    gn_weight, gn_bias = f32(gn_weight), f32(gn_bias)
    bias = None if bias is None else f32(bias)
    out_gn = np.empty((B, C0 + C1, H, W), np.float16)
    out_sc = np.empty((B, N, H, W), np.float16)
    ms = C.c_float(0)
    check(lib().sd_op_groupnorm_shortcut(ptr(x0), ptr(x1), fptr(gn_weight), fptr(gn_bias), ptr(w), fptr(bias), ptr(out_gn), ptr(out_sc),
                                         B, C0, C1, H, W, N, groups, eps, int(silu), int(side), iters, C.byref(ms)))
    return out_gn, out_sc, ms.value


def conv2d_groupnorm(x, w, gn_weight, gn_bias, bias=None, res=None, groups=32, eps=1e-5, silu=False, tile=0,
                     producer_stats=True, iters=1):
    x, w = f16(x), f16(w)
    B, Cin, H, W = x.shape
    Cout, Cin2, k, k2 = w.shape
    if Cin2 != Cin or k != k2:
        raise ValueError("conv2d_groupnorm: weight shape does not match input")
    bias = None if bias is None else f32(bias)
    res = None if res is None else f16(res)
    gn_weight, gn_bias = f32(gn_weight), f32(gn_bias)
    conv_out = np.empty((B, Cout, H, W), np.float16)
    out = np.empty((B, Cout, H, W), np.float16)
    ms, entries = C.c_float(0), C.c_int(0)
    check(lib().sd_op_conv2d_groupnorm(ptr(x), ptr(w), fptr(bias), ptr(res), fptr(gn_weight), fptr(gn_bias), ptr(conv_out),
                                       ptr(out), B, Cin, H, W, Cout, k, groups, eps, int(silu), tile, int(producer_stats),
                                       C.byref(entries), iters, C.byref(ms)))
    return conv_out, out, entries.value, ms.value


def conv2d_groupnorm_proj(x, w, gn_weight, gn_bias, proj_w, proj_bias=None, bias=None, res=None, groups=32, eps=1e-6, fold=True,
                          tile=0, iters=1):
    x, w, proj_w = f16(x), f16(w), f16(proj_w)
    B, Cin, H, W = x.shape
    Cout, k = w.shape[0], w.shape[2]
    Np = proj_w.shape[0]
    if w.shape[1] != Cin or proj_w.reshape(Np, -1).shape[1] != Cout:
        raise ValueError("conv2d_groupnorm_proj: inconsistent shapes")
    proj_w = np.ascontiguousarray(proj_w.reshape(Np, Cout))
    gn_weight, gn_bias = f32(gn_weight), f32(gn_bias)
    bias = None if bias is None else f32(bias)
    proj_bias = None if proj_bias is None else f32(proj_bias)
    res = None if res is None else f16(res)
    conv_out = np.empty((B, Cout, H, W), np.float16)
    out = np.empty((B, Np, H, W), np.float16)
    ms, entries = C.c_float(0), C.c_int(0)
    check(lib().sd_op_conv2d_groupnorm_proj(ptr(x), ptr(w), fptr(bias), ptr(res), fptr(gn_weight), fptr(gn_bias), ptr(proj_w),
                                            fptr(proj_bias), ptr(conv_out), ptr(out), B, Cin, H, W, Cout, k, Np, groups, eps,
                                            int(fold), tile, C.byref(entries), iters, C.byref(ms)))
    return conv_out, out, entries.value, ms.value


def conv2d_groupnorm_conv3x3(x, w, gn_weight, gn_bias, w2, bias2=None, res2=None, bias=None, res=None, groups=32, eps=1e-5, silu=True,
                             fold=True, tile=0, staging2=0, iters=1):
    x, w, w2 = f16(x), f16(w), f16(w2)
    B, Cin, H, W = x.shape
    Cout, k = w.shape[0], w.shape[2]
    N2 = w2.shape[0]
    if w.shape[1] != Cin or w2.shape[1:] != (Cout, 3, 3):
        raise ValueError("conv2d_groupnorm_conv3x3: inconsistent shapes")
    gn_weight, gn_bias = f32(gn_weight), f32(gn_bias)
    bias = None if bias is None else f32(bias)
    bias2 = None if bias2 is None else f32(bias2)
    res = None if res is None else f16(res)
    res2 = None if res2 is None else f16(res2)
    conv_out = np.empty((B, Cout, H, W), np.float16)
    out = np.empty((B, N2, H, W), np.float16)
    ms, entries = C.c_float(0), C.c_int(0)
    check(lib().sd_op_conv2d_groupnorm_conv3x3(ptr(x), ptr(w), fptr(bias), ptr(res), fptr(gn_weight), fptr(gn_bias), ptr(w2), fptr(bias2),
                                               ptr(res2), ptr(conv_out), ptr(out), B, Cin, H, W, Cout, k, N2, groups, eps, int(silu),
                                               int(fold), tile, staging2, C.byref(entries), iters, C.byref(ms)))
    return conv_out, out, entries.value, ms.value


def cross_attention_block(x, ln_weight, ln_bias, wq, k, v, wo, bo, heads, eps=1e-5, fused=True, iters=1, a1=None, wo1=None, bo1=None):
    x, k, v, wq, wo = f16(x), f16(k), f16(v), f16(wq), f16(wo)
    B, Cn, _, Sq = x.shape
    Sk = k.shape[3]
    if Cn != heads * 64 or k.shape[1] != Cn or v.shape != k.shape or wq.shape != (Cn, Cn) or wo.shape != (Cn, Cn):
        raise ValueError("cross_attention_block: inconsistent shapes")
    ln_weight, ln_bias, bo = f32(ln_weight), f32(ln_bias), f32(bo)
    if a1 is not None:
        a1, wo1, bo1 = f16(a1), f16(wo1), f32(bo1)
        if a1.shape != x.shape or wo1.shape != (Cn, Cn):
            raise ValueError("cross_attention_block: inconsistent shapes of a1 / wo1")
    out = np.empty_like(x)
    ms = C.c_float(0)
    check(lib().sd_op_cross_attention_block(ptr(x), fptr(ln_weight), fptr(ln_bias), ptr(wq), ptr(k), ptr(v), ptr(wo), fptr(bo), ptr(a1), ptr(wo1),
                                            fptr(bo1), ptr(out), B, heads, Sq, Sk, eps, int(fused), iters, C.byref(ms)))
    return out, ms.value


def ffn_out_proj(g, w1, b1, res1, w2, b2, res2, groups=0, fused=True, iters=1):
    g, res1, res2, w1, w2 = f16(g), f16(res1), f16(res2), f16(w1), f16(w2)
    B, Cn, _, S = res1.shape
    if g.shape != (B, 4 * Cn, 1, S) or res2.shape != res1.shape or w1.shape != (Cn, 4 * Cn) or w2.shape != (Cn, Cn):
        raise ValueError("ffn_out_proj: inconsistent shapes")
    b1, b2 = f32(b1), f32(b2)
    out = np.empty_like(res1)
    sums = np.empty((B, groups, 2), np.float32) if groups > 0 else None
    ms = C.c_float(0)
    check(lib().sd_op_ffn_out_proj(ptr(g), ptr(w1), fptr(b1), ptr(res1), ptr(w2), fptr(b2), ptr(res2), ptr(out), fptr(sums), B, Cn, S, groups,
                                   int(fused), iters, C.byref(ms)))
    return out, sums, ms.value


def cross_attention_fused(x, ln_weight, ln_bias, wq, k, v, heads, eps=1e-5, nst=0, iters=1):
    x, k, v, wq = f16(x), f16(k), f16(v), f16(wq)
    B, Cn, _, Sq = x.shape
    Sk = k.shape[3]
    if Cn != heads * 64 or k.shape[1] != Cn or v.shape != k.shape or wq.shape != (Cn, Cn):
        raise ValueError("cross_attention_fused: inconsistent shapes")
    ln_weight, ln_bias = f32(ln_weight), f32(ln_bias)
    out = np.empty_like(x)
    ms = C.c_float(0)
    check(lib().sd_op_cross_attention_fused(ptr(x), fptr(ln_weight), fptr(ln_bias), ptr(wq), ptr(k), ptr(v), ptr(out), B, heads,
                                            Sq, Sk, eps, nst, iters, C.byref(ms)))
    return out, ms.value


def geglu(x, w, bias=None, iters=1):
    x, w = f16(x), f16(w)
    M, Cn = x.shape
    N2 = w.shape[0]
    bias = None if bias is None else f32(bias)
    out = np.empty((M, N2 // 2), np.float16)
    ms = C.c_float(0)
    check(lib().sd_op_geglu(ptr(x), ptr(w), fptr(bias), ptr(out), M, Cn, N2, iters, C.byref(ms)))
    return out, ms.value


def geglu_ln(x, w, bias=None, ln_weight=None, ln_bias=None, eps=1e-5, kernel=0, iters=1):
    x, w = f16(x), f16(w)
    M, Cn = x.shape
    N2 = w.shape[0]
    bias = None if bias is None else f32(bias)
    ln_weight = None if ln_weight is None else f32(ln_weight)
    ln_bias = None if ln_bias is None else f32(ln_bias)
    out = np.empty((M, N2 // 2), np.float16)
    ms = C.c_float(0)
    check(lib().sd_op_geglu_ln(ptr(x), fptr(ln_weight), fptr(ln_bias), ptr(w), fptr(bias), ptr(out), M, Cn, N2, eps, kernel, iters,
                               C.byref(ms)))
    return out, ms.value


# ... 59 lines not shown
```

Before: 240.8 it/s.

## Add 3x3 conv kernel with pre-tiled register-streamed weights and halo LDS

Adds a new 3x3 convolution kernel (plan tile 14). It streams weights, retiled once into an MFMA-fragment order, straight into registers through a ring of buffer loads issued LEAD steps ahead. Input halos go to LDS by direct DMA. The UNet builder retiles eligible conv weights at build time and frees the original staged copy once only the tiled copy is needed. The aim is to cut LDS traffic for weights and hide their load latency, in exchange for more register pressure, extra build-time copies, and new planner paths.

```diff
diff --git a/include/sd_mi355x.h b/include/sd_mi355x.h
--- a/include/sd_mi355x.h
+++ b/include/sd_mi355x.h
@@ -141,6 +141,10 @@
 int sd_op_conv2d(const void* x, const void* w, const float* bias, const void* res, void* out, int B, int Cin, int H,
                  int W, int Cout, int ksize, int stride, int upsample, int tile, int splitk, int force_generic,
                  int iters, float* ms);
+int sd_op_conv3x3_ex(const void* x0, const void* x1, const void* w, const float* bias, const float* temb, const void* res, void* out,
+                     float* gn_sums, int B, int C0, int C1, int H, int W, int Cout, int upsample, int groups, int tile, int splitk,
+                     int* entries, int iters, float* ms);
+int sd_conv_bv_tiled_map(int N, int Ctot, int* row, int* k, long long count);
 int sd_op_conv2d_groupnorm(const void* x, const void* w, const float* bias, const void* res, const float* gn_weight,
                            const float* gn_bias, void* conv_out, void* out, int B, int Cin, int H, int W, int Cout, int ksize,
                            int groups, float eps, int silu, int tile, int producer_stats, int* entries, int iters, float* ms);
diff --git a/ml-stable-diffusion_amd/csrc/capi.cpp b/ml-stable-diffusion_amd/csrc/capi.cpp
--- a/ml-stable-diffusion_amd/csrc/capi.cpp
+++ b/ml-stable-diffusion_amd/csrc/capi.cpp
@@ -492,11 +492,21 @@
       d.tile = 12;
       d.staging = tile - 140;
     }
+    if (tile >= 150 && tile <= 151) {
+      d.tile = 14;
+      d.staging = tile - 150;
+    }
     d.splitk = splitk;
     d.debug = force_generic >= 2 ? force_generic - 1 : 0;
     if (d.debug & 4) d.prof = sc.dev<long long>(8);
     const bool fast = force_generic != 1 && conv_fast_path_ok(d);
     ConvWorkspace ws;
+    if (fast && d.tile == 14) {
+      SD_REQUIRE(conv_bv_shape_ok(d), kInvalidArgument, "conv2d: shape not eligible for plan tile 14 (conv3x3_bv_kernel)");
+      half_t* wtd = sc.dev<half_t>(conv_bv_tiled_halves(Cout, Cin));
+      launch_conv_bv_retile(d.w, wtd, Cout, Cin, sc.stream);
+      d.w_cbv = wtd;
+    }
     if (fast && d.tile == 9) {
       SD_REQUIRE(wstream_shape_ok(d), kInvalidArgument, "conv2d: shape not eligible for plan tile 9 (wstream.hip)");
       half_t* wtd = sc.dev<half_t>(wstream_tiled_halves(Cout, Cin, ksize));
@@ -531,6 +541,99 @@
     std::vector<half_t> ot(on);
     SD_HIP(hipMemcpy(ot.data(), dout, on * 2, hipMemcpyDeviceToHost));
     nhwc_to_nchw(ot.data(), reinterpret_cast<half_t*>(out), B, Cout, Ho, Wo);
+  });
+}
+
+int sd_op_conv3x3_ex(const void* x0, const void* x1, const void* w, const float* bias, const float* temb, const void* res, void* out,
+                     float* gn_sums, int B, int C0, int C1, int H, int W, int Cout, int upsample, int groups, int tile, int splitk,
+                     int* entries, int iters, float* ms) {
+  return guarded([&] {
+    SD_REQUIRE(x0 && w && out && (C1 == 0 || x1) && (upsample == 0 || upsample == 1), kInvalidArgument, "conv3x3_ex: NULL or inconsistent argument");
+    SD_REQUIRE(!gn_sums || (groups >= 1 && Cout % groups == 0), kInvalidArgument, "conv3x3_ex: groups %d", groups);
+    Scratch sc;
+    const int up = upsample ? 2 : 1, Ho = H * up, Wo = W * up, Cin = C0 + C1;
+    std::vector<half_t> xt0 = nchw_to_nhwc(reinterpret_cast<const half_t*>(x0), B, C0, H, W);
+    const half_t* wh = reinterpret_cast<const half_t*>(w);
+    std::vector<half_t> wt((size_t)Cout * Cin * 9);
+    for (int o = 0; o < Cout; ++o)
+      for (int c = 0; c < Cin; ++c)
+        for (int t = 0; t < 9; ++t) wt[((size_t)o * 9 + t) * Cin + c] = wh[((size_t)o * Cin + c) * 9 + t];
+    ConvDesc d;
+    d.x0 = sc.dev<half_t>(xt0.size(), xt0.data());
+    d.C0 = C0;
+    if (C1 > 0) {
+      std::vector<half_t> xt1 = nchw_to_nhwc(reinterpret_cast<const half_t*>(x1), B, C1, H, W);
+      d.x1 = sc.dev<half_t>(xt1.size(), xt1.data());
+      d.C1 = C1;
+    }
+    d.w = sc.dev<half_t>(wt.size(), wt.data());
+    d.bias = bias ? sc.dev<float>(Cout, bias) : nullptr;
+    if (temb) {
+      d.temb = sc.dev<float>((size_t)B * Cout, temb);
+      d.temb_stride = Cout;
+    }
+    if (res) {
+      std::vector<half_t> rt = nchw_to_nhwc(reinterpret_cast<const half_t*>(res), B, Cout, Ho, Wo);
+      d.res = sc.dev<half_t>(rt.size(), rt.data());
+    }
+    const size_t on = (size_t)B * Ho * Wo * Cout;
+    half_t* dout = sc.dev<half_t>(on);
+    d.out = dout;
+    d.B = B; d.Hi = H; d.Wi = W; d.Ho = Ho; d.Wo = Wo;
+    d.ksize = 3; d.stride = 1; d.up = up; d.N = Cout;
+    d.tile = tile % 10;
+    d.staging = tile / 10;
+    if (tile >= 150 && tile <= 151) {
+      d.tile = 14;
+      d.staging = tile - 150;
+    }
+    d.splitk = splitk;
+    SD_REQUIRE(conv_fast_path_ok(d), kInvalidArgument, "conv3x3_ex: C0=%d C1=%d N=%d not MFMA-tileable", C0, C1, Cout);
+    if (d.tile == 14) {
+      SD_REQUIRE(conv_bv_shape_ok(d), kInvalidArgument, "conv3x3_ex: shape not eligible for plan tile 14 (conv3x3_bv_kernel)");
+      half_t* wtd = sc.dev<half_t>(conv_bv_tiled_halves(Cout, Cin));
+      launch_conv_bv_retile(d.w, wtd, Cout, Cin, sc.stream);
+      d.w_cbv = wtd;
+    }
+    const size_t pn = gn_sums ? groupnorm_scratch_floats(B, Ho * Wo, groups) : 0;
+    float* partial = nullptr;
+    if (gn_sums) {
+      std::vector<float> poison(pn, 1.0e30f);
+      partial = sc.dev<float>(pn, poison.data());
+      d.gn_partial = partial;
+      d.gn_groups = groups;
+    }
+    ConvWorkspace ws;
+    ws.partial_bytes = conv_workspace_bytes(d);
+    if (ws.partial_bytes) ws.partial = reinterpret_cast<float*>(sc.dev<char>(ws.partial_bytes));
+    int n_entries = 0;
+    sc.timed(iters, ms, [&] { n_entries = launch_conv(d, ws, sc.stream); });
+    if (entries) *entries = n_entries;
+    if (gn_sums) {
+      std::vector<float> hp(pn);
+      SD_HIP(hipMemcpy(hp.data(), partial, pn * sizeof(float), hipMemcpyDeviceToHost));
+      for (int bg = 0; bg < B * groups; ++bg) {
+        float sum = 0.f, sq = 0.f;
+        for (int e = 0; e < n_entries; ++e) {
+          sum += hp[((size_t)bg * kGnMaxSlabs + e) * 2];
+          sq += hp[((size_t)bg * kGnMaxSlabs + e) * 2 + 1];
+        }
+        gn_sums[2 * bg] = sum;
+        gn_sums[2 * bg + 1] = sq;
+      }
+    }
+    std::vector<half_t> ot(on);
+    SD_HIP(hipMemcpy(ot.data(), dout, on * 2, hipMemcpyDeviceToHost));
+    nhwc_to_nchw(ot.data(), reinterpret_cast<half_t*>(out), B, Cout, Ho, Wo);
+  });
+}
+
+int sd_conv_bv_tiled_map(int N, int Ctot, int* row, int* k, long long count) {
+  return guarded([&] {
+    SD_REQUIRE(row && k && N >= 1 && Ctot >= 64 && Ctot % 64 == 0, kInvalidArgument, "conv_bv_tiled_map: N=%d Ctot=%d", N, Ctot);
+    const long long pieces = (long long)((N + 63) / 64) * (Ctot / 64) * 9 * 512;
+    SD_REQUIRE(count == pieces, kInvalidArgument, "conv_bv_tiled_map: %lld pieces, not %lld", pieces, count);
+    for (long long i = 0; i < count; ++i) conv_bv_piece_source((size_t)i, N, Ctot, &row[i], &k[i]);
   });
 }
 
diff --git a/ml-stable-diffusion_amd/csrc/igemm.hip b/ml-stable-diffusion_amd/csrc/igemm.hip
--- a/ml-stable-diffusion_amd/csrc/igemm.hip
+++ b/ml-stable-diffusion_amd/csrc/igemm.hip
@@ -1223,6 +1223,297 @@
     }
   }
   if (gn) tile_gn_stats<BN>(a, reinterpret_cast<float*>(smem), fs, fq, n_blk, b, ty * a.tiles_x + tx);
+}
+
+__device__ __forceinline__ void halo_ks_epilogue(const IgemmArgs& a, floatx16 (&acc)[2][2], char* smem, float* sconst, float const_b, float const_t,
+                                                 int wave, int lane, int y0, int x0, int n_blk, int b, int split, int tile_in_sample) {
+  constexpr int BN = 64, BM = 128;
+  const int tid = threadIdx.x, wm = wave >> 1, wk = wave & 1, frow = lane & 31, hi = lane >> 5;
+  const int H = a.Ho, W = a.Wo;
+  {
+    floatx4* red = reinterpret_cast<floatx4*>(smem);
+#pragma unroll
+    for (int j = 0; j < 2; ++j)
+#pragma unroll
+      for (int q = 0; q < 4; ++q) {
+        floatx4 v;
+#pragma unroll
+        for (int e = 0; e < 4; ++e) v[e] = wk ? acc[0][j][4 * q + e] : acc[1][j][4 * q + e];
+        red[((wave * 2 + j) * 4 + q) * 64 + lane] = v;
+      }
+    if (tid < BN) sconst[tid] = const_b + const_t;
+    __syncthreads();
+  }
+  floatx16 fin[2];
+  {
+    const floatx4* red = reinterpret_cast<const floatx4*>(smem);
+#pragma unroll
+    for (int j = 0; j < 2; ++j)
+#pragma unroll
+      for (int q = 0; q < 4; ++q) {
+        const floatx4 v = red[(((wave ^ 1) * 2 + j) * 4 + q) * 64 + lane];
+#pragma unroll
+        for (int e = 0; e < 4; ++e) fin[j][4 * q + e] = (wk ? acc[1][j][4 * q + e] : acc[0][j][4 * q + e]) + v[e];
+      }
+  }
+  const int ml = (wm * 2 + wk) * 32 + frow;
+  if (a.slab) {
+    const int y = y0 + (ml >> 4), x = x0 + (ml & 15);
+    if (y < H && x < W) {
+      const int m = (b * H + y) * W + x;
+      float* prow = a.partial + ((size_t)split * a.M + m) * a.N;
+#pragma unroll
+      for (int j = 0; j < 2; ++j)
+#pragma unroll
+        for (int q = 0; q < 4; ++q) {
+          const int n = n_blk + j * 32 + 8 * q + 4 * hi;
+          if (n < a.N) {
+            floatx4 v = {fin[j][4 * q], fin[j][4 * q + 1], fin[j][4 * q + 2], fin[j][4 * q + 3]};
+            out_store(reinterpret_cast<floatx4*>(prow + n), v);
+          }
+        }
+    }
+    return;
+  }
+  constexpr int OROW = BN + 8;
+  half_t* ot = reinterpret_cast<half_t*>(smem + 32 * 1024);
+#pragma unroll
+  for (int j = 0; j < 2; ++j)
+#pragma unroll
+    for (int q = 0; q < 4; ++q) {
+      const int nl = j * 32 + 8 * q + 4 * hi;
+      const floatx4 bb = *reinterpret_cast<const floatx4*>(sconst + nl);
+      half4 o = {(half_t)(fin[j][4 * q] + bb[0]), (half_t)(fin[j][4 * q + 1] + bb[1]), (half_t)(fin[j][4 * q + 2] + bb[2]),
+                 (half_t)(fin[j][4 * q + 3] + bb[3])};
+      *reinterpret_cast<half4*>(ot + ml * OROW + nl) = o;
+    }
+  __syncthreads();
+  constexpr int WC = BN / 8;
+  const bool gn = a.gn_partial != nullptr;
+  float fs[8] = {0.f, 0.f, 0.f, 0.f, 0.f, 0.f, 0.f, 0.f}, fq[8] = {0.f, 0.f, 0.f, 0.f, 0.f, 0.f, 0.f, 0.f};
+  for (int idx = tid; idx < BM * WC; idx += 256) {
+    const int r = idx / WC, c = idx - r * WC;
+    const int y = y0 + (r >> 4), x = x0 + (r & 15);
+    const int n = n_blk + c * 8;
+    if (y < H && x < W && n < a.N) {
+      const size_t m = (size_t)(b * H + y) * W + x;
+      half8 v = *reinterpret_cast<const half8*>(ot + r * OROW + c * 8);
+      half_t* dst = a.out + m * a.N + n;
+      if (n + 8 <= a.N) {
+        if (a.res) {
+          const half8 rr = *reinterpret_cast<const half8*>(a.res + m * a.N + n);
+#pragma unroll
+          for (int e = 0; e < 8; ++e) v[e] = (half_t)((float)v[e] + (float)rr[e]);
+        }
+        out_store(reinterpret_cast<half8*>(dst), v);
+        if (gn) {
+#pragma unroll
+          for (int e = 0; e < 8; ++e) {
+            const float f = (float)v[e];
+            fs[e] += f;
+            fq[e] = fmaf(f, f, fq[e]);
+          }
+        }
+      } else {
+        for (int e = 0; e < a.N - n; ++e) dst[e] = a.res ? (half_t)((float)v[e] + (float)a.res[m * a.N + n + e]) : v[e];
+      }
+    }
+  }
+  if (gn) tile_gn_stats<BN>(a, reinterpret_cast<float*>(smem), fs, fq, n_blk, b, tile_in_sample);
+}
+
+constexpr size_t conv_bv_lds_bytes() { return 32 * 1024 + 128 * (64 + 8) * 2 + 64 * sizeof(float); }
+static_assert(2 * HALO_LDS_ROWS * BK * sizeof(half_t) <= 32 * 1024 + 128 * (64 + 8) * 2, "the halo buffers fit under the epilogue constants");
+
+__global__ __launch_bounds__(256) void conv_bv_retile_kernel(const half_t* __restrict__ w, half_t* __restrict__ wt, int N, int Ctot, size_t total16) {
+  const size_t i = (size_t)blockIdx.x * 256 + threadIdx.x;
+  if (i >= total16) return;
+  int n, k;
+  conv_bv_piece_source(i, N, Ctot, &n, &k);
+  reinterpret_cast<half8*>(wt)[i] = *reinterpret_cast<const half8*>(w + (size_t)n * 9 * Ctot + k);
+}
+
+template <int LEAD, int OCC>
+__global__ __launch_bounds__(256, OCC) void conv3x3_bv_kernel(IgemmArgs a) {
+  constexpr int BN = 64, BM = 128, ROWB = BK * 2, R = 6, XBUF = HALO_LDS_ROWS * ROWB;
+  static_assert(LEAD >= 1 && LEAD < R, "a ring stage is requested LEAD steps before the step that consumes it");
+  extern __shared__ __attribute__((aligned(16))) char smem[];
+  char* const Xh = smem;
+  float* const sconst = reinterpret_cast<float*>(smem + 32 * 1024 + BM * (BN + 8) * 2);
+
+  const int tid = threadIdx.x, lane = tid & 63;
+  const int wave = __builtin_amdgcn_readfirstlane(tid >> 6);
+  const int wm = wave >> 1, wk = wave & 1;
+  const int H = a.Ho, W = a.Wo;
+  const int ush = a.up >> 1;
+
+  const int n_tiles = (a.N + BN - 1) / BN;
+  const int m_tiles = a.B * a.tiles_y * a.tiles_x;
+  const int nwg = m_tiles * n_tiles;
+  int bid = blockIdx.x;
+  {
+    int q = nwg >> 3, r = nwg & 7, xcd = bid & 7, idx = bid >> 3;
+    int base = (xcd < r) ? xcd * (q + 1) : r * (q + 1) + (xcd - r) * q;
+    bid = base + idx;
+  }
+  const int bn_idx = a.n_fast ? bid % n_tiles : bid / m_tiles, mt = a.n_fast ? bid / n_tiles : bid % m_tiles;
+  const int b = mt / (a.tiles_y * a.tiles_x);
+  const int trem = mt - b * (a.tiles_y * a.tiles_x);
+  const int ty = trem / a.tiles_x, tx = trem - ty * a.tiles_x;
+  const int y0 = ty * 8, x0 = tx * 16;
+  const int n_blk = bn_idx * BN;
+
+  const int nch = a.Ctot / BK;
+  const int split = blockIdx.y;
+  const int ch_begin = split * a.nk_per_split;
+  int ch_end = ch_begin + a.nk_per_split;
+  if (ch_end > nch) ch_end = nch;
+
+  constexpr unsigned kOob = 0x80000000u, kOutside = 0xffffffffu;
+  const size_t xpix = (size_t)a.B * a.Hi * a.Wi;
+  unsigned hpk[HALO_PPW];
+  auto piece_of = [&](int j) { return (wave + 4 * j < HALO_PIECES) ? wave + 4 * j : HALO_PIECES - 1; };
+#pragma unroll
+  for (int j = 0; j < HALO_PPW; ++j) {
+    const int p = piece_of(j);
+    const int hr = 8 * p + (lane >> 3);
+    const int hy = hr / HALO_W, hx = hr - hy * HALO_W;
+    const int iy = y0 - 1 + hy, ix = x0 - 1 + hx;
+    const bool ok = (hr < HALO_ROWS) && iy >= 0 && iy < H && ix >= 0 && ix < W;
+    const unsigned pix = (unsigned)((b * a.Hi + (iy >> ush)) * a.Wi + (ix >> ush));
+    hpk[j] = ok ? pix * 8u + (unsigned)((lane & 7) ^ ((hx >> 1) & 7)) : kOutside;
+  }
+  struct HaloSrc {
+    __amdgpu_buffer_rsrc_t rs;
+    int soff;
+    unsigned cbytes;
+  };
+  auto halo_src = [&](int ch) {
+    const bool second = ch * BK >= a.C0;
+    HaloSrc h;
+    h.cbytes = (unsigned)(second ? a.C1 : a.C0) * 2u;
+    h.rs = __builtin_amdgcn_make_buffer_rsrc(const_cast<half_t*>(second ? a.x1 : a.x0), 0, ch < ch_end ? (int)(xpix * h.cbytes) : 0, 0x00020000);
+    h.soff = (second ? ch * BK - a.C0 : ch * BK) * 2;
+    return h;
+  };
+  auto issue_x_piece = [&](int j, const HaloSrc& h, int xstage) {
+    const unsigned off = hpk[j] == kOutside ? kOob : (hpk[j] >> 3) * h.cbytes + (hpk[j] & 7u) * 16u;
+    dma16_to_lds(h.rs, Xh + xstage * XBUF + piece_of(j) * 1024, off, h.soff);
+  };
+
+  const __amdgpu_buffer_rsrc_t rs_w =
+      __builtin_amdgcn_make_buffer_rsrc(const_cast<half_t*>(a.w), 0, (int)(((size_t)n_tiles * nch * 9 + 5) * 8192), 0x00020000);
+  const unsigned wlane = (unsigned)lane * 16u;
+  [[maybe_unused]] int w_soff = ((bn_idx * nch + ch_begin) * 9) * 8192 + wk * 4096;
+  half8 wr[R][4];
+  auto issue_w = [&](half8 (&dst)[4]) {
+#if defined(__HIP_DEVICE_COMPILE__)
+#pragma unroll
+    for (int f = 0; f < 4; ++f) dst[f] = __builtin_bit_cast(half8, __builtin_amdgcn_raw_buffer_load_b128(rs_w, wlane, w_soff + f * 1024, 0));
+#endif
+    w_soff += 8192;
+  };
+
+  floatx16 acc[2][2];
+#pragma unroll
+  for (int i = 0; i < 2; ++i)
+#pragma unroll
+    for (int j = 0; j < 2; ++j)
+#pragma unroll
+      for (int r = 0; r < 16; ++r) acc[i][j][r] = 0.f;
+
+  const int frow = lane & 31, hi = lane >> 5;
+  int xaddr[3][2];
+#pragma unroll
+  for (int i = 0; i < 2; ++i) {
+    const int ml = (wm * 2 + i) * 32 + frow;
+    const int hrb = ((ml >> 4) * HALO_W + (ml & 15)) * ROWB;
+#pragma unroll
+    for (int kx = 0; kx < 3; ++kx) xaddr[kx][i] = hrb + (((4 * wk + hi) ^ ((((frow & 15) + kx) >> 1) & 7)) * 16);
+  }
+
+  float const_b = 0.f, const_t = 0.f;
+  if (!a.slab && tid < BN && n_blk + tid < a.N) {
+    if (a.bias) const_b = a.bias[n_blk + tid];
+    if (a.temb) const_t = a.temb[(size_t)b * a.temb_stride + n_blk + tid];
+  }
+
+  auto read_step = [&](half8 (&xf)[2][2], int xstage, int tap) {
+    const int ky = tap / 3, kx = tap - ky * 3;
+    const int immb = xstage * XBUF + (ky * HALO_W + kx) * ROWB;
+#pragma unroll
+    for (int s = 0; s < 2; ++s)
+#pragma unroll
+      for (int i = 0; i < 2; ++i) xf[s][i] = *reinterpret_cast<const half8*>(Xh + ((xaddr[kx][i] ^ (s * 32)) + immb));
+  };
+  auto mfma_step = [&](half8 (&xf)[2][2], half8 (&wf)[4]) {
+#pragma unroll
+    for (int s = 0; s < 2; ++s)
+#pragma unroll
+      for (int i = 0; i < 2; ++i)
+#pragma unroll
+        for (int j = 0; j < 2; ++j) acc[i][j] = __builtin_amdgcn_mfma_f32_32x32x16_f16(wf[s * 2 + j], xf[s][i], acc[i][j], 0, 0, 0);
+  };
+
+  half8 xfA[2][2], xfB[2][2];
+  if (ch_begin < ch_end) {
+    const HaloSrc h0 = halo_src(ch_begin);
+#pragma unroll
+    for (int j = 0; j < HALO_PPW; ++j) issue_x_piece(j, h0, 0);
+    asm volatile("" ::: "memory");
+#pragma unroll
+    for (int p = 0; p < LEAD; ++p) issue_w(wr[p]);
+    asm volatile("" ::: "memory");
+    wait_vmcnt_barrier<LEAD * 4>();
+    read_step(xfA, 0, 0);
+  }
+  auto chunk = [&](auto par, int ch) {
+    constexpr int PAR = decltype(par)::value;
+    const HaloSrc hn = halo_src(ch + 1);
+#pragma unroll
+    for (int tap = 0; tap < 9; ++tap) {
+      auto body = [&](half8 (&cx)[2][2], half8 (&nx)[2][2]) {
+        half8 (&cw)[4] = wr[(tap + 3 * PAR) % R];
+        half8 (&nw)[4] = wr[(tap + 3 * PAR + LEAD) % R];
+        if (tap == 8) {
+          asm volatile("s_waitcnt lgkmcnt(0)" ::: "memory");
+          wait_vmcnt_barrier<8>();
+        } else {
+          asm volatile("" ::: "memory");
+        }
+        read_step(nx, tap == 8 ? PAR ^ 1 : PAR, tap == 8 ? 0 : tap + 1);
+        issue_w(nw);
+        if (tap < HALO_PPW) issue_x_piece(tap < HALO_PPW ? tap : 0, hn, PAR ^ 1);
+        mfma_step(cx, cw);
+#pragma unroll
+        for (int g = 0; g < 4; ++g) {
+          __builtin_amdgcn_sched_group_barrier(0x008, 1, 0);
+          __builtin_amdgcn_sched_group_barrier(0x100, 1, 0);
+          __builtin_amdgcn_sched_group_barrier(0x020, 1, 0);
+        }
+        __builtin_amdgcn_sched_group_barrier(0x008, 1, 0);
+        __builtin_amdgcn_sched_group_barrier(0x020, 1, 0);
+        __builtin_amdgcn_sched_group_barrier(0x008, 3, 0);
+      };
+      if (((tap + PAR) & 1) == 0) body(xfA, xfB);
+      else body(xfB, xfA);
+      __builtin_amdgcn_sched_barrier(0);
+    }
+  };
+  {
+    using P0 = std::integral_constant<int, 0>;
+    using P1 = std::integral_constant<int, 1>;
+    int ch = ch_begin;
+    for (; ch + 1 < ch_end; ch += 2) {
+      chunk(P0{}, ch);
+      chunk(P1{}, ch + 1);
+    }
+    if (ch < ch_end) chunk(P0{}, ch);
+  }
+  asm volatile("s_waitcnt vmcnt(0) lgkmcnt(0)" ::: "memory");
+  __syncthreads();
+
+  halo_ks_epilogue(a, acc, smem, sconst, const_b, const_t, wave, lane, y0, x0, n_blk, b, split, ty * a.tiles_x + tx);
 }
 
 #undef HALO_SRC
@@ -2017,6 +2308,7 @@
 void tile_dims(int tile, int& bm, int& bn) {
   switch (tile) {
     case 7: bm = 128; bn = 64; break;
+    case 14: bm = 128; bn = 64; break;
     case 1: bm = 128; bn = 128; break;
     case 2: bm = 128; bn = 64; break;
     case 3: bm = 64; bn = 64; break;
@@ -2075,10 +2367,12 @@
   p.staging = d.staging;
   const bool geglu = d.out_mode == kOutGeglu;
   const bool can_split = d.out_mode == kOutHalf && !d.ln_colsum && !d.out_t;
-  auto is_halo = [](int c) { return c == 7; };
+  auto is_halo = [](int c) { return c == 7 || c == 14; };
+  static const int cbv_mode = tune_env_int("SD_CONVBV", 1);
   static const int ws_mode = tune_env_int("SD_WSTREAM", 1);
   auto tile_ok = [&](int c) {
     if (c == 9) return ws_mode != 0 && d.w_tiled != nullptr && can_split && wstream_shape_ok(d);
+    if (c == 14) return cbv_mode != 0 && d.w_cbv != nullptr && conv_bv_shape_ok(d);
     if (!((c >= 1 && c <= 4) || c == 7)) return false;
     if (is_halo(c)) return halo_ks_ok(d) && !d.ln_colsum && !d.out_t && !geglu;
     int bm, bn;
@@ -2102,6 +2396,7 @@
     return s;
   };
   const bool pinned = p.tile != 0 || p.splitk != 0 || p.staging != 0;
+  bool from_runtime_table = false;
   if (!pinned && g_tune.tile != 0 && tile_ok(g_tune.tile)) {
     p.tile = g_tune.tile;
     p.staging = g_tune.staging;
@@ -2115,6 +2410,7 @@
     const TunedConv* hit = nullptr;
     for (const TunedConv& t : runtime_table())
       if (!hit && match(t)) hit = &t;
+    from_runtime_table = hit != nullptr;
     for (int i = 0; i < kNumTuned && !hit; ++i)
       if (match(kTuned[i])) hit = &kTuned[i];
     if (hit) {
@@ -2132,6 +2428,10 @@
     p.tile = 7;
     if (p.staging == 0) p.staging = 3;
   }
+  if (p.tile == 7 && !pinned && g_tune.tile == 0 && !from_runtime_table && tile_ok(14) && conv_bv_wanted(d)) {
+    p.tile = 14;
+    p.staging = 0;
+  }
   if (p.tile == 0) {
     p.tile = 3;
     for (int c : {1, 2, 4, 3}) {
@@ -2143,7 +2443,7 @@
   if (p.splitk == 0) {
     p.splitk = 1;
     const int ms = max_split(p.tile);
-    const long want = p.tile == 7 ? 192 : 384;
+    const long want = is_halo(p.tile) ? 192 : 384;
     while (blocks_of(p.tile) * p.splitk < want && p.splitk < ms) p.splitk *= 2;
   }
   if (!can_split) p.splitk = 1;
@@ -2200,6 +2500,24 @@
   launch_halo_ks_d<2>(a, s);
 }
 
+template <int LEAD, int OCC>
+void launch_conv_bv_d(const IgemmArgs& a, hipStream_t s) {
+  auto k = conv3x3_bv_kernel<LEAD, OCC>;
+  static DynLdsOnce once;
+  once.set(k, conv_bv_lds_bytes());
+  dim3 grid(a.B * a.tiles_x * a.tiles_y * cdiv(a.N, 64), a.splitk);
+  hipLaunchKernelGGL(k, grid, dim3(256), conv_bv_lds_bytes(), s, a);
+}
+
+void launch_conv_bv(IgemmArgs a, int splitk, int staging, hipStream_t s) {
+  const int nch = a.Ctot / BK;
+  a.nk_total = nch;
+  a.nk_per_split = cdiv(nch, splitk);
+  a.splitk = cdiv(nch, a.nk_per_split);
+  if (staging == 1) launch_conv_bv_d<2, 2>(a, s);
+  else launch_conv_bv_d<4, 2>(a, s);
+}
+
 template <int BM, int BN, int WGM, int WGN, bool TRANS, bool GLDS, int NST, bool LNF = false, int KG = 1>
 void launch_variant(const IgemmArgs& a, hipStream_t s) {
   const size_t lds = (size_t)KG * NST * (BM + BN) * (GLDS ? BK : LDS_ROW) * sizeof(half_t) + 2 * BN * sizeof(float);
@@ -2361,6 +2679,32 @@
   if (!d.w_tiled) d.w_tiled = d.w;
   const IgemmArgs a = make_args(d);
   return choose_plan(d, a).tile == 9;
+}
+
+bool conv_bv_shape_ok(const ConvDesc& d) {
+  if (!conv_fast_path_ok(d) || !halo_ks_ok(d) || d.ln_colsum || d.out_t || d.out_mode != kOutHalf || d.debug) return false;
+  const int ctot = d.C0 + (d.x1 ? d.C1 : 0);
+  return conv_bv_tiled_halves(d.N, ctot) * sizeof(half_t) < ((size_t)1 << 31);
+}
+
+size_t conv_bv_tiled_halves(int N, int Ctot) { return ((size_t)cdiv(N, 64) * (Ctot / BK) * 9 + 5) * 4096; }
+
+void launch_conv_bv_retile(const half_t* w, half_t* wt, int N, int Ctot, hipStream_t s) {
+  const size_t total16 = (size_t)cdiv(N, 64) * (Ctot / BK) * 9 * 512;
+  hipLaunchKernelGGL(conv_bv_retile_kernel, dim3((unsigned)((total16 + 255) / 256)), dim3(256), 0, s, w, wt, N, Ctot, total16);
+  SD_HIP(hipGetLastError());
+}
+
+bool conv_bv_wanted(const ConvDesc& d) {
+  return conv_bv_shape_ok(d) && !d.gnf_partial && d.Ho * d.Wo >= 256;
+}
+
+bool conv_plan_is_bv(const ConvDesc& d0) {
+  if (!conv_bv_shape_ok(d0)) return false;
+  ConvDesc d = d0;
+  if (!d.w_cbv) d.w_cbv = d.w;
+  const IgemmArgs a = make_args(d);
+  return choose_plan(d, a).tile == 14;
 }
 
 size_t conv_workspace_bytes(const ConvDesc& d) {
@@ -2453,7 +2797,7 @@
 void choose_tile_order(IgemmArgs& a, int tile) {
   int bm, bn;
   tile_dims(tile, bm, bn);
-  const bool halo_tile = tile == 7;
+  const bool halo_tile = tile == 7 || tile == 14;
   const double nbn = (double)cdiv(a.N, bn);
   const double nbm = halo_tile ? (double)a.B * a.tiles_x * a.tiles_y : (double)cdiv(a.M, bm);
   const double a_bytes = 2.0 * a.B * a.Hi * a.Wi * a.Ctot, w_bytes = 2.0 * a.N * a.K;
@@ -2523,7 +2867,8 @@
   }
   IgemmArgs a = make_args(d);
   Plan p = choose_plan(d, a);
-  bool halo = p.tile == 7;
+  bool halo = p.tile == 7 || p.tile == 14;
+  SD_REQUIRE(d.w || (p.tile == 14 && !(d.gnf_partial && d.ksize == 3)), kInternal, "launch_conv: plan tile %d without its weights", p.tile);
   const bool twins = d.n_twins > 0;
   SD_REQUIRE(!twins || (d.out_mode == kOutHalf && !d.ln_colsum && !d.out_t && !d.debug && reduce_twin_ok(a.HoWo, a.N, d.n_twins, d.twin)),
              kInvalidArgument, "GroupNorm twins need a plain fp16 output and whole (sample, group) slices (HoWo=%d N=%d)", a.HoWo, a.N);
@@ -2542,7 +2887,7 @@
     if (p.staging != 6 && p.staging != 7 && p.staging != 8) p.staging = 6;
     p.splitk = 1;
   }
-  halo = p.tile == 7;
+  halo = p.tile == 7 || p.tile == 14;
   if (p.tile == 9) {
     const int nw = p.staging == 4 ? 4 : 8;
     const int S = wstream_splits(d, nw);
@@ -2588,7 +2933,12 @@
   int gn_entries = 0;
   if (halo) {
     gn_entries = setup_gn_stats(d, a, 0);
-    launch_halo_ks(a, a.splitk, st, s);
+    if (p.tile == 14) {
+      a.w = d.w_cbv;
+      launch_conv_bv(a, a.splitk, st, s);
+    } else {
+      launch_halo_ks(a, a.splitk, st, s);
+    }
   } else if (d.debug && d.debug < 64) {
     const bool ok = p.tile == 1 ? launch_debug_mode<128, 128>(a, d.debug, s) : launch_debug_mode<64, 64>(a, d.debug, s);
     SD_REQUIRE(ok && !trans, kInvalidArgument, "no ablation kernel for debug mode %d", d.debug);
diff --git a/ml-stable-diffusion_amd/csrc/kernels.h b/ml-stable-diffusion_amd/csrc/kernels.h
--- a/ml-stable-diffusion_amd/csrc/kernels.h
+++ b/ml-stable-diffusion_amd/csrc/kernels.h
@@ -59,6 +59,7 @@
   const half_t* w_tiled = nullptr;
   const half_t* w_ws = nullptr;
   const half_t* w_bv = nullptr;
+  const half_t* w_cbv = nullptr;
   GnTwin twin[2];
   int n_twins = 0;
 };
@@ -98,6 +99,21 @@
 void launch_bvgemm_retile(const half_t* w, half_t* wt, int N, int K, bool geglu, hipStream_t s);
 void launch_bvgemm(const ConvDesc& d, int variant, hipStream_t s);
 bool bvgemm_wanted(const ConvDesc& d);
+
+bool conv_bv_shape_ok(const ConvDesc& d);
+bool conv_bv_wanted(const ConvDesc& d);
+bool conv_plan_is_bv(const ConvDesc& d);
+size_t conv_bv_tiled_halves(int N, int Ctot);
+void launch_conv_bv_retile(const half_t* w, half_t* wt, int N, int Ctot, hipStream_t s);
+__host__ __device__ inline void conv_bv_piece_source(size_t i, int N, int Ctot, int* n, int* k) {
+  const int l = (int)(i & 63), j = (int)(i >> 6) & 1, s = (int)(i >> 7) & 1, kh = (int)(i >> 8) & 1;
+  const size_t step = i >> 9;
+  const int nch = Ctot / 64;
+  const int tap = (int)(step % 9), ch = (int)((step / 9) % nch), nt = (int)(step / ((size_t)9 * nch));
+  const int row = nt * 64 + 32 * j + (l & 31);
+  *n = row < N ? row : N - 1;
+  *k = tap * Ctot + ch * 64 + 32 * kh + 16 * s + 8 * (l >> 5);
+}
 
 bool smgemm_shape_ok(const ConvDesc& d, int variant);
 bool smgemm_wanted(const ConvDesc& d);
diff --git a/ml-stable-diffusion_amd/csrc/unet.cpp b/ml-stable-diffusion_amd/csrc/unet.cpp
--- a/ml-stable-diffusion_amd/csrc/unet.cpp
+++ b/ml-stable-diffusion_amd/csrc/unet.cpp
@@ -82,7 +82,7 @@
   return t;
 }
 
-half_t* UNet::upload_conv_weight(const std::string& name, int cout, int cin, int k, bool geglu) {
+half_t* UNet::upload_conv_weight(const std::string& name, int cout, int cin, int k, bool geglu, bool staged) {
   const HostTensor& t = ws_->get(name + ".weight");
   const size_t expect = (size_t)cout * cin * k * k;
   SD_REQUIRE(t.numel() == expect, kInvalidArgument, "%s.weight has %zu elements, expected %zu (%d,%d,%d,%d)",
@@ -101,7 +101,9 @@
       for (int t2 = 0; t2 < kk; ++t2)
         host[((size_t)dst_o * kk + t2) * cin + c] = (half_t)t.data[((size_t)o * cin + c) * kk + t2];
   }
-  half_t* d = arena_.alloc_n<half_t>(expect);
+  half_t* d = nullptr;
+  if (staged) SD_HIP(hipMalloc(reinterpret_cast<void**>(&d), expect * sizeof(half_t)));
+  else d = arena_.alloc_n<half_t>(expect);
   SD_HIP(hipMemcpy(d, host.data(), expect * sizeof(half_t), hipMemcpyHostToDevice));
   return d;
 }
@@ -144,7 +146,10 @@
     return conv_w(ops, name, reinterpret_cast<const half_t*>(d), b, x, x2, cout, k, stride, up, temb, res, out_mode, ldT, silu_out,
                   nullptr, pad);
   }
-  const half_t* w = upload_conv_weight(name, cout, cin, k, geglu);
+  static const bool tuning = getenv("SD_TUNE") != nullptr;
+  const bool staged = k == 3 && stride == 1 && !geglu && !tuning;
+  const half_t* w = upload_conv_weight(name, cout, cin, k, geglu, staged);
+  w_staged_pending_ = staged;
   return conv_w(ops, name, w, b, x, x2, cout, k, stride, up, temb, res, out_mode, ldT, silu_out, nullptr, pad);
 }
 
@@ -229,6 +234,21 @@
     d.C1 = x2->C;
   }
   d.w = w;
+  const bool w_staged = w_staged_pending_;
+  w_staged_pending_ = false;
+  auto settle_staged_w = [&](bool only_tiled) {
+    if (!w_staged) return;
+    const size_t n = (size_t)cout * (x.C + (x2 ? x2->C : 0)) * k * k;
+    if (only_tiled) {
+      d.w = nullptr;
+    } else {
+      half_t* keep = arena_.alloc_n<half_t>(n);
+      SD_HIP(hipMemcpyAsync(keep, w, n * sizeof(half_t), hipMemcpyDeviceToDevice, stream_));
+      d.w = keep;
+    }
+    SD_HIP(hipStreamSynchronize(stream_));
+    SD_HIP(hipFree(const_cast<half_t*>(w)));
+  };
   d.bias = bias;
   d.temb = temb;
   d.temb_stride = kTembCap;
@@ -337,6 +357,16 @@
         d.w_bv = wt;
       }
     }
+    {
+      static const bool cbv_on = tune_env_int("SD_CONVBV", 1) != 0;
+      if (cbv_on && !ex && (tuning ? conv_bv_shape_ok(d) : conv_plan_is_bv(d))) {
+        const int cin_t = x.C + (x2 ? x2->C : 0);
+        half_t* wt = arena_.alloc_n<half_t>(conv_bv_tiled_halves(cout, cin_t));
+        launch_conv_bv_retile(w, wt, cout, cin_t, stream_);
+        d.w_cbv = wt;
+      }
+    }
+    settle_staged_w(d.w_cbv != nullptr && !tuning);
     if (hook) {
       hook->twin_capable = !ex && d.Ho * d.Wo <= 256;
       hook->desc = d;
@@ -373,6 +403,7 @@
       });
     }
   } else {
+    settle_staged_w(false);
     const int so = silu_out ? 1 : 0;
     ops.push_back([d, so, hook, with_hook](hipStream_t s) {
       const int n = launch_conv_generic(with_hook(d), so, s);
diff --git a/ml-stable-diffusion_amd/csrc/unet.h b/ml-stable-diffusion_amd/csrc/unet.h
--- a/ml-stable-diffusion_amd/csrc/unet.h
+++ b/ml-stable-diffusion_amd/csrc/unet.h
@@ -87,7 +87,7 @@
   void build_vae_encoder();
   void run_vae_graph();
   Tensor new_tensor(int B, int H, int W, int C);
-  half_t* upload_conv_weight(const std::string& name, int cout, int cin, int k, bool geglu);
+  half_t* upload_conv_weight(const std::string& name, int cout, int cin, int k, bool geglu, bool staged = false);
   float* upload_vec(const std::string& name, int n, bool geglu = false);
   Tensor conv(std::vector<Op>& ops, const std::string& name, const Tensor& x, const Tensor* x2, int cout, int k,
               int stride, int up, bool bias, const float* temb, const half_t* res, int out_mode = kOutHalf,
@@ -161,6 +161,7 @@
   bool gn_loader_conv(std::vector<Op>& ops, const std::string& norm, const std::string& cv, const Tensor& x, int cout, const float* temb,
                       const half_t* res, Tensor* out);
   bool gn_loader_ok(const std::vector<Op>& ops, const Tensor& x, int cout) const;
+  bool w_staged_pending_ = false;
   bool w_f32_pending_ = false;
   hipStream_t stream_ = nullptr;
   hipStream_t side_ = nullptr;
diff --git a/ml-stable-diffusion_amd/python_hip_stable_diffusion/_lib.py b/ml-stable-diffusion_amd/python_hip_stable_diffusion/_lib.py
--- a/ml-stable-diffusion_amd/python_hip_stable_diffusion/_lib.py
+++ b/ml-stable-diffusion_amd/python_hip_stable_diffusion/_lib.py
@@ -84,6 +84,8 @@
     ("sd_op_groupnorm", _I, [_P, _FP, _FP, _P, _I, _I, _I, _I, _I, _F, _I, _I, _FP]),
     ("sd_op_groupnorm_shortcut", _I, [_P, _P, _FP, _FP, _P, _FP, _P, _P, _I, _I, _I, _I, _I, _I, _I, _F, _I, _I, _I, _FP]),
     ("sd_op_conv2d", _I, [_P, _P, _FP, _P, _P, _I, _I, _I, _I, _I, _I, _I, _I, _I, _I, _I, _I, _FP]),
+    ("sd_op_conv3x3_ex", _I, [_P, _P, _P, _FP, _FP, _P, _P, _FP, _I, _I, _I, _I, _I, _I, _I, _I, _I, _I, C.POINTER(_I), _I, _FP]),
+    ("sd_conv_bv_tiled_map", _I, [_I, _I, C.POINTER(_I), C.POINTER(_I), C.c_longlong]),
     ("sd_op_conv2d_groupnorm", _I, [_P, _P, _FP, _P, _FP, _FP, _P, _P, _I, _I, _I, _I, _I, _I, _I, _F, _I, _I, _I, C.POINTER(_I), _I, _FP]),
     ("sd_op_conv2d_groupnorm_proj", _I, [_P, _P, _FP, _P, _FP, _FP, _P, _FP, _P, _P, _I, _I, _I, _I, _I, _I, _I, _I, _F, _I, _I, C.POINTER(_I), _I, _FP]),
     ("sd_op_conv2d_groupnorm_conv3x3", _I, [_P, _P, _FP, _P, _FP, _FP, _P, _FP, _P, _P, _P, _I, _I, _I, _I, _I, _I, _I, _I, _F, _I, _I, _I, _I,
@@ -205,6 +207,36 @@
     return out, ms.value
 
 
+def conv3x3_ex(x0, w, x1=None, bias=None, temb=None, res=None, upsample=False, gn_groups=0, tile=0, splitk=0, iters=1):
+    x0, w = f16(x0), f16(w)
+    x1 = None if x1 is None else f16(x1)
+    B, C0, H, W = x0.shape
+    C1 = 0 if x1 is None else x1.shape[1]
+    Cout = w.shape[0]
+    if w.shape[1:] != (C0 + C1, 3, 3) or (x1 is not None and x1.shape != (B, C1, H, W)):
+        raise ValueError("conv3x3_ex: inconsistent shapes")
+    up = 2 if upsample else 1
+    bias = None if bias is None else f32(bias)
+    temb = None if temb is None else f32(temb)
+    if temb is not None and temb.shape != (B, Cout):
+        raise ValueError("conv3x3_ex: temb must be (B, Cout)")
+    res = None if res is None else f16(res)
+    out = np.empty((B, Cout, H * up, W * up), np.float16)
+    sums = np.zeros((B, gn_groups, 2), np.float32) if gn_groups > 0 else None
+    ms, entries = C.c_float(0), C.c_int(0)
+    check(lib().sd_op_conv3x3_ex(ptr(x0), ptr(x1), ptr(w), fptr(bias), fptr(temb), ptr(res), ptr(out), fptr(sums), B, C0, C1, H, W, Cout,
+                                 int(upsample), gn_groups, tile, splitk, C.byref(entries), iters, C.byref(ms)))
+    return out, sums, entries.value, ms.value
+
+
+def conv_bv_tiled_map(N, Ctot):
+    count = -(-N // 64) * (Ctot // 64) * 9 * 512
+    row, k = np.empty(count, np.int32), np.empty(count, np.int32)
+    ip = C.POINTER(C.c_int)
+    check(lib().sd_conv_bv_tiled_map(N, Ctot, row.ctypes.data_as(ip), k.ctypes.data_as(ip), count))
+    return row, k
+
+
 def groupnorm_shortcut(x0, x1, gn_weight, gn_bias, w, bias=None, groups=32, eps=1e-5, silu=True, side=True, iters=1):
     x0, w = f16(x0), f16(w)
     x1 = None if x1 is None else f16(x1)
```

Result: no change. 238.8 it/s (-0.9%).
